# StelaBou/stylegan_directions_face_reenactment

Measured on AMD Instinct MI355X. Metric: reenacted frames/sec @256x256, higher is better.
Workload: dtype f32 (operands as fp16 hi+lo, 3 MFMA products, f32 accumulate)

## Files before the change

### include/sgdfr.h

```cpp
#ifndef SGDFR_H
#define SGDFR_H

#include <stdint.h>

#ifdef __cplusplus
extern "C" {
#endif

#define SGDFR_ABI_VERSION 23

#define SGDFR_MODE_PLAIN3 0
#define SGDFR_MODE_UP3 1
#define SGDFR_MODE_DOWN3 2

#define SGDFR_ACT_NONE 0
#define SGDFR_ACT_LRELU 1

int sgdfr_abi_version(void);
const char* sgdfr_last_error(void);

int sgdfr_fused_bias_act_f32(const float* x, const float* bias, const float* ref, float* y, int64_t n,
                             int step_b, int size_b, int act, int grad, float alpha, float scale,
                             void* stream);

int sgdfr_upfirdn2d_f32(const float* x, const float* k, float* y, int major, int in_h, int in_w, int minor,
                        int kh, int kw, int up_x, int up_y, int down_x, int down_y, int pad_x0, int pad_x1,
                        int pad_y0, int pad_y1, void* stream);

#define SGDFR_DTYPE_F32 0
#define SGDFR_DTYPE_F16 1
#define SGDFR_DTYPE_F64 2
int sgdfr_fused_bias_act(const void* x, const void* bias, const void* ref, void* y, int64_t n, int step_b, int size_b, int act,
                         int grad, float alpha, float scale, int dtype, void* stream);
int sgdfr_upfirdn2d(const void* x, const void* k, void* y, int major, int in_h, int in_w, int minor, int kh, int kw, int up_x,
                    int up_y, int down_x, int down_y, int pad_x0, int pad_x1, int pad_y0, int pad_y1, int dtype, void* stream);

int sgdfr_linear_f32(const float* x, int64_t ldx, const float* w, const float* bias, float* y, int64_t ldy,
                     int M, int N, int K, float wscale, float bscale, int act, float slope, float gain,
                     void* stream);

int sgdfr_pixelnorm_f32(const float* x, float* y, int B, int D, float eps, void* stream);
int sgdfr_pixelnorm_bwd_f32(const float* x, const float* g, float* dx, int B, int D, float eps, void* stream);

int sgdfr_latent_prepare_f32(const float* w, int w_is_plus, const float* shift, int shift_is_plus,
                             int shift_layers, const float* trunc, float psi, float* out, int B, int L, int D,
                             void* stream);

int sgdfr_modconv_prepack_f32(const float* weight, float* wp, float* q, float* qt, int Cout, int Cin, int k,
                              void* stream);

int sgdfr_modconv_prepack_t_f32(const float* weight, float* wt, int Cout, int Cin, int k, int flip, void* stream);

int sgdfr_style_demod_f32(const float* style, int64_t ld_style, const float* mod_w, const float* mod_b,
                          const float* q, float* s, float* d, int B, int D, int Cin, int Cout, void* stream);

#define SGDFR_MAX_STYLE_LAYERS 40
typedef struct sgdfr_style_layer {
    const float* mod_w;
    const float* mod_b;
    const float* q;
    float* s;
    float* d;
    int cin, cout, latent_index;
    float* s_n;
    float* d_n;
    const unsigned* x_absmax;
    int x_log2, headroom;
} sgdfr_style_layer;
int sgdfr_styles_batched_f32(const float* latent, int B, int L, int D, const sgdfr_style_layer* layers, int n_layers,
                             void* stream);

int sgdfr_split_range_f32(const float* s, const float* d, float* s_n, float* d_n, const unsigned* x_absmax,
                          int x_absmax_bstride, int x_log2, int headroom, int B, int Cin, int Cout, void* stream);

int sgdfr_absmax_f32(const float* x, int64_t x_bstride, int64_t n_per_image, int B, unsigned* out, int per_image,
                     void* stream);

int sgdfr_modconv2d_fwd_f32(const float* x, int64_t x_bstride, const float* wp, const float* s, const float* d,
                            const float* noise, int64_t noise_bstride, const float* noise_w, const float* bias,
                            float* y, int B, int Cin, int Cout, int H, int W, int mode, int act, float slope,
                            float gain, void* stream);

int sgdfr_modconv2d_splitk_hint(int B, int Cin, int Cout, int H, int W, int mode);
int sgdfr_modconv2d_splitk_f32(const float* x, int64_t x_bstride, const float* wp, const float* s, const float* d,
                               const float* noise, int64_t noise_bstride, const float* noise_w, const float* bias, float* y,
                               float* partials, int splits, int B, int Cin, int Cout, int H, int W, int mode, int act,
                               float slope, float gain, void* stream);

int sgdfr_modconv_prepack_wino_f32(const float* weight, float* u, int Cout, int Cin, int transpose_flip, void* stream);
int sgdfr_modconv2d_wino_supported(int B, int Cin, int Cout, int H, int W);
int sgdfr_modconv2d_wino_f32(const float* x, int64_t x_bstride, const float* u, const float* s, const float* d,
                             const float* noise, int64_t noise_bstride, const float* noise_w, const float* bias,
                             const float* zeros, float* y, int B, int Cin, int Cout, int H, int W, int act, float slope,
                             float gain, void* stream);

int sgdfr_blur_bias_act_f32(const float* t, const float* fir, const float* noise, int64_t noise_bstride,
                            const float* noise_w, const float* bias, float* y, int B, int C, int H, int W, int act,
                            float slope, float gain, unsigned int* y_absmax, void* stream);

int sgdfr_blur_bias_act_split_f32(const float* t, const float* fir, const float* noise, int64_t noise_bstride,
                                  const float* noise_w, const float* bias, const float* s_next, unsigned short* xs, int B, int C,
                                  int H, int W, int64_t plane_stride, int arith, int wino, int act, float slope, float gain,
                                  unsigned int* sat, void* stream);

int sgdfr_torgb_fwd_f32(const float* x, const float* w_rgb, const float* s, const float* bias, const float* skip,
                        const float* fir, float* y, int B, int Cin, int H, int W, void* stream);

#define SGDFR_SPLIT_BF16 0
#define SGDFR_SPLIT_FP16 1
#define SGDFR_SPLIT_FP16F8 2
int64_t sgdfr_modconv_prepack_split_elems(int Cout, int Cin);
int sgdfr_modconv_prepack_split_f32(const float* weight, unsigned short* wsp, int Cout, int Cin, int arith, int transpose_flip,
                                    unsigned int* sat, void* stream);
int sgdfr_modconv2d_split_supported(int B, int Cin, int Cout, int H, int W, int mode);
int sgdfr_modconv2d_split_f8_ok(int B, int Cin, int Cout, int H, int W, int mode);
int sgdfr_modconv2d_split_f32(const float* x, int64_t x_bstride, const unsigned short* wsp, const float* s, const float* d,
                              const float* noise, int64_t noise_bstride, const float* noise_w, const float* bias,
                              const float* zeros, float* y, float* partials, int ksplit, const float* rgb_w,
                              const float* rgb_s, float* rgb_part, int x_is_split, unsigned short* xs_out, const float* s_next,
                              int B, int Cin, int Cout, int H, int W, int mode, int64_t plane_stride, int arith, int act,
                              float slope, float gain, unsigned int* sat, void* stream);
long long sgdfr_split_saturation_count(int reset);
int sgdfr_modconv2d_split_xin_supported(int B, int Cin, int Cout, int H, int W, int mode);
int sgdfr_to_split_f32(const float* x, const float* s, unsigned short* xs, int B, int Cin, int H, int W, int arith,
                       unsigned int* sat, void* stream);
int sgdfr_planes_to_split_f32(const float* gt, const float* d, unsigned short* xs, int B, int C, int H, int W, int arith,
                              unsigned int* sat, void* stream);
int sgdfr_blur_adjoint_split_f32(const float* g, const float* fir, const float* t, const float* d, unsigned short* xs,
                                 float* asum, int B, int C, int H, int W, int arith, unsigned int* sat, void* stream);
int sgdfr_modconv2d_split_cout_tiles(int B, int Cin, int Cout, int H, int W, int mode);
int sgdfr_modconv2d_split_cout_tiles_xin(int B, int Cin, int Cout, int H, int W, int mode);
int sgdfr_modconv2d_split_ksplit_hint(int B, int Cin, int Cout, int H, int W, int mode);
int sgdfr_modconv2d_split_plan_info(int B, int Cin, int Cout, int H, int W, int mode, int xin_whole);

int sgdfr_modconv2d_wsplit_supported(int B, int Cin, int Cout, int H, int W, int f);
int sgdfr_modconv2d_wsplit_wide(int B, int Cin, int Cout, int H, int W);
#define SGDFR_SPLIT_HANDOVER_F8 0x100
int64_t sgdfr_modconv_prepack_wsplit_elems(int Cout, int Cin, int f);
int sgdfr_modconv_prepack_wsplit_f32(const float* weight, unsigned short* wsp, int Cout, int Cin, int f, int arith,
                                     unsigned int* sat, void* stream);
int sgdfr_to_wsplit_f32(const float* x, const float* s, unsigned short* vs, int B, int Cin, int H, int W, int f, int arith,
                        unsigned int* sat, void* stream);
int sgdfr_modconv2d_wsplit_f32(const unsigned short* v, const unsigned short* wsp, const float* d, const float* noise,
                               int64_t noise_bstride, const float* noise_w, const float* bias, const float* zeros, float* y,
                               const float* rgb_w, const float* rgb_s, float* rgb_part, unsigned short* xs_out,
                               const float* s_next, int B, int Cin, int Cout, int H, int W, int f, int arith, int act,
                               float slope, float gain, unsigned int* sat, void* stream);

int sgdfr_torgb_finish_f32(const float* part, int T, const float* bias, const float* skip, const float* fir, float* y, int B,
                           int H, int W, void* stream);

int sgdfr_torgb_finish_u8_f32(const float* part, int T, const float* bias, const float* skip, const float* fir,
                              unsigned char* y, int64_t row_pitch, int x_offset, int swap_rb, int B, int H, int W,
                              void* stream);

int sgdfr_image_to_u8_f32(const float* x, unsigned char* y, int B, int H, int W, void* stream);

#define SGDFR_MAX_GRID_PANELS 4
int sgdfr_grid_to_u8_f32(const float* const* panels, const int64_t* bstrides, int K, unsigned char* y, int B, int H,
                         int W, int swap_rb, void* stream);


#define SGDFR_DIR_ZERO 0
#define SGDFR_DIR_ANGLE 1
#define SGDFR_DIR_JAW 2
#define SGDFR_DIR_EXP 3
#define SGDFR_MAX_DIRECTIONS 64
struct sgdfr_direction {
    int kind;
    int col;
    double a;
    double b;
};

int sgdfr_make_shift_f32(const float* ang_s, int64_t ang_s_bstride, const float* pose_s, int64_t pose_s_bstride,
                         const float* exp_s, int64_t exp_s_bstride, const float* ang_t, const float* pose_t,
                         const float* exp_t, int pose_dim, int exp_dim, const struct sgdfr_direction* table, int D,
                         float* shift, int N, int arith, void* stream);

int sgdfr_make_shift_random_f32(const float* ang_s, const float* pose_s, const float* exp_s, int pose_dim, int exp_dim,
                                const int* which, const float* u, float shift_scale, const struct sgdfr_direction* table,
                                int D, float* shift, int N, void* stream);

int sgdfr_gt_reenacted_f32(const float* pose_s, const float* exp_s, const float* ang_s, const float* pose_t, const float* exp_t,
                           int pose_dim, int exp_dim, const float* shift, const int* which, float shift_scale,
                           const struct sgdfr_direction* table, int D, float* pose_gt, float* exp_gt, int B, void* stream);

#define SGDFR_PAIRLOSS_PLAIN 0
#define SGDFR_PAIRLOSS_RANGE255 1
int64_t sgdfr_pairloss_workspace_bytes(int n);
int sgdfr_pairloss_forward_f32(const float* x, const float* y, int64_t n, int mode, float* x255, float* y255, float* loss,
                               void* workspace, int64_t workspace_bytes, void* stream);
int sgdfr_pairloss_backward_f32(const float* x, const float* y, int64_t n, int mode, const float* grad_loss,
                                const float* grad_x255, float* dx, void* stream);


struct sgdfr_sweep_record {
    double start;
    double min_shift;
    double max_shift;
    double step;
    int n_lo;
    int n_hi;
};

int sgdfr_sweep_plan_f32(const float* angles, const float* pose, const float* alpha_exp, int pose_dim, int exp_dim,
                         const struct sgdfr_direction* table, int D, const int* dirs, int K, double shift_scale, int shifts_count,
                         struct sgdfr_sweep_record* records, int N, void* stream);
int sgdfr_sweep_plan_host(const float* angles, const float* pose, const float* alpha_exp, int pose_dim, int exp_dim,
                          const struct sgdfr_direction* table, int D, const int* dirs, int K, double shift_scale, int shifts_count,
                          struct sgdfr_sweep_record* records, int N);

int sgdfr_sweep_rows_f32(const struct sgdfr_sweep_record* records, const int* row_offset, const struct sgdfr_direction* table, int D,
                         const int* dirs, int K, int N, float* rows, int* row_k, int* is_start, int R, void* stream);
int sgdfr_sweep_rows_host(const struct sgdfr_sweep_record* records, const struct sgdfr_direction* table, int D, const int* dirs, int K,
                          int N, float* rows, int* row_k, int* is_start, int64_t R);

int sgdfr_sweep_frames_f32(const float* x, int R, int P, int f, const int* is_start, const float* src, int64_t src_bstride,
                           float* pooled, float* bordered, unsigned char* frames, int panels, void* stream);

int sgdfr_video_frames_f32(const float* x, int B, int P, int f, const float* const* panels, const int64_t* bstrides, int n_left,
                           unsigned char* frames, int swap_rb, void* stream);

#define SGDFR_PANEL_F32 0
#define SGDFR_PANEL_U8 1
struct sgdfr_video_panel {
    const void* data;
    const int* index;
    int kind;
    int rows;
};

int sgdfr_video_frames_px(const float* x, int B, int P, int f, const struct sgdfr_video_panel* panels, int n_left,
                          unsigned char* frames, int swap_rb, void* stream);


int sgdfr_act_grad_reduce_f32(const float* g_out, const float* out, const float* noise, int64_t noise_bstride,
                              const float* noise_w, const float* bias, float* g_pre, float* sums, int B, int C, int HW,
                              float slope, float gain, int want_y, unsigned int* g_absmax, void* stream);

int sgdfr_blur_adjoint_f32(const float* g, const float* fir, const float* t, float* gt, float* asum, int B, int C, int H,
                           int W, void* stream);

int sgdfr_scale_reduce_f32(const float* gu, const float* x, int64_t x_bstride, const float* s, float* dx, float* r, int B,
                           int C, int HW, void* stream);

int sgdfr_torgb_bwd_f32(const float* x, const float* g, const float* w_rgb, const float* s, float* dx, float* r, int B,
                        int Cin, int H, int W, void* stream);

int sgdfr_grad_join_f32(const float* out, const float* gu, const float* s_next, const float* g_rgb, const float* w_rgb,
                        const float* s_rgb, const float* g_add, const float* noise, int64_t noise_bstride, const float* noise_w,
                        const float* bias, float* g_pre, float* sums, unsigned int* g_absmax, float* r_next, float* r_rgb, int B,
                        int C, int HW, float slope, float gain, int want_y, int zero_outputs, void* stream);

typedef struct sgdfr_style_grad_layer {
    const float* gs;
    const float* rgb_r;
    const float* rgb_w;
    const float* a;
    const float* d;
    const float* s;
    const float* qt;
    const float* mod_w;
    float* ds;
    float* gmod_w;
    float* gmod_b;
    int64_t a_stride;
    int cin, cout, latent_index;
} sgdfr_style_grad_layer;
int sgdfr_styles_batched_bwd_f32(const sgdfr_style_grad_layer* layers, int n_layers, const float* latent, float* glat, int B, int L,
                                 int D, void* stream);

int sgdfr_demod_dq_f32(const float* a, int64_t a_stride, const float* d, const float* s, float* dq, int B, int Cin, int Cout,
                       void* stream);

#define SGDFR_PGRAD_BIAS 0
#define SGDFR_PGRAD_NOISE 1
#define SGDFR_PGRAD_RGB_W 2
#define SGDFR_PGRAD_RGB_B 3
#define SGDFR_MAX_PARAM_GRADS 64
typedef struct sgdfr_param_grad {
    const float* in;
    const float* aux;
    float* out;
    int kind, C, HW;
    float scale;
} sgdfr_param_grad;
int sgdfr_param_grads_f32(const sgdfr_param_grad* entries, int n, int B, void* stream);

#define SGDFR_MAX_ADAM_TENSORS 96
typedef struct sgdfr_adam_tensor {
    float* p;
    const float* g;
    float* m;
    float* v;
    int64_t n;
} sgdfr_adam_tensor;
int sgdfr_adam_f32(const sgdfr_adam_tensor* tensors, int n, const float* step, float lr, float beta1, float beta2, float eps, void* stream);

int sgdfr_demod_grad_f32(const float* gd, const float* d, const float* qt, const float* s, const float* gs, float* ds,
                         int B, int Cin, int Cout, void* stream);

int sgdfr_modconv_wgrad_f32(const float* g, const float* d, const float* x, int64_t x_bstride, const float* s, float* dwp,
                            int B, int Cin, int Cout, int H, int W, int mode, void* stream);

int sgdfr_modconv_wgrad_finish_f32(const float* dwp, const float* wp, const float* dq, float* dweight, int Cout, int Cin,
                                   void* stream);
int sgdfr_modconv_wgrad_ksplit(int B, int Cin, int Cout, int H, int W, int mode);
// ... 150 lines not shown
```

### stylegan_directions_face_reenactment_amd/_native.py

```python
import ctypes
import os

import torch

_HERE = os.path.dirname(os.path.abspath(__file__))
LIB_PATH = os.path.join(_HERE, 'csrc', 'libsgdfr_hip.so')
if os.environ.get('SGDFR_LIB'):
    if os.environ.get('SGDFR_ALLOW_LIB_OVERRIDE') == '1':
        import sys as _sys
        LIB_PATH = os.environ['SGDFR_LIB']
        _sys.stderr.write('stylegan_directions_face_reenactment_amd: loading the native library from SGDFR_LIB=%s\n' % LIB_PATH)
    else:
        import warnings as _warnings
        _warnings.warn('SGDFR_LIB is set but ignored (set SGDFR_ALLOW_LIB_OVERRIDE=1 to load a probe build)', RuntimeWarning)
ABI_VERSION = 23

_c_f32p = ctypes.c_void_p
_i, _i64, _f = ctypes.c_int, ctypes.c_int64, ctypes.c_float

SIGNATURES = {
    'sgdfr_fused_bias_act_f32': [_c_f32p, _c_f32p, _c_f32p, _c_f32p, _i64, _i, _i, _i, _i, _f, _f, ctypes.c_void_p],
    'sgdfr_upfirdn2d_f32': [_c_f32p, _c_f32p, _c_f32p] + [_i] * 14 + [ctypes.c_void_p],
    'sgdfr_linear_f32': [_c_f32p, _i64, _c_f32p, _c_f32p, _c_f32p, _i64, _i, _i, _i, _f, _f, _i, _f, _f,
                         ctypes.c_void_p],
    'sgdfr_pixelnorm_f32': [_c_f32p, _c_f32p, _i, _i, _f, ctypes.c_void_p],
    'sgdfr_pixelnorm_bwd_f32': [_c_f32p, _c_f32p, _c_f32p, _i, _i, _f, ctypes.c_void_p],
    'sgdfr_latent_prepare_f32': [_c_f32p, _i, _c_f32p, _i, _i, _c_f32p, _f, _c_f32p, _i, _i, _i, ctypes.c_void_p],
    'sgdfr_modconv_prepack_f32': [_c_f32p, _c_f32p, _c_f32p, _c_f32p, _i, _i, _i, ctypes.c_void_p],
    'sgdfr_modconv_prepack_t_f32': [_c_f32p, _c_f32p, _i, _i, _i, _i, ctypes.c_void_p],
    'sgdfr_act_grad_reduce_f32': [_c_f32p, _c_f32p, _c_f32p, _i64, _c_f32p, _c_f32p, _c_f32p, _c_f32p, _i, _i, _i, _f,
                                  _f, _i, ctypes.c_void_p, ctypes.c_void_p],
    'sgdfr_blur_adjoint_f32': [_c_f32p, _c_f32p, _c_f32p, _c_f32p, _c_f32p, _i, _i, _i, _i, ctypes.c_void_p],
    'sgdfr_scale_reduce_f32': [_c_f32p, _c_f32p, _i64, _c_f32p, _c_f32p, _c_f32p, _i, _i, _i, ctypes.c_void_p],
    'sgdfr_torgb_bwd_f32': [_c_f32p, _c_f32p, _c_f32p, _c_f32p, _c_f32p, _c_f32p, _i, _i, _i, _i, ctypes.c_void_p],
    'sgdfr_modconv_wgrad_f32': [_c_f32p, _c_f32p, _c_f32p, _i64, _c_f32p, _c_f32p, _i, _i, _i, _i, _i, _i, ctypes.c_void_p],
    'sgdfr_modconv_wgrad_finish_f32': [_c_f32p, _c_f32p, _c_f32p, _c_f32p, _i, _i, ctypes.c_void_p],
    'sgdfr_modconv_wgrad_parts_f32': [_c_f32p, _c_f32p, _c_f32p, _i64, _c_f32p, _c_f32p, _i, _i, _i, _i, _i, _i, ctypes.c_void_p],
    'sgdfr_modconv_wgrad_finish_parts_f32': [_c_f32p, _i, _c_f32p, _c_f32p, _c_f32p, _i, _i, ctypes.c_void_p],
    'sgdfr_modconv_wgrad_finish_parts_oik_f32': [_c_f32p, _i, _c_f32p, _c_f32p, _c_f32p, _i64, _c_f32p, _c_f32p, _i, _c_f32p, _i, _i,
                                                 ctypes.c_void_p],
    'sgdfr_modconv_prepack_wino_f32': [_c_f32p, _c_f32p, _i, _i, _i, ctypes.c_void_p],
    'sgdfr_modconv2d_wino_supported': [_i, _i, _i, _i, _i],
    'sgdfr_modconv2d_wino_f32': [_c_f32p, _i64, _c_f32p, _c_f32p, _c_f32p, _c_f32p, _i64, _c_f32p, _c_f32p, _c_f32p,
                                 _c_f32p, _i, _i, _i, _i, _i, _i, _f, _f, ctypes.c_void_p],
    'sgdfr_modconv_prepack_split_f32': [_c_f32p, ctypes.c_void_p, _i, _i, _i, _i, ctypes.c_void_p, ctypes.c_void_p],
    'sgdfr_modconv2d_split_supported': [_i, _i, _i, _i, _i, _i],
    'sgdfr_modconv2d_split_f32': [_c_f32p, _i64, ctypes.c_void_p, _c_f32p, _c_f32p, _c_f32p, _i64, _c_f32p, _c_f32p, _c_f32p,
                                  _c_f32p, _c_f32p, _i, _c_f32p, _c_f32p, _c_f32p, _i, ctypes.c_void_p, _c_f32p, _i, _i, _i, _i,
                                  _i, _i, _i64, _i, _i, _f, _f, ctypes.c_void_p, ctypes.c_void_p],
    'sgdfr_to_split_f32': [_c_f32p, _c_f32p, ctypes.c_void_p, _i, _i, _i, _i, _i, ctypes.c_void_p, ctypes.c_void_p],
    'sgdfr_planes_to_split_f32': [_c_f32p, _c_f32p, ctypes.c_void_p, _i, _i, _i, _i, _i, ctypes.c_void_p, ctypes.c_void_p],
    'sgdfr_blur_adjoint_split_f32': [_c_f32p, _c_f32p, _c_f32p, _c_f32p, ctypes.c_void_p, _c_f32p, _i, _i, _i, _i, _i, ctypes.c_void_p,
                                     ctypes.c_void_p],
    'sgdfr_modconv2d_split_cout_tiles': [_i, _i, _i, _i, _i, _i],
    'sgdfr_modconv2d_split_cout_tiles_xin': [_i, _i, _i, _i, _i, _i],
    'sgdfr_modconv2d_split_xin_supported': [_i, _i, _i, _i, _i, _i],
    'sgdfr_modconv2d_split_ksplit_hint': [_i, _i, _i, _i, _i, _i],
    'sgdfr_modconv2d_split_plan_info': [_i, _i, _i, _i, _i, _i, _i],
    'sgdfr_torgb_finish_f32': [_c_f32p, _i, _c_f32p, _c_f32p, _c_f32p, _c_f32p, _i, _i, _i, ctypes.c_void_p],
    'sgdfr_torgb_finish_u8_f32': [_c_f32p, _i, _c_f32p, _c_f32p, _c_f32p, ctypes.c_void_p, _i64, _i, _i, _i, _i, _i, ctypes.c_void_p],
    'sgdfr_image_to_u8_f32': [_c_f32p, ctypes.c_void_p, _i, _i, _i, ctypes.c_void_p],
    'sgdfr_grid_to_u8_f32': [ctypes.POINTER(ctypes.c_void_p), ctypes.POINTER(ctypes.c_int64), _i, ctypes.c_void_p, _i, _i, _i,
                             _i, ctypes.c_void_p],
    'sgdfr_modconv2d_splitk_hint': [_i, _i, _i, _i, _i, _i],
    'sgdfr_modconv2d_splitk_f32': [_c_f32p, _i64, _c_f32p, _c_f32p, _c_f32p, _c_f32p, _i64, _c_f32p, _c_f32p, _c_f32p,
                                   _c_f32p, _i, _i, _i, _i, _i, _i, _i, _i, _f, _f, ctypes.c_void_p],
    'sgdfr_demod_grad_f32': [_c_f32p, _c_f32p, _c_f32p, _c_f32p, _c_f32p, _c_f32p, _i, _i, _i, ctypes.c_void_p],
    'sgdfr_style_demod_f32': [_c_f32p, _i64, _c_f32p, _c_f32p, _c_f32p, _c_f32p, _c_f32p, _i, _i, _i, _i,
                              ctypes.c_void_p],
    'sgdfr_modconv2d_fwd_f32': [_c_f32p, _i64, _c_f32p, _c_f32p, _c_f32p, _c_f32p, _i64, _c_f32p, _c_f32p, _c_f32p,
                                _i, _i, _i, _i, _i, _i, _i, _f, _f, ctypes.c_void_p],
    'sgdfr_blur_bias_act_f32': [_c_f32p, _c_f32p, _c_f32p, _i64, _c_f32p, _c_f32p, _c_f32p, _i, _i, _i, _i, _i, _f,
                                _f, ctypes.c_void_p, ctypes.c_void_p],
    'sgdfr_blur_bias_act_split_f32': [_c_f32p, _c_f32p, _c_f32p, _i64, _c_f32p, _c_f32p, _c_f32p, ctypes.c_void_p, _i, _i, _i, _i, _i64,
                                      _i, _i, _i, _f, _f, ctypes.c_void_p, ctypes.c_void_p],
    'sgdfr_torgb_fwd_f32': [_c_f32p, _c_f32p, _c_f32p, _c_f32p, _c_f32p, _c_f32p, _c_f32p, _i, _i, _i, _i,
                            ctypes.c_void_p],
}



class Direction(ctypes.Structure):
    _fields_ = [('kind', ctypes.c_int), ('col', ctypes.c_int), ('a', ctypes.c_double), ('b', ctypes.c_double)]


DIR_ZERO, DIR_ANGLE, DIR_JAW, DIR_EXP = 0, 1, 2, 3
MAX_DIRECTIONS = 64
SIGNATURES['sgdfr_make_shift_f32'] = [_c_f32p, _i64, _c_f32p, _i64, _c_f32p, _i64, _c_f32p, _c_f32p, _c_f32p, _i, _i,
                                      ctypes.POINTER(Direction), _i, _c_f32p, _i, _i, ctypes.c_void_p]
SIGNATURES['sgdfr_make_shift_random_f32'] = [_c_f32p, _c_f32p, _c_f32p, _i, _i, ctypes.c_void_p, _c_f32p, _f,
                                             ctypes.POINTER(Direction), _i, _c_f32p, _i, ctypes.c_void_p]
SIGNATURES['sgdfr_gt_reenacted_f32'] = [_c_f32p, _c_f32p, _c_f32p, _c_f32p, _c_f32p, _i, _i, _c_f32p, ctypes.c_void_p, _f,
                                        ctypes.POINTER(Direction), _i, _c_f32p, _c_f32p, _i, ctypes.c_void_p]


class StyleLayer(ctypes.Structure):
    _fields_ = [('mod_w', ctypes.c_void_p), ('mod_b', ctypes.c_void_p), ('q', ctypes.c_void_p),
                ('s', ctypes.c_void_p), ('d', ctypes.c_void_p), ('cin', ctypes.c_int), ('cout', ctypes.c_int),
                ('latent_index', ctypes.c_int), ('s_n', ctypes.c_void_p), ('d_n', ctypes.c_void_p),
                ('x_absmax', ctypes.c_void_p), ('x_log2', ctypes.c_int), ('headroom', ctypes.c_int)]


SIGNATURES['sgdfr_split_range_f32'] = [_c_f32p, _c_f32p, _c_f32p, _c_f32p, ctypes.c_void_p, _i, _i, _i, _i, _i, _i, ctypes.c_void_p]
SIGNATURES['sgdfr_absmax_f32'] = [_c_f32p, _i64, _i64, _i, ctypes.c_void_p, _i, ctypes.c_void_p]
SIGNATURES['sgdfr_styles_batched_f32'] = [_c_f32p, _i, _i, _i, ctypes.POINTER(StyleLayer), _i, ctypes.c_void_p]
MAX_STYLE_LAYERS = 40


class StyleGradLayer(ctypes.Structure):
    _fields_ = [('gs', ctypes.c_void_p), ('rgb_r', ctypes.c_void_p), ('rgb_w', ctypes.c_void_p), ('a', ctypes.c_void_p),
                ('d', ctypes.c_void_p), ('s', ctypes.c_void_p), ('qt', ctypes.c_void_p), ('mod_w', ctypes.c_void_p),
                ('ds', ctypes.c_void_p), ('gmod_w', ctypes.c_void_p), ('gmod_b', ctypes.c_void_p), ('a_stride', ctypes.c_longlong),
                ('cin', ctypes.c_int), ('cout', ctypes.c_int), ('latent_index', ctypes.c_int)]


class ParamGrad(ctypes.Structure):
    _fields_ = [('inp', ctypes.c_void_p), ('aux', ctypes.c_void_p), ('out', ctypes.c_void_p), ('kind', ctypes.c_int), ('C', ctypes.c_int),
                ('HW', ctypes.c_int), ('scale', ctypes.c_float)]


class AdamTensor(ctypes.Structure):
    _fields_ = [('p', ctypes.c_void_p), ('g', ctypes.c_void_p), ('m', ctypes.c_void_p), ('v', ctypes.c_void_p), ('n', ctypes.c_int64)]


MAX_ADAM_TENSORS = 96
SIGNATURES['sgdfr_adam_f32'] = [ctypes.POINTER(AdamTensor), _i, _c_f32p, _f, _f, _f, _f, ctypes.c_void_p]
PGRAD_BIAS, PGRAD_NOISE, PGRAD_RGB_W, PGRAD_RGB_B = 0, 1, 2, 3
MAX_PARAM_GRADS = 64
SIGNATURES['sgdfr_styles_batched_bwd_f32'] = [ctypes.POINTER(StyleGradLayer), _i, _c_f32p, _c_f32p, _i, _i, _i, ctypes.c_void_p]
SIGNATURES['sgdfr_demod_dq_f32'] = [_c_f32p, _i64, _c_f32p, _c_f32p, _c_f32p, _i, _i, _i, ctypes.c_void_p]
SIGNATURES['sgdfr_param_grads_f32'] = [ctypes.POINTER(ParamGrad), _i, _i, ctypes.c_void_p]
SIGNATURES['sgdfr_grad_join_f32'] = ([_c_f32p] * 7 + [_c_f32p, _i64, _c_f32p, _c_f32p, _c_f32p, _c_f32p, ctypes.c_void_p,
                                                                  _c_f32p, _c_f32p, _i, _i, _i, _f, _f, _i, _i, ctypes.c_void_p])
SIGNATURES['sgdfr_modconv2d_wsplit_supported'] = [_i, _i, _i, _i, _i, _i]
SIGNATURES['sgdfr_modconv2d_wsplit_wide'] = [_i, _i, _i, _i, _i]
SIGNATURES['sgdfr_modconv2d_split_f8_ok'] = [_i, _i, _i, _i, _i, _i]
SPLIT_HANDOVER_F8 = 0x100
SIGNATURES['sgdfr_modconv_prepack_wsplit_f32'] = [_c_f32p, ctypes.c_void_p, _i, _i, _i, _i, ctypes.c_void_p, ctypes.c_void_p]
SIGNATURES['sgdfr_to_wsplit_f32'] = [_c_f32p, _c_f32p, ctypes.c_void_p, _i, _i, _i, _i, _i, _i, ctypes.c_void_p, ctypes.c_void_p]
SIGNATURES['sgdfr_modconv2d_wsplit_f32'] = [ctypes.c_void_p, ctypes.c_void_p, _c_f32p, _c_f32p, _i64, _c_f32p, _c_f32p, _c_f32p, _c_f32p,
                                            _c_f32p, _c_f32p, _c_f32p, ctypes.c_void_p, _c_f32p, _i, _i, _i, _i, _i, _i, _i, _i, _f, _f,
                                            ctypes.c_void_p, ctypes.c_void_p]
SIGNATURES['sgdfr_fused_bias_act'] = [ctypes.c_void_p, ctypes.c_void_p, ctypes.c_void_p, ctypes.c_void_p, _i64, _i, _i, _i, _i, _f, _f, _i,
                                      ctypes.c_void_p]
SIGNATURES['sgdfr_upfirdn2d'] = [ctypes.c_void_p, ctypes.c_void_p, ctypes.c_void_p] + [_i] * 15 + [ctypes.c_void_p]
SIGNATURES['sgdfr_lpips_prepack_f32'] = [ctypes.POINTER(ctypes.c_void_p), _c_f32p, ctypes.c_void_p]
SIGNATURES['sgdfr_lpips_features_f32'] = [_c_f32p, _i, _c_f32p, _i, _i, _i, _c_f32p, _c_f32p, ctypes.c_void_p, _i64, ctypes.c_void_p]
SIGNATURES['sgdfr_lpips_distance_f32'] = [_c_f32p, _i, _c_f32p, _i, _i, _i, _i, _i, _i, _c_f32p, _c_f32p, ctypes.c_void_p, _i64,
                                          ctypes.c_void_p]
SIGNATURES['sgdfr_lpips_backward_f32'] = [_c_f32p, _c_f32p, _i, _c_f32p, _i, _i, _i, _i, _i, _i, _c_f32p, _c_f32p, ctypes.c_void_p, _i64,
                                          ctypes.c_void_p]
LPIPS_PARAMS = 17
SIGNATURES['sgdfr_idloss_prepack_f32'] = [ctypes.POINTER(ctypes.c_void_p), _c_f32p, ctypes.c_void_p]
SIGNATURES['sgdfr_idloss_forward_f32'] = [_c_f32p, _i, _c_f32p, _i, _i, _i, _i, _c_f32p, _c_f32p, _c_f32p, ctypes.c_void_p, _i64,
                                          ctypes.c_void_p]
SIGNATURES['sgdfr_idloss_backward_f32'] = [_c_f32p, _c_f32p, _i, _i, _i, _i, _c_f32p, _c_f32p, ctypes.c_void_p, _i64, ctypes.c_void_p]
IDLOSS_PARAMS = 245
SIGNATURES['sgdfr_flame_prepack_f32'] = [ctypes.POINTER(ctypes.c_void_p), _i, _i, _i, _i, _i, _i, _c_f32p, ctypes.c_void_p]
SIGNATURES['sgdfr_flame_decode_f32'] = [_c_f32p, _c_f32p, _c_f32p, _i, _c_f32p, _c_f32p, _c_f32p, _i, _c_f32p, _c_f32p, _i, _c_f32p, _c_f32p,
                                        _c_f32p, _c_f32p, ctypes.c_void_p]
SIGNATURES['sgdfr_flame_decode_backward_f32'] = [_c_f32p, _c_f32p, _c_f32p, _c_f32p, _i, _c_f32p, _i, _c_f32p, _c_f32p, _c_f32p, _c_f32p,
                                                 _c_f32p, ctypes.c_void_p, _i64, ctypes.c_void_p]
SIGNATURES['sgdfr_shape_loss_f32'] = [_c_f32p, _c_f32p, _i, _f, _f, _f, _c_f32p, _c_f32p, _c_f32p, _c_f32p, ctypes.c_void_p, _i64,
                                      ctypes.c_void_p]
FLAME_PARAMS = 15
SIGNATURES['sgdfr_deca_prepack_f32'] = [ctypes.POINTER(ctypes.c_void_p), _c_f32p, ctypes.c_void_p]
SIGNATURES['sgdfr_deca_forward_f32'] = [_c_f32p, _c_f32p, _i, _i, _i, _c_f32p, _c_f32p, _c_f32p, _c_f32p, ctypes.c_void_p, _c_f32p,
                                        ctypes.c_void_p, _i64, ctypes.c_void_p]
SIGNATURES['sgdfr_deca_backward_f32'] = [_c_f32p, _c_f32p, _c_f32p, ctypes.c_void_p, _i, _i, _i, _c_f32p, _c_f32p, ctypes.c_void_p, _i64,
                                         ctypes.c_void_p]
SIGNATURES['sgdfr_deca_crop_f32'] = [_c_f32p, _c_f32p, _i, _i, _i, _c_f32p, ctypes.c_void_p]
SIGNATURES['sgdfr_deca_crop_backward_f32'] = [_c_f32p, _c_f32p, _c_f32p, _i, _i, _i, _c_f32p, ctypes.c_void_p]
DECA_PARAMS = 134
SIGNATURES['sgdfr_fan_prepack_f32'] = [ctypes.POINTER(ctypes.c_void_p), _c_f32p, ctypes.c_void_p]
SIGNATURES['sgdfr_fan_crop_f32'] = [_c_f32p, _c_f32p, _i, _i, _i, _i, _c_f32p, ctypes.c_void_p]
SIGNATURES['sgdfr_fan_network_f32'] = [_c_f32p, _i, _c_f32p, _c_f32p, _c_f32p, ctypes.c_void_p, _i64, ctypes.c_void_p]
SIGNATURES['sgdfr_fan_decode_f32'] = [_c_f32p, _c_f32p, _i, _c_f32p, _c_f32p, _c_f32p, ctypes.c_void_p]
SIGNATURES['sgdfr_fan_boxes_f32'] = [_c_f32p, _i, _c_f32p, ctypes.c_void_p]
SIGNATURES['sgdfr_fan_forward_f32'] = [_c_f32p, _c_f32p, _i, _i, _i, _i, _c_f32p, _c_f32p, _c_f32p, _c_f32p, _c_f32p, _c_f32p,
                                       ctypes.c_void_p, _i64, ctypes.c_void_p]
FAN_PARAMS = 735
FAN_RANGE_255, FAN_RANGE_GAN = 0, 1
SIGNATURES['sgdfr_fan_flip_add_f32'] = [_c_f32p, _i, _c_f32p, ctypes.c_void_p]
SIGNATURES['sgdfr_fan_draw_f32'] = [_c_f32p, _i, _c_f32p, ctypes.c_void_p]
SIGNATURES['sgdfr_fan_forward3d_f32'] = ([_c_f32p, _c_f32p, _i, _i, _i, _i, _i] + [_c_f32p] * 11 + [ctypes.c_void_p, _i64, ctypes.c_void_p,
                                                                                                     _i64, ctypes.c_void_p])
SIGNATURES['sgdfr_fandepth_prepack_f32'] = [ctypes.POINTER(ctypes.c_void_p), _c_f32p, ctypes.c_void_p]
SIGNATURES['sgdfr_fandepth_network_f32'] = [_c_f32p, _c_f32p, _i, _c_f32p, _c_f32p, _c_f32p, ctypes.c_void_p, _i64, ctypes.c_void_p]
FANDEPTH_PARAMS = 312
_ip = ctypes.c_void_p
SIGNATURES['sgdfr_s3fd_level_dims'] = [_i, _i, ctypes.POINTER(ctypes.c_int)]
SIGNATURES['sgdfr_s3fd_prepack_f32'] = [ctypes.POINTER(ctypes.c_void_p), _c_f32p, ctypes.c_void_p]
SIGNATURES['sgdfr_s3fd_network_f32'] = [_c_f32p, _i, _i, _i, _i, _c_f32p, _c_f32p, _c_f32p, ctypes.c_void_p, _i64, ctypes.c_void_p]
SIGNATURES['sgdfr_s3fd_candidates_f32'] = [ctypes.POINTER(ctypes.c_void_p), ctypes.POINTER(ctypes.c_int), _i, _f, _i, _c_f32p, _ip, _ip,
                                           ctypes.c_void_p]
SIGNATURES['sgdfr_s3fd_nms_f32'] = [_c_f32p, _ip, _i, _i, _c_f32p, _ip, _ip, ctypes.c_void_p]
SIGNATURES['sgdfr_s3fd_forward_f32'] = [_c_f32p, _i, _i, _i, _i, _c_f32p, _f, _i, _c_f32p, _ip, _ip, _c_f32p, _ip, _ip, _c_f32p, _c_f32p,
                                        ctypes.c_void_p, _i64, ctypes.c_void_p]
S3FD_PARAMS = 50
SIGNATURES['sgdfr_e4e_prepack_f32'] = [ctypes.POINTER(ctypes.c_void_p), _i, _c_f32p, ctypes.c_void_p]
SIGNATURES['sgdfr_e4e_forward_f32'] = [_c_f32p, _i, _i, _c_f32p, _c_f32p, _c_f32p, ctypes.c_void_p, _i64, ctypes.c_void_p]
_u8p = ctypes.c_void_p
# ... 163 lines not shown
```

### stylegan_directions_face_reenactment_amd/chain.py

```python
import torch

from . import _native as N
from .config import config
from .functional import (_shape_query, blur_bias_act, blur_bias_act_split, modconv_split, modconv_wsplit, split_ok, wsplit_ok)


class SplitAct:
    __slots__ = ('xs', 'shape', 'wino', 'arith')

    def __init__(self, xs, shape, wino=0, arith=None):
        self.xs, self.shape, self.wino = xs, tuple(shape), (2 if wino is True else int(wino or 0))
        self.arith = arith


def xin_ok(B, cin, cout, H, W, mode=N.MODE_PLAIN3):
    return config().use_split_chain and split_ok(B, cin, cout, H, W, mode) and \
        bool(_shape_query('sgdfr_modconv2d_split_xin_supported', B, cin, cout, H, W, mode))


def styled_conv_split(x, wsp, s, d, cout, upsample=False, fir=None, noise=None, noise_weight=None, bias=None, batch=None,
                      s_next=None, rgb=None, want_y=True, wino_next=False, arith_next=None, xs_arith=None):
    if isinstance(x, SplitAct) and x.wino:
        if upsample:
            raise RuntimeError('styled_conv_split: the Winograd input form feeds plain convs only')
        B, cin, H, W = x.shape
        res = modconv_wsplit(x.xs, x.shape, wsp, d, cout, noise, noise_weight, bias, True, rgb=rgb,
                             want_y=want_y and s_next is None, s_next=s_next, f=x.wino, arith=x.arith,
                             xs_arith=xs_arith if s_next is not None else None)
        if s_next is not None:
            _, part, xs = res
            return SplitAct(xs, (B, cout, H, W), arith=xs_arith), part
        return res if rgb is not None else (res, None)
    x_arith = None
    if isinstance(x, SplitAct):
        B, cin, H, W = x.shape
        xin, x_split, s_arg = x.xs, x.shape, None
        batch = B
        x_arith = x.arith
    else:
        xin, x_split, s_arg = x, None, s
        B = s.shape[0] if batch is None else batch
        H, W = x.shape[2], x.shape[3]
    if not upsample:
        res = modconv_split(xin, wsp, s_arg, d, cout, noise, noise_weight, bias, True, batch=batch, rgb=rgb,
                            want_y=want_y and s_next is None, x_split=x_split, s_next=s_next, arith=x_arith)
        if s_next is not None:
            _, part, xs = res
            return SplitAct(xs, (B, cout, H, W)), part
        return res if rgb is not None else (res, None)
    if s_next is not None and config().use_plane_padding and \
            _shape_query('sgdfr_modconv2d_split_ksplit_hint', B, x_split[1] if x_split else x.shape[1], cout, H, W, N.MODE_UP3) == 1:
        ps = ((H + 1) * (W + 1) + 31) // 32 * 32
        planes = modconv_split(xin, wsp, s_arg, d, cout, batch=batch, mode=N.MODE_UP3, x_split=x_split, plane_stride=ps, arith=x_arith)
        xs = blur_bias_act_split(planes, fir, H, W, s_next, noise, noise_weight, bias, True, plane_stride=ps, wino=wino_next,
                                 arith=arith_next if wino_next != 2 else None)
        return SplitAct(xs, (B, cout, 2 * H, 2 * W), wino_next, arith_next if wino_next != 2 else None), None
    planes = modconv_split(xin, wsp, s_arg, d, cout, batch=batch, mode=N.MODE_UP3, x_split=x_split, arith=x_arith)
    if s_next is not None:
        xs = blur_bias_act_split(planes, fir, H, W, s_next, noise, noise_weight, bias, True, wino=wino_next,
                                 arith=arith_next if wino_next != 2 else None)
        return SplitAct(xs, (B, cout, 2 * H, 2 * W), wino_next, arith_next if wino_next != 2 else None), None
    return blur_bias_act(planes, fir, H, W, noise, noise_weight, bias, True), None


def _interleaved_planes_ok(B, cin, H, W):
    import os
    if not config().use_plane_padding or os.environ.get('SGDFR_PLANE_IL', '1') == '0':
        return False
    return all(_shape_query('sgdfr_modconv2d_split_ksplit_hint', B, c, cin, H // 2, W // 2, N.MODE_UP3) == 1 for c in (cin, 2 * cin))


def wsplit_chain_f(B, cin, cout, H, W):
    if not (config().use_wsplit and config().use_split_chain and config().wsplit_min_cin > 0 and cin >= config().wsplit_min_cin and W <= 256):
        return 0
    if W > 128 and not _interleaved_planes_ok(B, cin, H, W):
        return 0
    for f in ((4, 2) if config().wsplit_f == 4 else (2,)):
        if wsplit_ok(B, cin, cout, H, W, f) and (f == 4 or cin >= max(config().wsplit_min_cin, 256)) and (W <= 128 or f == 4):
            return f
    return 0


def _f8_cross_on():
    return config().precision == 'fp16x3' and config().cross_terms == 'fp8' and config().range_plan is True


def wsplit_chain_arith(B, cin, cout, H, W, f):
    if f == 4 and _f8_cross_on() and cin % 32 == 0 and \
            _shape_query('sgdfr_modconv2d_wsplit_wide', B, cin, cout, H, W):
        return 'fp16f8'
    return None


def xs_chain_arith(B, cin, cout, H, W, nxt_cout):
    if _f8_cross_on() and \
            _shape_query('sgdfr_modconv2d_split_f8_ok', B, cout, nxt_cout, H, W, N.MODE_UP3) and \
            _shape_query('sgdfr_modconv2d_split_ksplit_hint', B, cout, nxt_cout, H, W, N.MODE_UP3) == 1:
        return 'fp16f8'
    return None


def xs_plain_arith(B, cin, cout, H, W):
    if _f8_cross_on() and \
            _shape_query('sgdfr_modconv2d_split_f8_ok', B, cin, cout, H, W, N.MODE_PLAIN3) and \
            _shape_query('sgdfr_modconv2d_split_ksplit_hint', B, cin, cout, H, W, N.MODE_PLAIN3) == 1:
        return 'fp16f8'
    return None


def wsplit_chain_ok(B, cin, cout, H, W):
    return wsplit_chain_f(B, cin, cout, H, W) != 0


def rgb_fusable(B, cin, cout, H, W):
    return config().use_rgb_fusion and split_ok(B, cin, cout, H, W) and \
        (not config().use_splitk or _shape_query('sgdfr_modconv2d_split_ksplit_hint', B, cin, cout, H, W, N.MODE_PLAIN3) == 1)


class StreamPipeline:

    def __init__(self, n=2, device=None):
        self.streams = [torch.cuda.Stream(device=device) for _ in range(max(1, int(n)))]
        self._i = 0
        self.last = None

    def next(self):
        s = self.streams[self._i % len(self.streams)]
        self._i += 1
        s.wait_stream(torch.cuda.current_stream(s.device))
        self.last = s
        return torch.cuda.stream(s)

    def join(self, *tensors, stream=None):
        cur = torch.cuda.current_stream(self.streams[0].device)
        for s in ([stream] if stream is not None else self.streams):
            cur.wait_stream(s)
        for t in tensors:
            if isinstance(t, torch.Tensor) and t.is_cuda:
                t.record_stream(cur)
```

### stylegan_directions_face_reenactment_amd/csrc/split.hip

```cpp
#include "split_kernel.h"

namespace sgdfr {

template <int ET>
__global__ __launch_bounds__(256) void to_split_kernel(const float* __restrict__ x, const float* __restrict__ s,
                                                      unsigned char* __restrict__ xs, int B, int Cin, int HW,
                                                      unsigned* __restrict__ sat_word) {
    const int G = Cin / 8;
    const int64_t n = (int64_t)B * G * HW;
    unsigned sat = 0;
    for (int64_t idx = (int64_t)blockIdx.x * blockDim.x + threadIdx.x; idx < n; idx += (int64_t)gridDim.x * blockDim.x) {
        const int pix = (int)(idx % HW);
        const int64_t bg = idx / HW;
        const int g = (int)(bg % G);
        const int b = (int)(bg / G);
        const float* xp = x + ((int64_t)b * Cin + g * 8) * HW + pix;
        const float* sp = s + (int64_t)b * Cin + g * 8;
        uint4 vh, vl;
        unsigned* ph = reinterpret_cast<unsigned*>(&vh);
        unsigned* pl = reinterpret_cast<unsigned*>(&vl);
        constexpr int ETM = ws_main_et<ET>::value;
        const float sc = (ETM == SGDFR_SPLIT_FP16) ? SPLIT_F16_XSCALE : 1.f;
#pragma unroll
        for (int c = 0; c < 4; ++c)
// ... 145 lines not shown
            p.simgs = 1;
        } else if (PT % HW == 0) {
            span = (PT / HW - 1) * p.R * p.P + (H - 1) * p.P + (W - 1);
            p.simgs = PT / HW;
        } else {
            return 0;
        }
        p.xlen = span + 2 * p.P + 3;
        p.n_pix_tiles = (int)((p.total_pix + PT - 1) / PT);
    }
    const bool slim = plan.cfg == 8;
    p.xs = (plan.nw == 8 || slim) ? (p.xlen + 63) & ~63 : (p.xlen + 7) & ~7;
    p.n_cout_tiles = (Cout + plan.nt - 1) / plan.nt;
    const int nthr = plan.nw * 64;
    if ((2 * p.xs + nthr - 1) / nthr > (mode == SGDFR_MODE_DOWN3 ? 3 : 4)) return 0;
    const size_t lds = split_lds_bytes(p, plan.nt, plan.nss, down, 2, plan.pt, slim);
    if (lds > (plan.nw == 8 ? 160 : 80) * 1024) return 0;
    if (slim && p.simgs > 2) return 0;
    if (out) *out = p;
    return 1;
}

static const SplitPlan* split_plan(int B, int Cin, int Cout, int H, int W, int mode, SplitParams* out, bool xin_whole = false) {
    static const int deep = getenv("SGDFR_SPLIT_DEEP") ? atoi(getenv("SGDFR_SPLIT_DEEP")) : 1;
    static const int narrow_first = getenv("SGDFR_SPLIT_UP_NARROW") ? atoi(getenv("SGDFR_SPLIT_UP_NARROW")) : 0;
    const SplitPlan* order[6] = {nullptr, nullptr, nullptr, nullptr, nullptr, nullptr};
    int n = 0;
    if (mode == SGDFR_MODE_UP3) {
        const bool big = (int64_t)B * (H + 1) * (W + 1) * (Cout / 64) >= 256 * 256;
        if (deep && big) order[n++] = &kPlanUpDeep;
        if (narrow_first && big) order[n++] = &kPlanUpNarrow;
        if (Cout % 128 == 0) order[n++] = &kPlanUpWide;
        order[n++] = &kPlanUpNarrow;
    } else if (mode == SGDFR_MODE_PLAIN3) {
        static const int xl = getenv("SGDFR_SPLIT_XL") ? atoi(getenv("SGDFR_SPLIT_XL")) : 1;
        if (xl && xin_whole && Cout % 128 == 0 && (int64_t)B * H * W * (Cout / 128) >= 2ll * 256 * 512) order[n++] = &kPlanPlainXL;
        const int p4 = getenv("SGDFR_SPLIT_P4") ? atoi(getenv("SGDFR_SPLIT_P4")) : 64;
        const bool p4_ok = p4 > 0 && xin_whole && Cin <= p4 && (int64_t)B * H * W * ((Cout + 63) / 64) >= 4ll * 512 * 256;
        if (p4_ok && Cout % 128 == 0 && p4 >= 128) order[n++] = &kPlanPlain4;
        if (Cout % 128 == 0) order[n++] = &kPlanPlainWide;
        if (p4_ok) order[n++] = &kPlanPlain4;
        order[n++] = &kPlanPlainNarrow;
    } else if (mode == SGDFR_MODE_DOWN3) {
        order[n++] = &kPlanDown;
    }
    for (int i = 0; i < n; ++i)
        if (split_geometry(B, Cin, Cout, H, W, mode, *order[i], out)) return order[i];
    return nullptr;
}


extern "C" int sgdfr_modconv2d_split_supported(int B, int Cin, int Cout, int H, int W, int mode) {
    SplitParams p;
    return split_plan(B, Cin, Cout, H, W, mode, &p) ? 1 : 0;
}

extern "C" int sgdfr_modconv2d_split_f8_ok(int B, int Cin, int Cout, int H, int W, int mode) {
    SplitParams p;
    if (mode != SGDFR_MODE_UP3 && mode != SGDFR_MODE_PLAIN3) return 0;
    const SplitPlan* plan = split_plan(B, Cin, Cout, H, W, mode, &p, true);
    return plan && plan->cfg == (mode == SGDFR_MODE_UP3 ? 4 : 8) ? 1 : 0;
}

extern "C" int sgdfr_modconv2d_split_ksplit_hint(int B, int Cin, int Cout, int H, int W, int mode) {
    SplitParams p;
    if (!split_plan(B, Cin, Cout, H, W, mode, &p)) return 1;
    const int blocks = p.n_pix_tiles * p.n_cout_tiles;
    if (blocks >= 192) return 1;
    static const int target = getenv("SGDFR_SPLIT_KTARGET") ? atoi(getenv("SGDFR_SPLIT_KTARGET")) : 256;
    int s = target / blocks;
    const int max_by_k = (Cin / SPLIT_CB) / 2;
    if (s > max_by_k) s = max_by_k;
    if (s > 16) s = 16;
    return s < 2 ? 1 : s;
}

extern "C" int sgdfr_to_split_f32(const float* x, const float* s, unsigned short* xs, int B, int Cin, int H, int W, int arith,
                                  unsigned int* sat, void* stream) {
    SGDFR_REQUIRE(B >= 0 && Cin > 0 && Cin % 8 == 0 && H > 0 && W > 0, "to_split: bad shape B=%d Cin=%d H=%d W=%d (Cin %% 8)", B, Cin, H, W);
    SGDFR_REQUIRE(arith == SGDFR_SPLIT_BF16 || arith == SGDFR_SPLIT_FP16 || arith == SGDFR_SPLIT_FP16F8, "to_split: arith must be SGDFR_SPLIT_BF16/FP16/FP16F8");
    if (B == 0) return 0;
    SGDFR_REQUIRE(x && s && xs && (reinterpret_cast<uintptr_t>(xs) & 15) == 0, "to_split: null or misaligned pointer");
    int64_t g = ((int64_t)B * (Cin / 8) * H * W + 255) / 256;
    if (g > 256 * 32) g = 256 * 32;
    if (arith == SGDFR_SPLIT_FP16F8)
        hipLaunchKernelGGL(to_split_kernel<SGDFR_SPLIT_FP16F8>, dim3((int)g), dim3(256), 0, as_stream(stream), x, s,
                           reinterpret_cast<unsigned char*>(xs), B, Cin, H * W, sat);
    else if (arith == SGDFR_SPLIT_FP16)
        hipLaunchKernelGGL(to_split_kernel<SGDFR_SPLIT_FP16>, dim3((int)g), dim3(256), 0, as_stream(stream), x, s,
                           reinterpret_cast<unsigned char*>(xs), B, Cin, H * W, sat);
    else
        hipLaunchKernelGGL(to_split_kernel<SGDFR_SPLIT_BF16>, dim3((int)g), dim3(256), 0, as_stream(stream), x, s,
                           reinterpret_cast<unsigned char*>(xs), B, Cin, H * W, sat);
    return check_launch("to_split");
}

extern "C" int sgdfr_planes_to_split_f32(const float* gt, const float* d, unsigned short* xs, int B, int C, int H, int W,
                                        int arith, unsigned int* sat, void* stream) {
    SGDFR_REQUIRE(B >= 0 && C > 0 && C % 8 == 0 && H > 0 && W > 0, "planes_to_split: bad shape B=%d C=%d H=%d W=%d (C %% 8)", B, C, H, W);
    SGDFR_REQUIRE(arith == SGDFR_SPLIT_BF16 || arith == SGDFR_SPLIT_FP16, "planes_to_split: arith must be SGDFR_SPLIT_BF16/FP16");
    if (B == 0) return 0;
    SGDFR_REQUIRE(gt && xs && (reinterpret_cast<uintptr_t>(xs) & 15) == 0, "planes_to_split: null or misaligned pointer");
    const int RP = (H + 1) * (W + 1);
    int64_t g = ((int64_t)B * 4 * (C / 8) * RP + 255) / 256;
    if (g > 256 * 32) g = 256 * 32;
    if (arith == SGDFR_SPLIT_FP16)
        hipLaunchKernelGGL(planes_to_split_kernel<SGDFR_SPLIT_FP16>, dim3((int)g), dim3(256), 0, as_stream(stream), gt, d,
                           reinterpret_cast<unsigned char*>(xs), B, C, RP, sat);
    else
        hipLaunchKernelGGL(planes_to_split_kernel<SGDFR_SPLIT_BF16>, dim3((int)g), dim3(256), 0, as_stream(stream), gt, d,
                           reinterpret_cast<unsigned char*>(xs), B, C, RP, sat);
    return check_launch("planes_to_split");
}

unsigned int blur_split_saturation_count(int reset);
namespace sgdfr { unsigned int wsplit_saturation_count(int reset); }

extern "C" long long sgdfr_split_saturation_count(int reset) {
    unsigned int v = 0;
    if (hipMemcpyFromSymbol(&v, HIP_SYMBOL(g_split_saturated), sizeof(v)) != hipSuccess) return -1;
    if (reset) {
        const unsigned int z = 0;
        if (hipMemcpyToSymbol(HIP_SYMBOL(g_split_saturated), &z, sizeof(z)) != hipSuccess) return -1;
    }
    return (long long)v + (long long)blur_split_saturation_count(reset) + (long long)sgdfr::wsplit_saturation_count(reset);
}

#ifdef SGDFR_SPLIT_PROBE
extern "C" int sgdfr_split_trace_read(unsigned long long* out, int n) {
    if (n > 4096) n = 4096;
    if (hipDeviceSynchronize() != hipSuccess) return 1;
    return hipMemcpyFromSymbol(out, HIP_SYMBOL(g_split_trace), sizeof(unsigned long long) * n) == hipSuccess ? 0 : 1;
}
#endif

extern "C" int sgdfr_modconv2d_split_xin_supported(int B, int Cin, int Cout, int H, int W, int mode) {
    SplitParams p;
    const SplitPlan* plan = split_plan(B, Cin, Cout, H, W, mode, &p);
    if (!plan || !(plan->cfg == 0 || plan->cfg == 1 || plan->cfg == 3 || plan->cfg == 4 || plan->cfg == 5)) return 0;
    if (plan->nss == 3 && plan->cfg != 5 && split_lds_bytes(p, plan->nt, plan->nss, false, 3) > 160 * 1024) return 0;
    return 1;
}

extern "C" int sgdfr_modconv2d_split_cout_tiles(int B, int Cin, int Cout, int H, int W, int mode) {
    SplitParams p;
    return split_plan(B, Cin, Cout, H, W, mode, &p) ? p.n_cout_tiles : 0;
}

extern "C" int sgdfr_modconv2d_split_cout_tiles_xin(int B, int Cin, int Cout, int H, int W, int mode) {
    SplitParams p;
    return split_plan(B, Cin, Cout, H, W, mode, &p, true) ? p.n_cout_tiles : 0;
}

extern "C" int sgdfr_modconv2d_split_plan_info(int B, int Cin, int Cout, int H, int W, int mode, int xin_whole) {
    SplitParams p;
    const SplitPlan* plan = split_plan(B, Cin, Cout, H, W, mode, &p, xin_whole != 0);
    if (!plan) return -1;
    const int nthr = plan->nw * 64, nex = (2 * p.xs + nthr - 1) / nthr;
    const int nex_max = mode == SGDFR_MODE_DOWN3 ? 3 : 4;
    const int half = (plan->nt == 64 && Cout % 64 == 32) ? 1 : 0;
    return plan->cfg | (nex <= 2 ? 2 : nex == 3 ? 3 : nex_max) << 4 | p.simgs << 8 | half << 20;
}

static int64_t split_pack_body_elems(int n_out, int n_in) { return (int64_t)((n_out + 63) / 64 * 64) * n_in * 9 * 2; }
extern "C" int64_t sgdfr_modconv_prepack_split_elems(int Cout, int Cin) { return split_pack_body_elems(Cout, Cin) + 8; }

extern "C" int sgdfr_modconv_prepack_split_f32(const float* weight, unsigned short* wsp, int Cout, int Cin, int arith,
                                               int transpose_flip, unsigned int* sat, void* stream) {
    SGDFR_REQUIRE(arith == SGDFR_SPLIT_BF16 || arith == SGDFR_SPLIT_FP16 || (arith == SGDFR_SPLIT_FP16F8 && transpose_flip == 0),
                  "prepack_split: arith must be SGDFR_SPLIT_BF16/FP16 (or FP16F8 for a forward pack)");
    SGDFR_REQUIRE(transpose_flip >= 0 && transpose_flip <= 2, "prepack_split: transpose_flip is 0 (forward), 1 (adjoint of "
                  "the plain conv) or 2 (adjoint of the transposed conv)");
    const int n_out = transpose_flip ? Cin : Cout, n_in = transpose_flip ? Cout : Cin;
    SGDFR_REQUIRE(Cout > 0 && Cin > 0 && n_in % SPLIT_CB == 0 && (n_out % 64 == 0 || (transpose_flip == 0 && n_out % 64 == 32)),
                  "prepack_split: needs in-channels %% 16 == 0 and out-channels %% 64 == 0 (forward pack: %% 32), got in=%d out=%d",
                  n_in, n_out);
    SGDFR_REQUIRE(weight && wsp, "prepack_split: null pointer");
    if (n_out % 64 != 0) {
        if (hipMemsetAsync(wsp, 0, sizeof(unsigned short) * (size_t)split_pack_body_elems(Cout, Cin), as_stream(stream)) !=
            hipSuccess) {
            set_error("prepack_split: hipMemsetAsync failed");
            return 2;
        }
    }
    const int64_t n = (int64_t)Cout * Cin * 9;
    int64_t g = (n + 255) / 256;
    if (g > 4096) g = 4096;
    const float scale = (arith != SGDFR_SPLIT_BF16 ? SPLIT_F16_WSCALE : 1.f) / sqrtf((float)Cin * 9);
    {
        unsigned* const trailer = reinterpret_cast<unsigned*>(wsp + split_pack_body_elems(n_out, n_in));
        if (hipMemsetAsync(trailer, 0, 16, as_stream(stream)) != hipSuccess) { (void)hipGetLastError(); set_error("prepack_split: hipMemsetAsync failed"); return 2; }
        if (arith == SGDFR_SPLIT_FP16F8) hipLaunchKernelGGL(split_absmax_kernel, dim3(256), dim3(256), 0, as_stream(stream), weight, n, scale, trailer);
    }
    hipLaunchKernelGGL(prepack_split_kernel, dim3((int)g), dim3(256), 0, as_stream(stream), weight, wsp, Cout, Cin,
                       64, scale, arith, transpose_flip, sat);
    return check_launch("modconv_prepack_split");
}

template <int MODE, int ET, int WM, int WN, int MI, int NI, int NSS = 3, bool XIN = false>
static int launch_split(const SplitParams& p, hipStream_t st, int lid0 = 0, int count = -1) {
    constexpr int NTHR = WM * WN * 64;
    const int nex = (2 * p.xs + NTHR - 1) / NTHR;
    constexpr int NEX_MAX = (MODE == SGDFR_MODE_DOWN3) ? 3 : 4;
    SGDFR_REQUIRE(nex <= NEX_MAX, "modconv_split: staged range %d too long for mode %d", p.xlen, MODE);
    void (*kern)(SplitParams) = nex <= 2   ? split_mfma_kernel<MODE, ET, WM, WN, MI, NI, 2, NSS, XIN>
                                : nex == 3 ? split_mfma_kernel<MODE, ET, WM, WN, MI, NI, 3, NSS, XIN>
                                           : split_mfma_kernel<MODE, ET, WM, WN, MI, NI, NEX_MAX, NSS, XIN>;
    const size_t lds = split_lds_bytes(p, WM * MI * 32, NSS, MODE == SGDFR_MODE_DOWN3,
                                       (XIN && MODE != SGDFR_MODE_DOWN3 && NSS == 3 && NI <= 2 && WM * WN == 8) ? 3 : 2, WN * NI * 32,
                                       XIN && WM * WN == 4);
    if (hipFuncSetAttribute(reinterpret_cast<const void*>(kern), hipFuncAttributeMaxDynamicSharedMemorySize, (int)lds) !=
        hipSuccess) {
        (void)hipGetLastError();
        set_error("modconv_split: LDS request %zu B refused (B=%d Cin=%d Cout=%d H=%d W=%d xs=%d simgs=%d)", lds, p.B, p.Cin, p.Cout,
                  p.H, p.W, p.xs, p.simgs);
        return 2;
    }
    SplitParams q = p;
    q.total_blocks = count >= 0 ? count : p.n_pix_tiles * p.n_cout_tiles * p.ksplit;
    q.lid0 = lid0;
    static const int persist = getenv("SGDFR_SPLIT_PERSIST") ? atoi(getenv("SGDFR_SPLIT_PERSIST")) : 256;
    static const int persist_min = getenv("SGDFR_SPLIT_PERSIST_MIN") ? atoi(getenv("SGDFR_SPLIT_PERSIST_MIN")) : 4;
    static const int persist_min_up = getenv("SGDFR_SPLIT_PERSIST_MIN_UP") ? atoi(getenv("SGDFR_SPLIT_PERSIST_MIN_UP")) : 4;
    constexpr bool kCanPersist = XIN && NSS == 3 && WM * WN == 8 && (MODE == SGDFR_MODE_PLAIN3 || MODE == SGDFR_MODE_UP3);
    const bool persistent = kCanPersist && persist > 0 &&
                            q.total_blocks >= (MODE == SGDFR_MODE_UP3 ? persist_min_up : persist_min) * persist;
    const int grid = persistent ? persist : q.total_blocks;
    hipLaunchKernelGGL(kern, dim3(grid), dim3(NTHR), lds, st, q);
    return check_launch("modconv2d_split");
}

template <int MODE, int ET, int MI, bool XIN>
static int launch_deep_tail(const SplitParams& p, hipStream_t st) {
    const char* env = getenv("SGDFR_SPLIT_UP_TAIL");
    const int total = p.n_pix_tiles * p.n_cout_tiles;
    const int n_full = total / 256 * 256, tail = total - n_full;
    const int max_full = (env && atoi(env) > 1) ? atoi(env) : (MODE == SGDFR_MODE_DOWN3 ? 1024 : 512);
    if ((env && atoi(env) == 0) || p.ksplit != 1 || n_full == 0 || n_full > max_full || tail == 0 || tail > 128)
        return launch_split<MODE, ET, 2, 4, MI, 2, 1, XIN>(p, st);
    if (int rc = launch_split<MODE, ET, 2, 4, MI, 2, 1, XIN>(p, st, 0, n_full)) return rc;
    SplitParams t = p;
    constexpr int PT2 = 128;
    t.xlen = PT2 + p.P + 2;
    t.xs = (t.xlen + 63) & ~63;
    t.simgs = (t.xlen - 1) / p.rps + 2;
    t.n_pix_tiles = (int)((p.total_pix + PT2 - 1) / PT2);
    t.desync = 0;
    fill_fastdivs(t);
    const int c0 = n_full / p.n_pix_tiles, p0 = n_full - c0 * p.n_pix_tiles;
    const int lid0 = c0 * t.n_pix_tiles + 2 * p0;
    const int count = t.n_cout_tiles * t.n_pix_tiles - lid0;
    if (count <= 0) return 0;
    return launch_split<MODE, ET, 2, 4, MI, 1, 1, XIN>(t, st, lid0, count);
}

template <int ET>
static int launch_plan(int cfg, const SplitParams& p, hipStream_t st, bool xin) {
    if (xin) {
        switch (cfg) {
            case 0: return launch_split<SGDFR_MODE_PLAIN3, ET, 2, 4, 2, 2, 3, true>(p, st);
            case 1: return launch_split<SGDFR_MODE_PLAIN3, ET, 1, 8, 2, 2, 3, true>(p, st);
            case 3: return launch_split<SGDFR_MODE_UP3, ET, 2, 4, 1, 2, 3, true>(p, st);
            case 4: return launch_deep_tail<SGDFR_MODE_UP3, ET, 1, true>(p, st);
            case 5: return launch_deep_tail<SGDFR_MODE_DOWN3, ET, 2, true>(p, st);
            case 6: return launch_split<SGDFR_MODE_PLAIN3, ET, 2, 4, 2, 4, 3, true>(p, st);
            case 8: return launch_split<SGDFR_MODE_PLAIN3, ET, 1, 4, 2, 2, 3, true>(p, st);
            default: set_error("modconv_split: pre-split input is not built for tiling plan %d", cfg); return 1;
        }
    }
    if (cfg == 5) {
        set_error("modconv_split: DOWN3 reads the phase-major split planes of sgdfr_planes_to_split_f32 (x_is_split = 1)");
        return 1;
    }
    switch (cfg) {
        case 0: return launch_split<SGDFR_MODE_PLAIN3, ET, 2, 4, 2, 2, 3>(p, st);
        case 1: return launch_split<SGDFR_MODE_PLAIN3, ET, 1, 8, 2, 2, 3>(p, st);
        case 2: return launch_split<SGDFR_MODE_UP3, ET, 4, 2, 1, 2, 3>(p, st);
        case 3: return launch_split<SGDFR_MODE_UP3, ET, 2, 4, 1, 2, 3>(p, st);
        default: return launch_deep_tail<SGDFR_MODE_UP3, ET, 1, false>(p, st);
    }
}

extern "C" int sgdfr_modconv2d_split_f32(const float* x, int64_t x_bstride, const unsigned short* wsp, const float* s,
                                         const float* d, const float* noise, int64_t noise_bstride, const float* noise_w,
                                         const float* bias, const float* zeros, float* y, float* partials, int ksplit,
                                         const float* rgb_w, const float* rgb_s, float* rgb_part, int x_is_split,
                                         unsigned short* xs_out, const float* s_next, int B, int Cin, int Cout, int H, int W,
                                         int mode, int64_t plane_stride, int arith, int act, float slope, float gain,
                                         unsigned int* sat, void* stream) {
    SGDFR_REQUIRE(arith == SGDFR_SPLIT_BF16 || arith == SGDFR_SPLIT_FP16 ||
                      (arith == SGDFR_SPLIT_FP16F8 && sgdfr_modconv2d_split_f8_ok(B, Cin, Cout, H, W, mode) && x_is_split && ksplit <= 1),
                  "modconv_split: arith must be SGDFR_SPLIT_BF16/FP16 (FP16F8: only where sgdfr_modconv2d_split_f8_ok() says so, with a "
                  "pre-split input and no K slices)");
    SGDFR_REQUIRE(B >= 0 && Cin > 0 && Cout > 0 && H > 0 && W > 0, "modconv_split: bad shape B=%d Cin=%d Cout=%d H=%d W=%d",
                  B, Cin, Cout, H, W);
    if (B == 0) return 0;
    SGDFR_REQUIRE(sgdfr_modconv2d_split_supported(B, Cin, Cout, H, W, mode),
                  "modconv_split: shape B=%d Cin=%d Cout=%d H=%d W=%d mode=%d not supported; use sgdfr_modconv2d_fwd_f32", B,
                  Cin, Cout, H, W, mode);
    SGDFR_REQUIRE(mode == SGDFR_MODE_PLAIN3 || (!noise && !bias && !act), "modconv_split: UP3 writes raw parity planes "
                  "(noise / bias / activation belong to sgdfr_blur_bias_act_f32), DOWN3 a raw gradient");
    SGDFR_REQUIRE(mode != SGDFR_MODE_DOWN3 || (x_is_split && y && !rgb_part && !xs_out), "modconv_split: DOWN3 takes "
                  "pre-split planes and writes y only");
    SGDFR_REQUIRE(x && wsp && zeros && (y || rgb_part || xs_out) && (s || x_is_split), "modconv_split: null pointer");
    SGDFR_REQUIRE(!xs_out || (s_next && mode == SGDFR_MODE_PLAIN3 && ksplit <= 1 && Cout % 8 == 0 &&
                              (reinterpret_cast<uintptr_t>(xs_out) & 15) == 0),
                  "modconv_split: xs_out needs s_next, mode PLAIN3, ksplit == 1 and a 16-byte aligned buffer");
    SGDFR_REQUIRE(!x_is_split || (x_bstride != 0 && (reinterpret_cast<uintptr_t>(x) & 15) == 0),
                  "modconv_split: a pre-split input is per image and 16-byte aligned");
    SGDFR_REQUIRE(!noise || noise_w, "modconv_split: noise without noise_w");
    SGDFR_REQUIRE(((reinterpret_cast<uintptr_t>(wsp) | reinterpret_cast<uintptr_t>(s)) & 15) == 0,
                  "modconv_split: wsp and s must be 16-byte aligned");
    SplitParams p;
    const SplitPlan* plan = split_plan(B, Cin, Cout, H, W, mode, &p, x_is_split != 0 && ksplit <= 1);
    if (plane_stride != 0) {
        SGDFR_REQUIRE(mode == SGDFR_MODE_UP3 && plane_stride >= (int64_t)p.R * p.P && plane_stride < (1 << 30) && ksplit <= 1,
                      "modconv_split: plane_stride is for UP3 launches without K slices, >= (H+1)*(W+1)");
        p.rps = (int)plane_stride;
        static const int il_env = getenv("SGDFR_PLANE_IL") ? atoi(getenv("SGDFR_PLANE_IL")) : 1;
        p.plane_il = il_env;
        p.total_pix = (int64_t)B * p.rps;
        SGDFR_REQUIRE(p.total_pix + 4ll * p.P + 8 < (1ll << 31), "modconv_split: padded position space too large");
        p.n_pix_tiles = (int)((p.total_pix + plan->pt - 1) / plan->pt);
        p.simgs = (p.xlen - 1) / p.rps + 2;
    }
    p.f8_max = nullptr;
    p.x = x; p.x_bstride = x_bstride; p.wsp = wsp; p.s = s; p.d = d; p.noise = noise; p.noise_bstride = noise_bstride;
    p.noise_w = noise_w; p.bias = bias; p.zeros = zeros; p.y = y;
    p.act = act; p.slope = slope; p.gain = gain; p.sat = sat;
    if (ksplit < 1) ksplit = 1;
    SGDFR_REQUIRE(!rgb_part || (rgb_w && rgb_s && mode == SGDFR_MODE_PLAIN3 && ksplit == 1),
                  "modconv_split: the fused ToRGB needs rgb_w, rgb_s, mode PLAIN3 and ksplit == 1");
    p.rgb_w = rgb_w; p.rgb_s = rgb_s; p.rgb_part = rgb_part;
    p.xs_out = reinterpret_cast<unsigned char*>(xs_out); p.s_next = s_next;
    SGDFR_REQUIRE(ksplit == 1 || (partials && ksplit <= Cin / SPLIT_CB), "modconv_split: ksplit %d needs a partials buffer "
                  "and at most %d slices", ksplit, Cin / SPLIT_CB);
    const int64_t n_out = (mode == SGDFR_MODE_UP3) ? (int64_t)B * Cout * 4 * p.rps : (int64_t)B * Cout * H * W;
    p.ksplit = ksplit;
    p.split_stride = n_out;
    if (ksplit > 1) p.y = partials;
    static const int stagger = getenv("SGDFR_SPLIT_STAGGER") ? atoi(getenv("SGDFR_SPLIT_STAGGER")) : 1;
    p.stagger = stagger;
    p.dbg = getenv("SGDFR_SPLIT_DBG") ? atoi(getenv("SGDFR_SPLIT_DBG")) : 0;
    {
        static const int pct = getenv("SGDFR_SPLIT_DESYNC") ? atoi(getenv("SGDFR_SPLIT_DESYNC")) : 75;
        const bool up = mode == SGDFR_MODE_UP3;
        const double mfma_clk = (double)(Cin / SPLIT_CB / ksplit) * (up ? 54 : 108) * 32 * 2 / 0.55;
        const double store_clk = (double)plan->nt * plan->pt * (up ? 4 : 1) * 4 / 8.3;
        const int blocks = p.n_pix_tiles * p.n_cout_tiles * ksplit;
        p.desync = (up && pct > 0 && blocks >= 1024) ? (int)((mfma_clk + store_clk) * pct / 100 / 4096) : 0;
    }
    fill_fastdivs(p);
    hipStream_t st = as_stream(stream);
    if (arith == SGDFR_SPLIT_FP16F8) {
        p.f8_max = reinterpret_cast<const float*>(wsp + split_pack_body_elems(Cout, Cin));
        return mode == SGDFR_MODE_UP3 ? launch_split<SGDFR_MODE_UP3, SGDFR_SPLIT_FP16F8, 2, 4, 1, 2, 1, true>(p, st)
                                      : launch_split<SGDFR_MODE_PLAIN3, SGDFR_SPLIT_FP16F8, 1, 4, 2, 2, 3, true>(p, st);
    }
    const int rc = arith == SGDFR_SPLIT_FP16 ? launch_plan<SGDFR_SPLIT_FP16>(plan->cfg, p, st, x_is_split != 0)
                                             : launch_plan<SGDFR_SPLIT_BF16>(plan->cfg, p, st, x_is_split != 0);
    if (rc || ksplit == 1) return rc;
    const bool plain = mode == SGDFR_MODE_PLAIN3;
    return launch_splitk_reduce(partials, ksplit, n_out, plain ? noise : nullptr, noise_bstride, noise_w, plain ? bias : nullptr, y,
                                Cout, plain ? H * W : 1, plain ? act : 0, slope, gain, st);
}
```

### stylegan_directions_face_reenactment_amd/csrc/split_kernel.h

```cpp
#pragma once
#include <stdlib.h>

#include <type_traits>

#include "common.h"

namespace sgdfr {

typedef float f32x16 __attribute__((ext_vector_type(16)));
typedef __bf16 bf16x8 __attribute__((ext_vector_type(8)));
typedef __bf16 bf16x2 __attribute__((ext_vector_type(2)));
typedef _Float16 f16x8 __attribute__((ext_vector_type(8)));
typedef _Float16 f16x2 __attribute__((ext_vector_type(2)));
typedef float f32x2 __attribute__((ext_vector_type(2)));
typedef int frag128 __attribute__((ext_vector_type(4)));

template <int ET>
__device__ __forceinline__ f32x16 split_mfma(frag128 a, frag128 b, f32x16 c) {
    if (ET == SGDFR_SPLIT_FP16 || ET == SGDFR_SPLIT_FP16F8)
        return __builtin_amdgcn_mfma_f32_32x32x16_f16(__builtin_bit_cast(f16x8, a), __builtin_bit_cast(f16x8, b), c, 0, 0, 0);
    return __builtin_amdgcn_mfma_f32_32x32x16_bf16(__builtin_bit_cast(bf16x8, a), __builtin_bit_cast(bf16x8, b), c, 0, 0, 0);
}
static __device__ unsigned int g_split_saturated = 0;

#ifdef SGDFR_SPLIT_PROBE
__device__ unsigned long long g_split_trace[4096];
#define SPLIT_TRACE(id)                                                                                              \
    do {                                                                                                             \
        if (trace_on) {                                                                                              \
            if (ntrace < 4094)                                                                                       \
                g_split_trace[1 + ntrace] = ((unsigned long long)(id) << 48) | (__builtin_amdgcn_s_memtime() & 0xffffffffffffull); \
            ++ntrace;                                                                                                \
        }                                                                                                            \
    } while (0)
#else
#define SPLIT_TRACE(id) do {} while (0)
#endif

#define SGDFR_MODE_UPF 3

constexpr float SPLIT_F16_XSCALE = 0.0625f, SPLIT_F16_WSCALE = 64.f, SPLIT_F16_OUT = 0.25f, SPLIT_F16_MAX = 65504.f;

struct SplitParams {
    const float* x;
    int64_t x_bstride;
    const unsigned short* wsp;
    const float* s;
    const float* d;
    const float* noise;
    int64_t noise_bstride;
    const float* noise_w;
    const float* bias;
    const float* zeros;
    float* y;
    const float* rgb_w;
    const float* rgb_s;
    float* rgb_part;
    unsigned char* xs_out;
    const float* s_next;
    unsigned* sat;
    int B, Cin, Cout, H, W;
    int P, R;
    int n_pix_tiles, n_cout_tiles;
    int xs, xlen;
    int patch;
    int TC, TR, tiles_x, tiles_y, seglen;
    int simgs;
    int64_t total_pix;
    int act;
    float slope, gain;
    int ksplit;
    int64_t split_stride;
    int desync;
    int stagger;
    int dbg;
    int total_blocks;
    int rps;
    int plane_il;
    int tstep_r, tstep_c, torg;
    int tpos;
    const float* fir;
    const float* f8_max;
    FastDiv fd_xs, fd_seglen, fd_P, fd_R, fd_RP, fd_rps, fd_HW, fd_W, fd_TC, fd_tiles_x, fd_per_img, fd_npt, fd_tps, fd_Cin;
    int lid0;
};

static void fill_fastdivs(SplitParams& p) {
    p.fd_xs = make_fastdiv(p.xs); p.fd_seglen = make_fastdiv(p.seglen); p.fd_P = make_fastdiv(p.P); p.fd_R = make_fastdiv(p.R);
    p.fd_RP = make_fastdiv(p.R * p.P); p.fd_rps = make_fastdiv(p.rps); p.fd_HW = make_fastdiv(p.H * p.W); p.fd_W = make_fastdiv(p.W);
    p.fd_TC = make_fastdiv(p.TC); p.fd_tiles_x = make_fastdiv(p.tiles_x); p.fd_per_img = make_fastdiv(p.tiles_x * p.tiles_y);
    p.fd_npt = make_fastdiv(p.n_pix_tiles); p.fd_tps = make_fastdiv(p.n_pix_tiles * p.n_cout_tiles); p.fd_Cin = make_fastdiv(p.Cin);
}

constexpr int SPLIT_CB = 16;

template <int N>
__device__ __forceinline__ void split_wait_vmcnt() {
    asm volatile("s_waitcnt vmcnt(%0)" ::"n"(N) : "memory");
}

__device__ __forceinline__ void split_wait_vmcnt_dyn(int n) {
    switch (n) {
        case 0: split_wait_vmcnt<0>(); break;
        case 1: split_wait_vmcnt<1>(); break;
        case 2: split_wait_vmcnt<2>(); break;
        case 3: split_wait_vmcnt<3>(); break;
        case 4: split_wait_vmcnt<4>(); break;
        case 5: split_wait_vmcnt<5>(); break;
        case 6: split_wait_vmcnt<6>(); break;
        case 7: split_wait_vmcnt<7>(); break;
        default: split_wait_vmcnt<8>(); break;
    }
}

template <int ET>
__device__ __forceinline__ void split_pair(float a, float b, unsigned& hi, unsigned& lo, unsigned& sat) {
    if (ET == SGDFR_SPLIT_FP16) {
        sat += (!(fabsf(a) <= SPLIT_F16_MAX) || !(fabsf(b) <= SPLIT_F16_MAX)) ? 1u : 0u;
        a = __builtin_amdgcn_fmed3f(a, -SPLIT_F16_MAX, SPLIT_F16_MAX);
        b = __builtin_amdgcn_fmed3f(b, -SPLIT_F16_MAX, SPLIT_F16_MAX);
        f32x2 v = {a, b};
        f16x2 h = __builtin_convertvector(v, f16x2);
        hi = __builtin_bit_cast(unsigned, h);
        f32x2 hf = __builtin_convertvector(h, f32x2);
        f32x2 r = {a - hf[0], b - hf[1]};
        f16x2 l = __builtin_convertvector(r, f16x2);
        lo = __builtin_bit_cast(unsigned, l);
    } else {
        f32x2 v = {a, b};
        bf16x2 h = __builtin_convertvector(v, bf16x2);
        hi = __builtin_bit_cast(unsigned, h);
        const float ha = __builtin_bit_cast(float, hi << 16), hb = __builtin_bit_cast(float, hi & 0xffff0000u);
        f32x2 r = {a - ha, b - hb};
        bf16x2 l = __builtin_convertvector(r, bf16x2);
        lo = __builtin_bit_cast(unsigned, l);
    }
}

__device__ __forceinline__ void split_flush_saturation(unsigned sat, unsigned* word) {
    if (__builtin_expect(sat != 0, 0)) atomicAdd(word ? word : &g_split_saturated, sat);
}

template <int MODE, int ET_, int WM, int WN, int MI, int NI, int NEX, int NSS, bool XIN = false>
__global__ __launch_bounds__(WM * WN * 64, WM * WN == 4 ? 2 : 1) void split_mfma_kernel(SplitParams p) {
    constexpr bool F8 = (ET_ == SGDFR_SPLIT_FP16F8);
    constexpr int ET = F8 ? SGDFR_SPLIT_FP16 : ET_;
    static_assert(!F8 || (XIN && ((MODE == SGDFR_MODE_UP3 && NSS == 1 && MI == 1) || (MODE == SGDFR_MODE_PLAIN3 && NSS == 3 && NI == 2 && WM * WN == 4))),
                  "fp8 cross terms: the deep transposed plan and the 4-wave plain plan only");
    constexpr int NW = WM * WN;
    constexpr int NTHR = NW * 64;
    constexpr int NT = WM * MI * 32, PT = WN * NI * 32;
    constexpr bool UPF = (MODE == SGDFR_MODE_UPF);
    constexpr bool UP = (MODE == SGDFR_MODE_UP3) || UPF, DOWN = (MODE == SGDFR_MODE_DOWN3);
    static_assert(!UPF || (XIN && NSS == 1 && MI == 1 && NI == 2 && NW == 8), "the fused blur epilogue is written for the 64 x 256 deep plan");
    constexpr int PH = UP ? 4 : 1;
    static_assert(!DOWN || (XIN && NSS == 1), "DOWN3 stages pre-split planes, one (channel block, phase) pair per stage");
    static_assert(NW == 8 || NW == 4, "4 or 8 waves per block");
    static_assert(NT % 64 == 0 && (NSS == 1 || NSS == 3), "cout tiles are packed 64 wide");
    constexpr int RPS = 3 / NSS;
    constexpr int WT = NT / 64;
    constexpr int WROW64 = 64 * 192;
    constexpr int WTAP = 4096;
    constexpr int WSLOT_TAPS = DOWN ? 4 : RPS * 3;
    constexpr int WTILE_BYTES = WSLOT_TAPS * WTAP;
    constexpr int WROW_BYTES = WT * WTILE_BYTES;
    constexpr int WCHUNKS = WROW_BYTES / 1024;
    constexpr bool RING3 = XIN && !DOWN && NSS == 3 && NI <= 2 && NW == 8;
    constexpr int NWS = RING3 ? 3 : 2;
    extern __shared__ __attribute__((aligned(16))) unsigned char smem[];
    const int xbuf_bytes = 64 * p.xs;
    unsigned char* const xb0 = smem;
    unsigned char* const wb0 = smem + 2 * xbuf_bytes;
    float* const ls = reinterpret_cast<float*>(wb0 + NWS * WROW_BYTES);

    const int tid = threadIdx.x, lane = tid & 63, wave = __builtin_amdgcn_readfirstlane(tid >> 6);
    const int f8_sa = F8 ? 127 + ws_f8_wexp(*p.f8_max) - WS_F8_XLO : 127;
    const int wm = wave / WN, wn = wave % WN;
    const int l31 = lane & 31, hi = lane >> 5;
    const int HW = p.H * p.W;
    const int HWin = DOWN ? p.R * p.P : HW;

    constexpr bool PERSIST = XIN && NW == 8 && (MODE == SGDFR_MODE_PLAIN3 || (UP && RING3));
    auto lid_of = [&](int base) -> int {
        if (base >= p.total_blocks) return -1;
        const int nblk = PERSIST ? min((int)gridDim.x, p.total_blocks - base) : (int)gridDim.x, q8 = nblk >> 3, r8 = nblk & 7;
        if ((int)blockIdx.x >= nblk) return -1;
        const int xcd = blockIdx.x & 7, idx = blockIdx.x >> 3;
        return p.lid0 + base + (xcd < r8 ? xcd * (q8 + 1) : r8 * (q8 + 1) + (xcd - r8) * q8) + idx;
    };
    struct TileOrg { int ks, ct, pt, q0, img0, row0, col0; };
    auto tile_org = [&](int lid) -> TileOrg {
        TileOrg t;
        const int tiles_per_slice = p.n_pix_tiles * p.n_cout_tiles;
        t.ks = fdiv(lid, p.fd_tps);
        const int lt = lid - t.ks * tiles_per_slice;
        t.ct = fdiv(lt, p.fd_npt);
        t.pt = lt - t.ct * p.n_pix_tiles;
        t.q0 = 0; t.row0 = 0; t.col0 = 0;
        if (p.patch) {
            const int per_img = p.tiles_x * p.tiles_y;
            t.img0 = fdiv(t.pt, p.fd_per_img);
            const int rem = t.pt - t.img0 * per_img;
            const int ty = fdiv(rem, p.fd_tiles_x), tx = rem - ty * p.tiles_x;
            t.row0 = ty * p.tstep_r + p.torg;
            t.col0 = tx * p.tstep_c + p.torg;
        } else if (UP || DOWN) {
            t.q0 = t.pt * PT;
            t.img0 = fdiv(t.q0, UP ? p.fd_rps : p.fd_RP);
        } else {
            const int p0 = t.pt * PT;
            t.img0 = fdiv(p0, p.fd_HW);
            const int rem = p0 - t.img0 * HW;
            const int a = fdiv(rem, p.fd_W), b = rem - a * p.W;
            t.q0 = (t.img0 * p.R + a + 1) * p.P + b + 1 - p.P - 1;
        }
        return t;
    };
    auto xin_addr = [&](const TileOrg& t, int e) -> int64_t {
        const int i = tid + e * NTHR;
        const int h = fdiv(i, p.fd_xs);
        const int j = i - h * p.xs;
        if (!(h < 2 && j < p.xs)) return -2;
        bool ok = j < p.xlen;
        int img, pix;
        if (p.patch) {
            const int sg = fdiv(j, p.fd_seglen), cc = j - sg * p.seglen;
            const int row = t.row0 - 1 + sg, col = t.col0 - 1 + cc;
            img = t.img0;
            ok = ok && row >= 0 && row < p.H && col >= 0 && col < p.W && img < p.B;
            pix = row * p.W + col;
        } else if (DOWN) {
            const int q = t.q0 + j;
            img = fdiv(q, p.fd_RP);
            pix = q - img * HWin;
            ok = ok && img < p.B;
        } else if (UP) {
            const int q = t.q0 + j;
            img = fdiv(q, p.fd_rps);
            const int r = q - img * p.rps;
            const int pr = fdiv(r, p.fd_P), pc = r - pr * p.P;
            ok = ok && r < p.R * p.P && pc >= 1 && pr >= 1 && img < p.B;
            pix = (pr - 1) * p.W + (pc - 1);
        } else {
            const int q = t.q0 + j;
            const int qq = q < 0 ? 0 : q;
            const int pir = fdiv(qq, p.fd_P), pc = qq - pir * p.P;
            img = fdiv(pir, p.fd_R);
            const int pr = pir - img * p.R;
            ok = ok && pc >= 1 && pr >= 1 && img < p.B && q >= 0;
            pix = (pr - 1) * p.W + (pc - 1);
        }
        return ok ? ((((int64_t)img * (p.Cin / 8) + h) * 2) * HWin + pix) * 16 : -1;
    };
    const bool late = XIN && !DOWN && NW == 8 && wave >= 4 && !(p.stagger & 4);
    int nxw[2] = {0, 0};
    if (RING3) {
#pragma unroll
        for (int e = 0; e < NEX; ++e)
            if (wave * 64 + e * NTHR < 2 * p.xs) nxw[e & 1] += 2;
    }
    unsigned sat = 0;
    int base = 0;
    int xsel = 0, wsel = 0;
    bool prefetched = false;
#ifdef SGDFR_SPLIT_PROBE
    const bool trace_on = (p.dbg & 64) && (int)blockIdx.x == ((p.dbg >> 8) & 0xff) && tid == 64 * ((p.dbg >> 16) & 7);
    int ntrace = 0;
#endif
    do {
    SPLIT_TRACE(1);
    const int lid = lid_of(base);
    if (lid < 0) break;
    const int lid_n = PERSIST ? lid_of(base + gridDim.x) : -1;
    const bool has_next = PERSIST && lid_n >= 0 && p.simgs <= 2;
    if (p.desync > 0 && blockIdx.x < 256 && base == 0) {
        const int slot = (int)((blockIdx.x * 2654435761u) >> 24);
        const int n_sleep = (slot * p.desync) >> 8;
        for (int i = 0; i < n_sleep; ++i) __builtin_amdgcn_s_sleep(64);
    }
    const TileOrg T = tile_org(lid), Tn = has_next ? tile_org(lid_n) : T;
    const int ks = T.ks, ct = T.ct, pt = T.pt, q0 = T.q0, img0 = T.img0, row0 = T.row0, col0 = T.col0;
    const int n0 = ct * NT;

    const bool whole = p.ksplit == 1;
    const bool fuse_rgb = !UP && !DOWN && whole && p.rgb_part != nullptr;
    const bool early = p.simgs <= 2;
    constexpr bool SLIM = XIN && NW == 4;
    float* const dl = early ? ls + ((DOWN || SLIM) ? 0 : ((p.simgs * p.Cin + 3) & ~3)) : reinterpret_cast<float*>(smem);
    float* const bl = dl + p.simgs * NT;
    float* const cw = bl + NT;
    float* const red = cw + p.simgs * NT * 4;
    float* const sn = red + WM * PT * 3;
    const bool emit_xs = (!UP || UPF) && !DOWN && whole && p.xs_out != nullptr;
    struct TabVals { float dv, bv, sv, rv, w0, w1, w2; };
    auto tables_load = [&](int e) -> TabVals {
        const int m = e / NT, c = e - m * NT;
        const bool cok = n0 + c < p.Cout;
        const bool in = img0 + m < p.B && cok;
        const int64_t bc = (int64_t)(img0 + m) * p.Cout + n0 + c;
        TabVals t;
        t.dv = (p.d && in) ? p.d[bc] : 1.f;
        t.bv = (whole && p.bias && cok) ? p.bias[n0 + c] : 0.f;
        t.sv = (emit_xs && in) ? p.s_next[bc] : 0.f;
        t.rv = (fuse_rgb && in) ? p.rgb_s[bc] : 0.f;
        t.w0 = (fuse_rgb && cok) ? p.rgb_w[n0 + c] : 0.f;
        t.w1 = (fuse_rgb && cok) ? p.rgb_w[p.Cout + n0 + c] : 0.f;
        t.w2 = (fuse_rgb && cok) ? p.rgb_w[2 * p.Cout + n0 + c] : 0.f;
        return t;
    };
    auto tables_store = [&](int e, const TabVals& t) {
        const float oscale = (ET == SGDFR_SPLIT_FP16) ? SPLIT_F16_OUT : 1.f;
        const float xsc = (ET == SGDFR_SPLIT_FP16) ? SPLIT_F16_XSCALE : 1.f;
        const float rs = rsqrtf((float)p.Cout);
        const int m = e / NT, c = e - m * NT;
        dl[e] = t.dv * oscale;
        if (m == 0) bl[c] = t.bv;
        if (emit_xs) sn[e] = t.sv * xsc;
        if (fuse_rgb) *reinterpret_cast<float4*>(cw + 4 * e) = make_float4(t.w0 * (t.rv * rs), t.w1 * (t.rv * rs), t.w2 * (t.rv * rs), 0.f);
    };
    auto fill_tables = [&]() {
        for (int e = tid; e < p.simgs * NT; e += NTHR) tables_store(e, tables_load(e));
    };
    const bool tv_has = early && tid < p.simgs * NT;
    TabVals tv{};
    if (tv_has) tv = tables_load(tid);

    int boff[NI];
    int64_t ybase[NI];
    int64_t nzoff[NI];
    int dimg[NI];
    const int pitch = p.patch ? p.seglen : p.P;
    const int RP = p.R * p.P;
#pragma unroll
    for (int n = 0; n < NI; ++n) {
        const int l = (wn * NI + n) * 32 + l31;
        if (UPF) {
            const int lc = min(l, p.TR * p.TC - 1);
            const int r = fdiv(lc, p.fd_TC), c = lc - r * p.TC;
            boff[n] = r * p.seglen + c;
            ybase[n] = 0; nzoff[n] = 0; dimg[n] = img0;
        } else if (UP) {
            int64_t pix = (int64_t)pt * PT + l;
            const bool ok = pix < p.total_pix;
            if (!ok) pix = p.total_pix - 1;
            const int img = fdiv((int)pix, p.fd_rps);
            const int rem = (int)(pix - (int64_t)img * p.rps);
            boff[n] = l;
            ybase[n] = (ok && rem < RP) ? (int64_t)img * p.Cout * 4 * p.rps + rem : -1;
            nzoff[n] = 0;
            dimg[n] = img;
        } else if (DOWN) {
            int64_t pix = (int64_t)pt * PT + l;
            bool ok = pix < p.total_pix;
            if (!ok) pix = p.total_pix - 1;
            const int img = fdiv((int)pix, p.fd_RP);
            const int rem = (int)(pix - (int64_t)img * RP);
            const int a = fdiv(rem, p.fd_P), b = rem - a * p.P;
            ok = ok && a < p.H && b < p.W;
            boff[n] = l;
            ybase[n] = ok ? (int64_t)img * p.Cout * HW + a * p.W + b : -1;
            nzoff[n] = 0;
            dimg[n] = img;
        } else if (p.patch) {
            const int r = fdiv(l, p.fd_TC), c = l - r * p.TC;
            boff[n] = (r + 1) * p.seglen + c + 1;
            const int rem = (row0 + r) * p.W + col0 + c;
            const bool ok = img0 < p.B;
            ybase[n] = ok ? (int64_t)img0 * p.Cout * HW + rem : -1;
            nzoff[n] = (int64_t)img0 * p.noise_bstride + rem;
            dimg[n] = img0;
        } else {
            int64_t pix = (int64_t)pt * PT + l;
            const bool ok = pix < p.total_pix;
            if (!ok) pix = p.total_pix - 1;
            const int img = fdiv((int)pix, p.fd_HW);
            const int rem = (int)(pix - (int64_t)img * HW);
            const int a = fdiv(rem, p.fd_W), b = rem - a * p.W;
            boff[n] = (img * p.R + a + 1) * p.P + b + 1 - q0;
            ybase[n] = ok ? (int64_t)img * p.Cout * HW + rem : -1;
            nzoff[n] = (int64_t)img * p.noise_bstride + rem;
            dimg[n] = img;
        }
        boff[n] += hi * p.xs;
    }

    const float* xsrc[NEX];
    int64_t xs16[NEX];
    int soff[NEX];
    int ldst[NEX];
#pragma unroll
    for (int e = 0; e < NEX; ++e) {
        if (XIN) {
            xs16[e] = xin_addr(T, e);
            xsrc[e] = nullptr; soff[e] = -1; ldst[e] = 0;
            continue;
        }
        const int i = tid + e * NTHR;
        const int h = fdiv(i, p.fd_xs);
        const int j = i - h * p.xs;
        const bool in_range = (h < 2) && (j < p.xlen);
        bool ok;
        int img, pix;
        if (p.patch) {
            const int sg = fdiv(j, p.fd_seglen), cc = j - sg * p.seglen;
            const int row = row0 - 1 + sg, col = col0 - 1 + cc;
            img = img0;
            ok = in_range && row >= 0 && row < p.H && col >= 0 && col < p.W && img < p.B;
            pix = row * p.W + col;
        } else if (UP) {
            const int q = q0 + j;
            img = fdiv(q, p.fd_rps);
            const int r = q - img * p.rps;
            const int pr = fdiv(r, p.fd_P), pc = r - pr * p.P;
            ok = in_range && r < p.R * p.P && pc >= 1 && pr >= 1 && img < p.B;
            pix = (pr - 1) * p.W + (pc - 1);
        } else {
            const int q = q0 + j;
            const int qq = q < 0 ? 0 : q;
            const int pir = fdiv(qq, p.fd_P), pc = qq - pir * p.P;
            img = fdiv(pir, p.fd_R);
            const int pr = pir - img * p.R;
            ok = in_range && pc >= 1 && pr >= 1 && img < p.B && q >= 0;
            pix = (pr - 1) * p.W + (pc - 1);
        }
        xsrc[e] = ok ? p.x + (int64_t)img * p.x_bstride + (int64_t)(8 * h) * HW + pix : nullptr;
        soff[e] = !(h < 2 && j < p.xs) ? -1 : ok ? (img - img0) * p.Cin + 8 * h : 0;
        ldst[e] = (h * p.xs + j) * 16;
        xs16[e] = -2;
    }

    SPLIT_TRACE(2);
    f32x16 acc[PH][MI][NI];
#pragma unroll
    for (int ph = 0; ph < PH; ++ph)
#pragma unroll
        for (int m = 0; m < MI; ++m)
#pragma unroll
            for (int n = 0; n < NI; ++n)
// ... 589 lines not shown
                        *reinterpret_cast<uint4*>(dst + OHW * 16) = make_uint4(ll[0][rr][0], ll[1][rr][0], ll[0][rr][1], ll[1][rr][1]);
                    }
                }
            }
        }
        break;
    }
    if (!early) {
        __syncthreads();
        fill_tables();
        __syncthreads();
    }
    float* const yout = p.y + (int64_t)ks * p.split_stride;
    float rgb[NI][3];
#pragma unroll
    for (int n = 0; n < NI; ++n) rgb[n][0] = rgb[n][1] = rgb[n][2] = 0.f;
    const float e_slope = (whole && p.act) ? p.slope : 1.f, e_gain = (whole && p.act) ? p.gain : 1.f;
    auto epilogue = [&](auto has_y_t, auto emit_xs_t, auto fuse_rgb_t) {
        constexpr bool HAS_Y = decltype(has_y_t)::value, EMIT_XS = decltype(emit_xs_t)::value, FUSE_RGB = decltype(fuse_rgb_t)::value;
#pragma unroll
        for (int n = 0; n < NI; ++n) {
            if (ybase[n] < 0) continue;
            const int io = (dimg[n] - img0) * NT + wm * (MI * 32) + 4 * hi;
            if (UP) {
                const float4* const d4p = reinterpret_cast<const float4*>(dl + io);
                float* const yp = yout + ybase[n] + (int64_t)(n0 + wm * (MI * 32) + 4 * hi) * 4 * p.rps;
                if (p.plane_il) {
                    float* const yq = yp + 3 * (ybase[n] - (int64_t)dimg[n] * p.Cout * 4 * p.rps);
#pragma unroll
                    for (int m = 0; m < MI; ++m) {
                        if (n0 + wm * (MI * 32) + m * 32 >= p.Cout) continue;
#pragma unroll
                        for (int g = 0; g < 4; ++g) {
                            const float4 d4 = d4p[m * 8 + 2 * g];
                            const float dv[4] = {d4.x, d4.y, d4.z, d4.w};
#pragma unroll
                            for (int j = 0; j < 4; ++j)
                                *reinterpret_cast<float4*>(yq + (int64_t)(m * 32 + 8 * g + j) * 4 * p.rps) =
                                    make_float4(acc[0][m][n][4 * g + j] * dv[j], acc[PH > 2 ? 2 : 0][m][n][4 * g + j] * dv[j],
                                                acc[PH > 1 ? 1 : 0][m][n][4 * g + j] * dv[j], acc[PH > 3 ? 3 : 0][m][n][4 * g + j] * dv[j]);
                        }
                    }
                    continue;
                }
#pragma unroll
                for (int m = 0; m < MI; ++m) {
                    if (n0 + wm * (MI * 32) + m * 32 >= p.Cout) continue;
#pragma unroll
                    for (int g = 0; g < 4; ++g) {
                        const float4 d4 = d4p[m * 8 + 2 * g];
                        const float dv[4] = {d4.x, d4.y, d4.z, d4.w};
#pragma unroll
                        for (int j = 0; j < 4; ++j) {
                            float* dst = yp + (int64_t)(m * 32 + 8 * g + j) * 4 * p.rps;
#pragma unroll
                            for (int ph = 0; ph < PH; ++ph) dst[(int64_t)ph * p.rps] = acc[ph][m][n][4 * g + j] * dv[j];
                        }
                    }
                }
                continue;
            }
            const float4* const d4p = reinterpret_cast<const float4*>(dl + io);
            const float4* const b4p = reinterpret_cast<const float4*>(bl + wm * (MI * 32) + 4 * hi);
            const float4* const s4p = reinterpret_cast<const float4*>(sn + io);
            const float4* const cwp = reinterpret_cast<const float4*>(cw) + io;
            const int rem = (int)(ybase[n] - (int64_t)dimg[n] * p.Cout * HW);
            float* const yp = yout + ybase[n] + (int64_t)(n0 + wm * (MI * 32) + 4 * hi) * HW;
            unsigned char* const xp =
                p.xs_out + ((((int64_t)dimg[n] * (p.Cout / 8) + (n0 + wm * (MI * 32)) / 8) * 2) * HW + rem) * 16 + 8 * hi;
#pragma unroll
            for (int m = 0; m < MI; ++m) {
                if (n0 + wm * (MI * 32) + m * 32 >= p.Cout) continue;
                float4 d4[2], b4[2], s4[2], q[2][4];
                d4[0] = d4p[m * 8];
                b4[0] = b4p[m * 8];
                if (EMIT_XS) s4[0] = s4p[m * 8];
                if (FUSE_RGB) {
#pragma unroll
                    for (int j = 0; j < 4; ++j) q[0][j] = cwp[m * 32 + j];
                }
#pragma unroll
                for (int g = 0; g < 4; ++g) {
                    if (g + 1 < 4) {
                        d4[(g + 1) & 1] = d4p[m * 8 + 2 * (g + 1)];
                        b4[(g + 1) & 1] = b4p[m * 8 + 2 * (g + 1)];
                        if (EMIT_XS) s4[(g + 1) & 1] = s4p[m * 8 + 2 * (g + 1)];
                        if (FUSE_RGB) {
#pragma unroll
                            for (int j = 0; j < 4; ++j) q[(g + 1) & 1][j] = cwp[m * 32 + (g + 1) * 8 + j];
                        }
                    }
                    const float4 dq = d4[g & 1], bq = b4[g & 1], sq = s4[g & 1];
                    const float dv[4] = {dq.x, dq.y, dq.z, dq.w}, bv[4] = {bq.x, bq.y, bq.z, bq.w};
                    float v[4];
#pragma unroll
                    for (int j = 0; j < 4; ++j) v[j] = lrelu_gain(acc[0][m][n][4 * g + j] * dv[j] + nz[n] + bv[j], e_slope, e_gain);
                    if (HAS_Y) {
#pragma unroll
                        for (int j = 0; j < 4; ++j) yp[(int64_t)(m * 32 + 8 * g + j) * HW] = v[j];
                    }
                    if (EMIT_XS) {
                        unsigned h01, l01, h23, l23;
                        split_pair<ET>(v[0] * sq.x, v[1] * sq.y, h01, l01, sat);
                        split_pair<ET>(v[2] * sq.z, v[3] * sq.w, h23, l23, sat);
                        unsigned char* dst = xp + (int64_t)(m * 4 + g) * 2 * HW * 16;
                        *reinterpret_cast<uint2*>(dst) = make_uint2(h01, h23);
                        *reinterpret_cast<uint2*>(dst + (int64_t)HW * 16) = make_uint2(l01, l23);
                    }
                    if (FUSE_RGB) {
#pragma unroll
                        for (int j = 0; j < 4; ++j) {
                            rgb[n][0] = fmaf(v[j], q[g & 1][j].x, rgb[n][0]);
                            rgb[n][1] = fmaf(v[j], q[g & 1][j].y, rgb[n][1]);
                            rgb[n][2] = fmaf(v[j], q[g & 1][j].z, rgb[n][2]);
                        }
                    }
                }
            }
        }
    };
    {
        using yes = std::true_type;
        using no = std::false_type;
        if (UP || DOWN) {
            epilogue(yes{}, no{}, no{});
        } else {
            switch ((p.y ? 1 : 0) | (emit_xs ? 2 : 0) | (fuse_rgb ? 4 : 0)) {
                case 1: epilogue(yes{}, no{}, no{}); break;
                case 2: epilogue(no{}, yes{}, no{}); break;
                case 3: epilogue(yes{}, yes{}, no{}); break;
                case 4: epilogue(no{}, no{}, yes{}); break;
                case 5: epilogue(yes{}, no{}, yes{}); break;
                case 6: epilogue(no{}, yes{}, yes{}); break;
                case 7: epilogue(yes{}, yes{}, yes{}); break;
                default: break;
            }
        }
    }
    SPLIT_TRACE(5);
    if (fuse_rgb) {
#pragma unroll
        for (int n = 0; n < NI; ++n)
#pragma unroll
            for (int j = 0; j < 3; ++j) {
                rgb[n][j] += __shfl_xor(rgb[n][j], 32, 64);
                if (hi == 0) red[(wm * PT + (wn * NI + n) * 32 + l31) * 3 + j] = rgb[n][j];
            }
        __syncthreads();
        if (wm == 0 && hi == 0) {
#pragma unroll
            for (int n = 0; n < NI; ++n) {
                if (ybase[n] < 0) continue;
                const int rem = (int)(ybase[n] - (int64_t)dimg[n] * p.Cout * HW);
#pragma unroll
                for (int j = 0; j < 3; ++j) {
                    float t = 0.f;
#pragma unroll
                    for (int w2 = 0; w2 < WM; ++w2) t += red[(w2 * PT + (wn * NI + n) * 32 + l31) * 3 + j];
                    p.rgb_part[(((int64_t)dimg[n] * p.n_cout_tiles + ct) * 3 + j) * HW + rem] = t;
                }
            }
        }
    }
    SPLIT_TRACE(6);
    if (PERSIST) __syncthreads();
    SPLIT_TRACE(7);
    } while (PERSIST && (base += gridDim.x) < p.total_blocks);
    if (ET == SGDFR_SPLIT_FP16) split_flush_saturation(sat, p.sat);
#ifdef SGDFR_SPLIT_PROBE
    if (trace_on) g_split_trace[0] = (unsigned long long)ntrace;
#endif
}

}
```

### stylegan_directions_face_reenactment_amd/functional.py

```python
import functools
import math
import sys
import threading
import types

import torch
from torch.autograd import Function

from . import _native as N
from . import config as _config
from .config import Config, config, precision, set_default, set_precision, using
from . import timing
from .timing import timed_conv as _timed_conv, timed_hbm as _timed_hbm

SQRT2 = 2 ** 0.5

_CHAIN_NAMES = ('SplitAct', 'xin_ok', 'styled_conv_split', 'wsplit_chain_f', 'wsplit_chain_arith', 'xs_chain_arith', 'xs_plain_arith', 'wsplit_chain_ok', 'rgb_fusable', 'StreamPipeline')


class _Facade(types.ModuleType):

    def __getattr__(self, name):
        if name in _config.LEGACY:
            return getattr(config(), _config.LEGACY[name])
        if name == 'DEFAULT':
            return _config.DEFAULT
        if name in _CHAIN_NAMES:
            from . import chain
            return getattr(chain, name)
        raise AttributeError('module %r has no attribute %r' % (self.__name__, name))

    def __setattr__(self, name, value):
        if name in _config.LEGACY or name == 'DEFAULT':
            raise AttributeError('functional.%s is a read-only view of the ambient Config: use `with functional.using(functional.'
                                 'config().replace(%s=...))`, functional.set_default(...), or a Generator\'s `config`'
                                 % (name, _config.LEGACY.get(name, 'field')))
        super().__setattr__(name, value)


sys.modules[__name__].__class__ = _Facade


def pixel_norm(x, eps=1e-8):
    N.require_device(x)
    x2 = N.f32c(x).reshape(x.shape[0], -1) if x.ndim != 2 else N.f32c(x)
    y = torch.empty_like(x2)
    N.call('sgdfr_pixelnorm_f32', N.ptr(x2), N.ptr(y), x2.shape[0], x2.shape[1], float(eps), N.stream())
    return y.view(x.shape)


def linear(x, weight, bias=None, wscale=1.0, bscale=1.0, lrelu=False, slope=0.2, gain=SQRT2):
    N.require_device(x, weight, bias)
    K = weight.shape[1]
    if x.shape[-1] != K:
        raise RuntimeError('linear: input has %d features, weight expects %d' % (x.shape[-1], K))
    x2 = x.reshape(-1, K)
    if x2.stride(1) != 1 or (x2.shape[0] > 1 and x2.stride(0) < K):
        x2 = x2.contiguous()
    ldx = x2.stride(0) if x2.shape[0] > 1 else K
    w = N.f32c(weight)
    b = N.f32c(bias) if bias is not None else None
    M, Nn = x2.shape[0], w.shape[0]
    y = torch.empty(M, Nn, device=x.device, dtype=torch.float32)
    N.call('sgdfr_linear_f32', N.ptr(x2), ldx, N.ptr(w), N.ptr(b), N.ptr(y), Nn, M, Nn, K, float(wscale),
           float(bscale), N.ACT_LRELU if lrelu else N.ACT_NONE, float(slope), float(gain), N.stream())
    return y.view(*x.shape[:-1], Nn)


def latent_prepare(w, n_latent, shift=None, shift_layers=0, trunc=None, psi=1.0):
    N.require_device(w, shift, trunc)
    w = N.f32c(w)
    B, D = w.shape[0], w.shape[-1]
    w_plus = w.ndim == 3
    if w_plus and w.shape[1] != n_latent:
        raise RuntimeError('W+ code has %d rows, generator needs %d' % (w.shape[1], n_latent))
    shift_plus = 0
    if shift is not None:
        shift = N.f32c(shift)
        shift_plus = int(shift.ndim == 3)
        if shift_plus:
            shift_layers = shift.shape[1]
        if shift.shape[0] != B or shift.shape[-1] != D:
            raise RuntimeError('shift shape %s does not match latent %s' % (tuple(shift.shape), tuple(w.shape)))
    if trunc is not None:
        trunc = N.f32c(trunc).reshape(-1)
        if trunc.numel() != D:
            raise RuntimeError('truncation latent must have %d elements' % D)
    out = torch.empty(B, n_latent, D, device=w.device, dtype=torch.float32)
    N.call('sgdfr_latent_prepare_f32', N.ptr(w), int(w_plus), N.ptr(shift), shift_plus, int(shift_layers),
           N.ptr(trunc), float(psi), N.ptr(out), B, n_latent, D, N.stream())
    return out



def prepack(weight):
    N.require_device(weight)
    w = N.f32c(weight)
    _, cout, cin, k, _ = w.shape
    wp = torch.empty(cin, k * k, cout, device=w.device, dtype=torch.float32)
    q = torch.empty(cout, cin, device=w.device, dtype=torch.float32)
    qt = torch.empty(cin, cout, device=w.device, dtype=torch.float32)
    N.call('sgdfr_modconv_prepack_f32', N.ptr(w), N.ptr(wp), N.ptr(q), N.ptr(qt), cout, cin, k, N.stream())
    return wp, q, qt


def prepack_t(weight, flip):
    N.require_device(weight)
    w = N.f32c(weight)
    _, cout, cin, k, _ = w.shape
    wt = torch.empty(cout, k * k, cin, device=w.device, dtype=torch.float32)
    N.call('sgdfr_modconv_prepack_t_f32', N.ptr(w), N.ptr(wt), cout, cin, k, int(bool(flip)), N.stream())
    return wt


def style_demod(style, mod_weight, mod_bias, q=None, cout=0):
    N.require_device(style, mod_weight, mod_bias, q)
    B, D = style.shape
    if style.stride(1) != 1:
        style = style.contiguous()
    ld = style.stride(0) if B > 1 else D
    cin = mod_weight.shape[0]
    s = torch.empty(B, cin, device=style.device, dtype=torch.float32)
    d = torch.empty(B, cout, device=style.device, dtype=torch.float32) if q is not None else None
    N.call('sgdfr_style_demod_f32', N.ptr(style), ld, N.ptr(N.f32c(mod_weight)), N.ptr(N.f32c(mod_bias)),
           N.ptr(q), N.ptr(s), N.ptr(d), B, D, cin, cout, N.stream())
    return s, d


def styles_batched(latent, specs, plans=None):
    N.require_device(latent)
    latent = N.f32c(latent)
    B, L, D = latent.shape
    if len(specs) > N.MAX_STYLE_LAYERS:
        raise RuntimeError('too many modulated layers (%d)' % len(specs))
    planned = [plans is not None and plans[i] is not None and specs[i][3] is not None for i in range(len(specs))]
    n_s = sum(mw.shape[0] for _, mw, _, _, _ in specs)
    n_d = sum(cout for _, _, _, q, cout in specs if q is not None)
    n_sn = sum(specs[i][1].shape[0] for i in range(len(specs)) if planned[i])
    n_dn = sum(specs[i][4] for i in range(len(specs)) if planned[i])
    buf = torch.empty(B * (n_s + n_d + n_sn + n_dn) + 1, device=latent.device, dtype=torch.float32)
    offs = [0]

    def take(n, shape):
        v = buf[offs[0]:offs[0] + n].view(shape)
        offs[0] += n
        return v
    arr = (N.StyleLayer * len(specs))()
    out, keep = [], []
    for i, (li, mw, mb, q, cout) in enumerate(specs):
        N.require_device(mw, mb, q)
        cin = mw.shape[0]
        s = take(B * cin, (B, cin))
        d = take(B * cout, (B, cout)) if q is not None else None
        e = arr[i]
        e.mod_w, e.mod_b = N.f32c(mw).data_ptr(), N.f32c(mb).data_ptr()
        e.q = q.data_ptr() if q is not None else None
        e.s, e.d = s.data_ptr(), (d.data_ptr() if d is not None else None)
        e.cin, e.cout, e.latent_index = cin, cout, li
        e.s_n = e.d_n = e.x_absmax = None
        e.x_log2 = e.headroom = 0
        if planned[i]:
            bound, headroom = plans[i]
            s, d = take(B * cin, (B, cin)), take(B * cout, (B, cout))
            e.s_n, e.d_n, e.headroom = s.data_ptr(), d.data_ptr(), int(headroom)
            if isinstance(bound, torch.Tensor):
                keep.append(bound)
                e.x_absmax = bound.data_ptr()
            else:
                e.x_log2 = int(bound)
        out.append((s, d))
# ... 76 lines not shown


def current_sink():
    return getattr(_sink, 'word', None)


class saturation_sink:

    def __init__(self, word):
        if word is not None and (word.dtype != torch.int32 or not word.is_cuda or word.numel() != 1):
            raise RuntimeError('a saturation word is one int32 on the device (new_saturation_word)')
        self.word, self.prev = word, None

    def __enter__(self):
        self.prev = current_sink()
        _sink.word = self.word
        return self.word

    def __exit__(self, *exc):
        _sink.word = self.prev


def new_saturation_word(device):
    return torch.zeros(1, device=device, dtype=torch.int32)


def _sat():
    return N.ptr(getattr(_sink, 'word', None))


def split_saturation_count(reset=True):
    n = N.load().sgdfr_split_saturation_count(int(bool(reset)))
    if n < 0:
        raise RuntimeError('sgdfr_split_saturation_count failed')
    return int(n)


def mfma_ceiling(arith='fp16x3', lds_fragments=True, random_operands=True, iters=2000):
    import ctypes
    if not hasattr(N.load(), 'sgdfr_mfma_ceiling_probe'):
        raise RuntimeError('this build of libsgdfr_hip.so has no sgdfr_mfma_ceiling_probe (measurement-only symbol)')
    scratch = torch.empty(256 * 512, device='cuda', dtype=torch.float32)
    out = ctypes.c_double(0.0)
    N.call('sgdfr_mfma_ceiling_probe', N.SPLIT_FP16 if arith == 'fp16x3' else N.SPLIT_BF16, int(bool(lds_fragments)),
           int(bool(random_operands)), int(iters), 256, N.ptr(scratch), ctypes.byref(out), N.stream())
    return float(out.value)


class capture_graph:

    def __init__(self, g):
        self.ctx = torch.cuda.graph(g, capture_error_mode='thread_local')
        self.was = False

    def __enter__(self):
        import gc
        self.was = gc.isenabled()
        gc.collect()
        gc.disable()
        try:
            return self.ctx.__enter__()
        except BaseException:
            if self.was:
                gc.enable()
            raise

    def __exit__(self, *exc):
        import gc
        try:
            return self.ctx.__exit__(*exc)
        finally:
            if self.was:
                gc.enable()


def _zero_words(device):
    z = _zeros.get(device)
    if z is None:
        z = _zeros[device] = torch.zeros(64, device=device, dtype=torch.float32)
    return z


def prepack_wino(weight, adjoint=False):
    N.require_device(weight)
    w = N.f32c(weight)
    _, cout, cin, k, _ = w.shape
    u = torch.empty((cout if adjoint else cin), (cin if adjoint else cout), 16, device=w.device, dtype=torch.float32)
    N.call('sgdfr_modconv_prepack_wino_f32', N.ptr(w), N.ptr(u), cout, cin, int(bool(adjoint)), N.stream())
    return u


def wino_ok(B, cin, cout, H, W):
    if not config().use_winograd:
        return False
    if not N.load().sgdfr_modconv2d_wino_supported(B, cin, cout, H, W):
        return False
    return ((B * (H // 2) * (W // 2) + 63) // 64) * (cout // 64) >= config().winograd_min_blocks


def modconv_wino(x, u, s, d, cout, noise=None, noise_weight=None, bias=None, activate=False, slope=0.2, gain=SQRT2,
                 batch=None, desc=None):
    N.require_device(x, u, s, d, bias, noise_weight)
    x = N.f32c(x)
    B = s.shape[0] if batch is None else batch
    _, cin, H, W = x.shape
    xb = 0 if (x.shape[0] == 1 and B != 1) else cin * H * W
    nz, nzb = _noise_args(noise, B, H, W)
    y = torch.empty(B, cout, H, W, device=x.device, dtype=torch.float32)
    st = N.stream()
    _timed_conv(desc or ('wino3 %d->%d @%dx%d' % (cin, cout, H, W)), B * conv_flops(cin, cout, H, W), lambda: N.call(
        'sgdfr_modconv2d_wino_f32', N.ptr(x), xb, N.ptr(u), N.ptr(s), N.ptr(d), N.ptr(nz), nzb,
        N.ptr(noise_weight) if nz is not None else None, N.ptr(bias), N.ptr(_zero_words(x.device)), N.ptr(y), B, cin,
        cout, H, W, int(activate), float(slope), float(gain), st))
    return y


_SPLIT_ARITH = {'bf16x3': N.SPLIT_BF16, 'fp16x3': N.SPLIT_FP16}
_WSPLIT_ARITH = dict(_SPLIT_ARITH, fp16f8=N.SPLIT_FP16F8)


def _f8_tag(arith):
    return ' [f8 cross]' if (arith & 0xff) == N.SPLIT_FP16F8 else ''


def _plan_tag(B, cin, cout, H, W, mode, ks):
    if mode == N.MODE_UP3 and ks <= 1 and timing.active() is not None and _shape_query('sgdfr_modconv2d_split_f8_ok', B, cin, cout, H, W, mode):
        return '/deep'
    return ''


def prepack_split(weight, arith=None, adjoint=False):
    arith = _WSPLIT_ARITH[arith or config().precision]
    N.require_device(weight)
    w = N.f32c(weight)
    _, cout, cin, k, _ = w.shape
    n = N.load().sgdfr_modconv_prepack_split_elems(cout, cin)
    wsp = torch.empty(n, device=w.device, dtype=torch.int16)
    N.call('sgdfr_modconv_prepack_split_f32', N.ptr(w), N.ptr(wsp), cout, cin, arith, 2 if adjoint == 'down' else int(bool(adjoint)),
           _sat(), N.stream())
    return wsp


@functools.lru_cache(maxsize=None)
def _shape_query(name, *shape):
    return getattr(N.load(), name)(*shape)


def split_ok(B, cin, cout, H, W, mode=N.MODE_PLAIN3):
    return config().precision in _SPLIT_ARITH and bool(_shape_query('sgdfr_modconv2d_split_supported', B, cin, cout, H, W, mode))


def modconv_split(x, wsp, s, d, cout, noise=None, noise_weight=None, bias=None, activate=False, slope=0.2, gain=SQRT2,
                  batch=None, desc=None, mode=N.MODE_PLAIN3, arith=None, rgb=None, out=None, want_y=True, x_split=None, s_next=None,
                  plane_stride=0):
    arith = _WSPLIT_ARITH[arith or config().precision]
    N.require_device(s, d, bias, noise_weight)
    if not wsp.is_cuda or wsp.dtype != torch.int16:
        raise RuntimeError('modconv_split: wsp must be the int16 device buffer made by prepack_split')
    if x_split is not None:
        if not x.is_cuda or x.dtype != torch.int16:
            raise RuntimeError('modconv_split: a pre-split input is the int16 buffer made by to_split')
        B, cin, H, W = x_split
        xb = cin * H * W
        if mode == N.MODE_DOWN3:
            xb = cin * 4 * (H + 1) * (W + 1)
    else:
        N.require_device(x)
        x = N.f32c(x)
        B = s.shape[0] if batch is None else batch
        _, cin, H, W = x.shape
        xb = 0 if (x.shape[0] == 1 and B != 1) else cin * H * W
    if mode == N.MODE_DOWN3:
        if x_split is None:
            raise RuntimeError('modconv_split: DOWN3 reads the buffer made by planes_to_split (x_split=(B, C, H, W))')
        nz, nzb = None, 0
        y = torch.empty(B, cout, H, W, device=x.device, dtype=torch.float32)
    elif mode == N.MODE_UP3:
        nz, nzb = None, 0
        pshape = (B, cout, 4, H + 1, W + 1) if not plane_stride else (B, cout, 4, int(plane_stride))
        y = out if out is not None else torch.empty(pshape, device=x.device, dtype=torch.float32)
        if tuple(y.shape) != pshape or not y.is_contiguous():
            raise RuntimeError('modconv_split: out must be a contiguous %s tensor' % (pshape,))
    else:
        nz, nzb = _noise_args(noise, B, H, W)
        if not want_y and rgb is None and s_next is None:
            raise RuntimeError('modconv_split: want_y=False only makes sense with the fused ToRGB (rgb=...) or s_next')
        y = torch.empty(B, cout, H, W, device=x.device, dtype=torch.float32) if want_y else None
    st, sat = N.stream(), _sat()
    ks = _shape_query('sgdfr_modconv2d_split_ksplit_hint', B, cin, cout, H, W, mode) if config().use_splitk else 1
    if ks > 1 and y is None:
        raise RuntimeError('modconv_split: this launch is K-sliced and cannot fuse ToRGB (check rgb_fusable first)')
    partials = torch.empty((ks,) + tuple(y.shape), device=x.device, dtype=torch.float32) if ks > 1 else None
    rgb_w = rgb_s = part = xs_out = None
    if s_next is not None:
        if ks > 1 or mode != N.MODE_PLAIN3:
            raise RuntimeError('modconv_split: this launch cannot emit the split activation (K-sliced or not PLAIN3)')
        N.require_device(s_next)
        s_next = N.f32c(s_next)
        xs_out = torch.empty(B, cout // 8, 2, H * W, 8, device=s_next.device, dtype=torch.int16)
    if rgb is not None:
        if ks > 1 or mode != N.MODE_PLAIN3:
            raise RuntimeError('modconv_split: this launch cannot fuse ToRGB (check rgb_fusable first)')
        rgb_w, rgb_s = N.f32c(rgb[0]), N.f32c(rgb[1])
        N.require_device(rgb_w, rgb_s)
        tiles = _shape_query('sgdfr_modconv2d_split_cout_tiles_xin' if (x_split is not None and ks <= 1) else
                             'sgdfr_modconv2d_split_cout_tiles', B, cin, cout, H, W, mode)
        part = torch.empty(B, tiles * 3, H, W, device=x.device, dtype=torch.float32)
    _timed_conv((desc or ('split mode%d%s %d->%d @%dx%d%s' % (mode, _plan_tag(B, cin, cout, H, W, mode, ks), cin, cout, H, W,
                                                              ' K/%d' % ks if ks > 1 else ''))) + _f8_tag(arith),
                B * conv_flops(cin, cout, H, W), lambda: N.call(
        'sgdfr_modconv2d_split_f32', N.ptr(x), xb, N.ptr(wsp), N.ptr(s), N.ptr(d), N.ptr(nz), nzb,
        N.ptr(noise_weight) if nz is not None else None, N.ptr(bias), N.ptr(_zero_words(x.device)), N.ptr(y),
        N.ptr(partials), ks, N.ptr(rgb_w), N.ptr(rgb_s), N.ptr(part), int(x_split is not None), N.ptr(xs_out),
        N.ptr(s_next) if s_next is not None else None, B, cin, cout, H, W, mode, int(plane_stride), arith, int(activate),
        float(slope), float(gain), sat, st))
    if s_next is not None:
        return y, part, xs_out
    return y if rgb is None else (y, part)


def prepack_wsplit(weight, arith=None, f=2):
    arith = _WSPLIT_ARITH[arith or config().precision]
    N.require_device(weight)
    w = N.f32c(weight)
    _, cout, cin, k, _ = w.shape
    wsp = torch.empty(N.load().sgdfr_modconv_prepack_wsplit_elems(cout, cin, f), device=w.device, dtype=torch.int16)
    N.call('sgdfr_modconv_prepack_wsplit_f32', N.ptr(w), N.ptr(wsp), cout, cin, f, arith, _sat(), N.stream())
    return wsp


def wsplit_ok(B, cin, cout, H, W, f=2):
    return config().precision in _SPLIT_ARITH and bool(_shape_query('sgdfr_modconv2d_wsplit_supported', B, cin, cout, H, W, f))


WSPLIT_GROWTH_LOG2 = {2: 1, 4: 4}


def to_wsplit(x, s, arith=None, f=2):
    arith = _WSPLIT_ARITH[arith or config().precision]
    N.require_device(x, s)
    x, s = N.f32c(x), N.f32c(s)
    B, cin, H, W = x.shape
    vs = torch.empty(B, cin // 8, f + 2, 2, H * W // f, 8, device=x.device, dtype=torch.int16)
    N.call('sgdfr_to_wsplit_f32', N.ptr(x), N.ptr(s), N.ptr(vs), B, cin, H, W, f, arith, _sat(), N.stream())
    return vs


def modconv_wsplit(vs, shape, wsp, d, cout, noise=None, noise_weight=None, bias=None, activate=False, slope=0.2, gain=SQRT2,
                   arith=None, rgb=None, want_y=True, s_next=None, desc=None, f=2, xs_arith=None):
    arith = _WSPLIT_ARITH[arith or config().precision]
    if xs_arith not in (None, 'fp16f8'):
        raise ValueError("modconv_wsplit: xs_arith is None or 'fp16f8'")
    if xs_arith == 'fp16f8':
        arith |= N.SPLIT_HANDOVER_F8
    N.require_device(d, bias, noise_weight)
    if not vs.is_cuda or vs.dtype != torch.int16 or not wsp.is_cuda or wsp.dtype != torch.int16:
        raise RuntimeError('modconv_wsplit: vs / wsp are the int16 device buffers made by to_wsplit / prepack_wsplit')
    B, cin, H, W = shape
    nz, nzb = _noise_args(noise, B, H, W)
    if not want_y and rgb is None and s_next is None:
        raise RuntimeError('modconv_wsplit: want_y=False only makes sense with the fused ToRGB (rgb=...) or s_next')
    y = torch.empty(B, cout, H, W, device=vs.device, dtype=torch.float32) if want_y else None
    rgb_w = rgb_s = part = xs_out = None
    if s_next is not None:
        N.require_device(s_next)
        s_next = N.f32c(s_next)
        xs_out = torch.empty(B, cout // 8, 2, H * W, 8, device=vs.device, dtype=torch.int16)
    if rgb is not None:
        rgb_w, rgb_s = N.f32c(rgb[0]), N.f32c(rgb[1])
        N.require_device(rgb_w, rgb_s)
        part = torch.empty(B, (cout // 128) * 3, H, W, device=vs.device, dtype=torch.float32)
    _timed_conv((desc or ('wsplit F(%d,3) %d->%d @%dx%d' % (f, cin, cout, H, W))) + _f8_tag(arith), B * conv_flops(cin, cout, H, W), lambda: N.call(
        'sgdfr_modconv2d_wsplit_f32', N.ptr(vs), N.ptr(wsp), N.ptr(d), N.ptr(nz), nzb,
        N.ptr(noise_weight) if nz is not None else None, N.ptr(bias), N.ptr(_zero_words(vs.device)), N.ptr(y), N.ptr(rgb_w),
        N.ptr(rgb_s), N.ptr(part), N.ptr(xs_out), N.ptr(s_next) if s_next is not None else None, B, cin, cout, H, W, f, arith,
        int(activate), float(slope), float(gain), _sat(), N.stream()))
    if s_next is not None:
        return y, part, xs_out
    return y if rgb is None else (y, part)


def planes_to_split(gt, d, arith=None):
    arith = _SPLIT_ARITH[arith or config().precision]
    N.require_device(gt, d)
    gt = N.f32c(gt)
    B, C, _, R, P = gt.shape
    xs = torch.empty(B, 4 * C // 8, 2, R * P, 8, device=gt.device, dtype=torch.int16)
    N.call('sgdfr_planes_to_split_f32', N.ptr(gt), N.ptr(N.f32c(d)) if d is not None else None, N.ptr(xs), B, C, R - 1, P - 1, arith,
           _sat(), N.stream())
    return xs


def to_split(x, s, arith=None):
    arith = _WSPLIT_ARITH[arith or config().precision]
    N.require_device(x, s)
    x, s = N.f32c(x), N.f32c(s)
    B, cin, H, W = x.shape
    xs = torch.empty(B, cin // 8, 2, H * W, 8, device=x.device, dtype=torch.int16)
    N.call('sgdfr_to_split_f32', N.ptr(x), N.ptr(s), N.ptr(xs), B, cin, H, W, arith, _sat(), N.stream())
    return xs


class U8Target:
    __slots__ = ('frames', 'panel', 'swap_rb')

    def __init__(self, frames=None, panel=0, swap_rb=False):
        self.frames, self.panel, self.swap_rb = frames, int(panel), bool(swap_rb)


def torgb_finish(part, bias=None, skip=None, fir=None, u8=None):
    N.require_device(part, bias, skip, fir)
    B, c3, H, W = part.shape
    if skip is not None and tuple(skip.shape) != (B, 3, H // 2, W // 2):
        raise RuntimeError('skip shape %s does not match output [%d,3,%d,%d]/2' % (tuple(skip.shape), B, H, W))
    skip_bytes = 3 * (H // 2) * (W // 2) * 4 if skip is not None else 0
    if u8 is not None:
        frames = u8.frames
        if frames is None:
            frames = torch.empty(B, H, W, 3, device=part.device, dtype=torch.uint8)
        if frames.dtype != torch.uint8 or not frames.is_cuda or not frames.is_contiguous() or frames.ndim != 4 or \
                frames.shape[0] != B or frames.shape[1] != H or frames.shape[3] != 3 or frames.shape[2] < (u8.panel + 1) * W:
            raise RuntimeError('uint8 target %s cannot hold panel %d of [%d,%d,%d,3] frames' % (tuple(frames.shape), u8.panel, B, H, W))
        _timed_hbm('torgb_finish_u8 T=%d @%dx%d' % (c3 // 3, H, W), B * (c3 * H * W * 4 + skip_bytes + 3 * H * W), lambda: N.call(
            'sgdfr_torgb_finish_u8_f32', N.ptr(part), c3 // 3, N.ptr(N.f32c(bias)) if bias is not None else None,
            N.ptr(N.f32c(skip)) if skip is not None else None, N.ptr(N.f32c(fir)) if fir is not None else None, N.ptr(frames),
            frames.shape[2] * 3, u8.panel * W, int(u8.swap_rb), B, H, W, N.stream()))
        return frames
    y = torch.empty(B, 3, H, W, device=part.device, dtype=torch.float32)
    _timed_hbm('torgb_finish T=%d @%dx%d' % (c3 // 3, H, W), B * (c3 * H * W * 4 + skip_bytes + 3 * H * W * 4), lambda: N.call(
        'sgdfr_torgb_finish_f32', N.ptr(part), c3 // 3, N.ptr(N.f32c(bias)) if bias is not None else None,
        N.ptr(N.f32c(skip)) if skip is not None else None, N.ptr(N.f32c(fir)) if fir is not None else None, N.ptr(y), B, H, W,
        N.stream()))
    return y


def modconv_raw(x, wp, s, d, cout, mode, H, W, noise=None, noise_weight=None, bias=None, activate=False, slope=0.2,
                gain=SQRT2, batch=None, desc=None):
    N.require_device(x, wp, s, d, bias, noise_weight)
    x = N.f32c(x)
    B = s.shape[0] if batch is None else batch
    cin = x.shape[1]
    per_img = x[0].numel()
    xb = 0 if (x.shape[0] == 1 and B != 1) else per_img
    if x.shape[0] not in (1, B):
        raise RuntimeError('input batch %d does not match styles %d' % (x.shape[0], B))
    if mode == N.MODE_UP3:
        y = torch.empty(B, cout, 4, H + 1, W + 1, device=x.device, dtype=torch.float32)
    else:
        y = torch.empty(B, cout, H, W, device=x.device, dtype=torch.float32)
    nz, nzb = _noise_args(noise, B, H, W) if mode == N.MODE_PLAIN3 else (None, 0)
    st = N.stream()
    splits = N.load().sgdfr_modconv2d_splitk_hint(B, cin, cout, H, W, mode) if config().use_splitk else 1
    if splits > 1:
        partials = torch.empty((splits,) + tuple(y.shape), device=x.device, dtype=torch.float32)
        _timed_conv((desc or 'conv') + ' splitK%d' % splits, B * conv_flops(cin, cout, H, W), lambda: N.call(
            'sgdfr_modconv2d_splitk_f32', N.ptr(x), xb, N.ptr(wp), N.ptr(s), N.ptr(d), N.ptr(nz), nzb,
            N.ptr(noise_weight) if nz is not None else None, N.ptr(bias), N.ptr(y), N.ptr(partials), splits, B, cin, cout,
            H, W, mode, int(activate), float(slope), float(gain), st))
        return y
    _timed_conv(desc or ('mode%d %d->%d @%dx%d' % (mode, cin, cout, H, W)), B * conv_flops(cin, cout, H, W), lambda: N.call(
        'sgdfr_modconv2d_fwd_f32', N.ptr(x), xb, N.ptr(wp), N.ptr(s), N.ptr(d), N.ptr(nz), nzb,
        N.ptr(noise_weight) if nz is not None else None, N.ptr(bias), N.ptr(y), B, cin, cout, H, W, mode,
        int(activate), float(slope), float(gain), st))
    return y


def blur_bias_act(planes, fir, H, W, noise=None, noise_weight=None, bias=None, activate=False, slope=0.2, gain=SQRT2, out=None,
                  absmax_out=None):
    N.require_device(planes, fir, bias, noise_weight)
    B, C = planes.shape[0], planes.shape[1]
    nz, nzb = _noise_args(noise, B, 2 * H, 2 * W)
    y = out if out is not None else torch.empty(B, C, 2 * H, 2 * W, device=planes.device, dtype=torch.float32)
    if tuple(y.shape) != (B, C, 2 * H, 2 * W) or not y.is_contiguous():
        raise RuntimeError('blur_bias_act: out must be a contiguous [B,C,2H,2W] tensor')
    if absmax_out is not None and (absmax_out.dtype != torch.int32 or not absmax_out.is_cuda or absmax_out.numel() != B * C or
                                   not absmax_out.is_contiguous()):
        raise RuntimeError('blur_bias_act: absmax_out must be a contiguous int32 device tensor with B*C words')
    _timed_hbm('blur %d ch %dx%d -> %dx%d fp32' % (C, H, W, 2 * H, 2 * W), B * C * (16 * (H + 1) * (W + 1) + 16 * H * W), lambda: N.call(
        'sgdfr_blur_bias_act_f32', N.ptr(planes), N.ptr(N.f32c(fir)), N.ptr(nz), nzb,
        N.ptr(noise_weight) if nz is not None else None, N.ptr(bias), N.ptr(y), B, C, H, W, int(activate),
        float(slope), float(gain), N.ptr(absmax_out), N.stream()))
    return y


def blur_bias_act_split(planes, fir, H, W, s_next, noise=None, noise_weight=None, bias=None, activate=False, slope=0.2,
                        gain=SQRT2, arith=None, plane_stride=0, wino=False):
    wino = 2 if wino is True else int(wino or 0)
    arith = (_WSPLIT_ARITH if wino != 2 else _SPLIT_ARITH)[arith or config().precision]
    N.require_device(planes, fir, bias, noise_weight, s_next)
    B, C = planes.shape[0], planes.shape[1]
    nz, nzb = _noise_args(noise, B, 2 * H, 2 * W)
    if wino:
        xs = torch.empty(B, C // 8, wino + 2, 2, 4 * H * W // wino, 8, device=planes.device, dtype=torch.int16)
    else:
        xs = torch.empty(B, C // 8, 2, 4 * H * W, 8, device=planes.device, dtype=torch.int16)
    out_b = 4 * H * W * (4 * (wino + 2) // wino if wino else 4)
    _timed_hbm('blur %d ch %dx%d -> %dx%d %s' % (C, H, W, 2 * H, 2 * W, 'WS F(%d,3)' % wino if wino else 'XS'),
               B * C * (16 * (H + 1) * (W + 1) + out_b), lambda: N.call(
        'sgdfr_blur_bias_act_split_f32', N.ptr(planes), N.ptr(N.f32c(fir)), N.ptr(nz), nzb,
        N.ptr(noise_weight) if nz is not None else None, N.ptr(bias), N.ptr(N.f32c(s_next)), N.ptr(xs), B, C, H, W,
        int(plane_stride), arith, wino, int(activate), float(slope), float(gain), _sat(), N.stream()))
    return xs


def modconv3x3(x, wp, s, d, cout, upsample=False, fir=None, noise=None, noise_weight=None, bias=None,
               activate=False, slope=0.2, gain=SQRT2, batch=None, return_planes=False, wino=None, split=None, rgb=None,
               want_y=True, ranged=False, x_absmax=None, absmax_out=None):
    _, cin, H, W = x.shape
    if not upsample:
        B = s.shape[0] if batch is None else batch
        if split is not None and split_ok(B, cin, cout, H, W):
            if config().range_plan and not ranged and config().precision == 'fp16x3' and d is not None:
                s, d = _exact_range(x, s, d, batch, x_absmax)
            return modconv_split(x, split() if callable(split) else split, s, d, cout, noise, noise_weight, bias,
                                 activate, slope, gain, batch, rgb=rgb, want_y=want_y)
        if rgb is not None:
            raise RuntimeError('modconv3x3: ToRGB fusion needs the split kernel (check rgb_fusable first)')
        if wino is not None and wino_ok(B, cin, cout, H, W):
            return modconv_wino(x, wino() if callable(wino) else wino, s, d, cout, noise, noise_weight, bias, activate,
                                slope, gain, batch)
        return modconv_raw(x, wp, s, d, cout, N.MODE_PLAIN3, H, W, noise, noise_weight, bias, activate, slope, gain,
                           batch, 'plain3 %d->%d @%dx%d' % (cin, cout, H, W))
    if fir is None:
        raise RuntimeError('upsample modconv needs the blur FIR taps')
    Bu = s.shape[0] if batch is None else batch
    use_split = split is not None and split_ok(Bu, cin, cout, H, W, N.MODE_UP3)
    if use_split:
        if config().range_plan and not ranged and config().precision == 'fp16x3' and d is not None:
            s, d = _exact_range(x, s, d, batch, x_absmax)
        planes = modconv_split(x, split() if callable(split) else split, s, d, cout, batch=batch, mode=N.MODE_UP3)
    else:
        planes = modconv_raw(x, wp, s, d, cout, N.MODE_UP3, H, W, batch=batch, desc='up3 %d->%d @%dx%d' % (cin, cout, H, W))
    y = blur_bias_act(planes, fir, H, W, noise, noise_weight, bias, activate, slope, gain, absmax_out=absmax_out)
    return (y, planes) if return_planes else y


def torgb(x, w_rgb, s, bias=None, skip=None, fir=None):
    N.require_device(x, w_rgb, s, bias, skip, fir)
    x = N.f32c(x)
    B, cin, H, W = x.shape
    if skip is not None and tuple(skip.shape) != (B, 3, H // 2, W // 2):
        raise RuntimeError('skip shape %s does not match output [%d,3,%d,%d]/2' % (tuple(skip.shape), B, H, W))
    y = torch.empty(B, 3, H, W, device=x.device, dtype=torch.float32)
    _timed_hbm('torgb %d ch @%dx%d' % (cin, H, W), B * ((cin + 3) * H * W * 4 + (3 * (H // 2) * (W // 2) * 4 if skip is not None else 0)),
               lambda: N.call(
        'sgdfr_torgb_fwd_f32', N.ptr(x), N.ptr(N.f32c(w_rgb)), N.ptr(s), N.ptr(N.f32c(bias)) if bias is not None else None,
        N.ptr(N.f32c(skip)) if skip is not None else None, N.ptr(N.f32c(fir)) if fir is not None else None,
        N.ptr(y), B, cin, H, W, N.stream()))
    return y


def conv_flops(cin, cout, h, w, upsample=False):
    return 2.0 * 9 * cin * cout * h * w



class _Affine(Function):

    @staticmethod
    def forward(ctx, x, weight, bias):
        ctx.save_for_backward(x, weight)
        ctx.has_bias = bias is not None
        return linear(x, weight, bias)

    @staticmethod
    def backward(ctx, g):
        x, weight = ctx.saved_tensors
        g2 = g.reshape(-1, weight.shape[0])
        x2 = x.reshape(-1, weight.shape[1])
        gx = gw = gb = None
        if ctx.needs_input_grad[0]:
            gx = linear(g2, weight.t().contiguous()).view_as(x)
        if ctx.needs_input_grad[1]:
            gw = linear(g2.t().contiguous(), x2.t().contiguous())
        if ctx.has_bias and ctx.needs_input_grad[2]:
# ... 217 lines not shown
```

### stylegan_directions_face_reenactment_amd/model.py

```python
import math
import os
import random
import struct
import warnings

import torch
from torch import nn

from . import autograd as AG
from . import functional as F_
from .graph_runner import GraphReplayMixin
from .planner import PlannerMixin
from .range_plan import RangePlanMixin, RangeToken
from .op import FusedLeakyReLU, fused_leaky_relu, upfirdn2d


def make_kernel(k):
    k = torch.as_tensor(k, dtype=torch.float32)
    if k.ndim == 1:
        k = torch.outer(k, k)
    return k / k.sum()


_SIDE_STREAMS = {}
# ... 115 lines not shown
        super()._load_from_state_dict(*args, **kwargs)
        self.invalidate_packs()

    def packed(self):
        key = self._key()
        if self._pack is None or self._pack[0] != key:
            with torch.no_grad():
                self._pack = (key,) + F_.prepack(self.weight.detach())
            self._pack_t = None
        return self._pack[1], self._pack[2], self._pack[3]

    def packed_t(self):
        key = self._key()
        if getattr(self, '_pack_t', None) is None or self._pack_t[0] != key:
            with torch.no_grad():
                self._pack_t = (key, F_.prepack_t(self.weight.detach(), flip=not self.upsample))
        return self._pack_t[1]

    def packed_wino(self, adjoint=False):
        key = self._key()
        cache = getattr(self, '_pack_w', None)
        if cache is None or cache[0] != key:
            cache = self._pack_w = [key, None, None]
        if cache[1 + int(adjoint)] is None:
            with torch.no_grad():
                cache[1 + int(adjoint)] = F_.prepack_wino(self.weight.detach(), adjoint=adjoint)
        return cache[1 + int(adjoint)]

    def packed_split(self, adjoint=False, arith=None):
        arith = arith or F_.config().precision
        key = self._key()
        cache = getattr(self, '_pack_s', None)
        if cache is None or cache[0] != key:
            cache = self._pack_s = [key, {}]
        slot = (arith, adjoint if adjoint == 'down' else bool(adjoint))
        if slot not in cache[1]:
            with torch.no_grad():
                cache[1][slot] = F_.prepack_split(self.weight.detach(), arith=arith, adjoint=adjoint)
        return cache[1][slot]

    def packed_wsplit(self, arith=None, f=2):
        arith = arith or F_.config().precision
        key = self._key()
        cache = getattr(self, '_pack_s', None)
        if cache is None or cache[0] != key:
            cache = self._pack_s = [key, {}]
        slot = (arith, 'wino', f)
        if slot not in cache[1]:
            with torch.no_grad():
                cache[1][slot] = F_.prepack_wsplit(self.weight.detach(), arith=arith, f=f)
        return cache[1][slot]

    def style_spec(self, latent_index):
        q = self.packed()[1] if (self.kernel_size == 3 and self.demodulate) else None
        return (latent_index, self.modulation.weight, self.modulation.bias, q, self.out_channel)

    def styles(self, style):
        mod = self.modulation
        q = qt = None
        if self.kernel_size == 3 and self.demodulate:
            _, q, qt = self.packed()
        if _needs_grad(style, mod.weight, mod.bias):
            out = AG.StyleFn.apply(style, mod.weight, mod.bias, q, qt, self.out_channel)
            return out if q is not None else (out, None)
        return F_.style_demod(style, mod.weight, mod.bias, q, self.out_channel)

    def fused(self, input, style, noise=None, noise_weight=None, bias=None, activate=False, batch=None, sd=None, rgb=None,
              want_y=True, ranged=False):
        if self.kernel_size != 3:
            raise NotImplementedError('only the 3x3 modulated conv has a fused StyledConv form (1x1 lives in ToRGB)')
        s, d = self.styles(style) if sd is None else sd
        if _needs_grad(input, s, d, self.weight, noise_weight, bias):
            return AG.StyledConvFn.apply(input, s, d, self.weight, noise_weight, bias, noise, self, activate, batch)
        return F_.modconv3x3(input, self.packed()[0], s, d, self.out_channel, upsample=self.upsample,
                             fir=self.blur.kernel if self.upsample else None, noise=noise,
                             noise_weight=noise_weight, bias=bias, activate=activate, batch=batch,
                             wino=None if self.upsample else self.packed_wino,
                             split=self.packed_split, rgb=rgb, want_y=want_y, ranged=ranged)

    def forward(self, input, style):
        if self.kernel_size == 1:
            if self.demodulate or self.out_channel != 3:
                raise NotImplementedError('1x1 modulated conv is only built as ToRGB (3 outputs, no demodulation)')
            s, _ = self.styles(style)
            if _needs_grad(input, s, self.weight):
                return AG.ToRGBFn.apply(input, s, self.weight, None, None, None)
            return F_.torgb(input, self.weight.view(3, self.in_channel), s)
        return self.fused(input, style)


class NoiseInjection(nn.Module):

    def __init__(self):
        super().__init__()
        self.weight = nn.Parameter(torch.zeros(1))

    def forward(self, image, noise=None):
        if noise is None:
            batch, _, height, width = image.shape
            noise = image.new_empty(batch, 1, height, width).normal_()
        return image + self.weight * noise


class ConstantInput(nn.Module):
    def __init__(self, channel, size=4):
        super().__init__()
        self.input = nn.Parameter(torch.randn(1, channel, size, size))

    def forward(self, input):
        return self.input.repeat(input.shape[0], 1, 1, 1)


class StyledConv(nn.Module):

    def __init__(self, in_channel, out_channel, kernel_size, style_dim, upsample=False, blur_kernel=[1, 3, 3, 1],
                 demodulate=True):
        super().__init__()
        self.conv = ModulatedConv2d(in_channel, out_channel, kernel_size, style_dim, upsample=upsample,
                                    blur_kernel=blur_kernel, demodulate=demodulate)
        self.noise = NoiseInjection()
        self.activate = FusedLeakyReLU(out_channel)

    def forward(self, input, style, noise=None, batch=None, sd=None, rgb=None, want_y=True, ranged=False):
        if noise is None:
            B = style.shape[0] if sd is None else sd[0].shape[0]
            r = input.shape[-1] * (2 if self.conv.upsample else 1)
            noise = torch.empty(B, 1, r, r, device=input.device, dtype=torch.float32).normal_()
        return self.conv.fused(input, style, noise=noise, noise_weight=self.noise.weight, bias=self.activate.bias,
                               activate=True, batch=batch, sd=sd, rgb=rgb, want_y=want_y, ranged=ranged)


class ToRGB(nn.Module):

    def __init__(self, in_channel, style_dim, upsample=True, blur_kernel=[1, 3, 3, 1]):
        super().__init__()
        if upsample:
            self.upsample = Upsample(blur_kernel)
        self.conv = ModulatedConv2d(in_channel, 3, 1, style_dim, demodulate=False)
        self.bias = nn.Parameter(torch.zeros(1, 3, 1, 1))

    def forward(self, input, style, skip=None, sd=None):
        conv = self.conv
        s = sd[0] if sd is not None else conv.styles(style)[0]
        fir = None
        if skip is not None:
            up = getattr(self, 'upsample', None)
            if up is None or tuple(up.kernel.shape) != (4, 4) or up.pad != (2, 1):
                raise NotImplementedError('ToRGB skip path is built for the 4-tap 2x Upsample')
            fir = up.kernel
        if _needs_grad(input, s, skip, conv.weight, self.bias):
            return AG.ToRGBFn.apply(input, s, conv.weight, self.bias, skip, fir)
        return F_.torgb(input, conv.weight.view(3, conv.in_channel), s, bias=self.bias.view(3), skip=skip, fir=fir)

    def finish(self, part, skip=None, u8=None):
        fir = None
        if skip is not None:
            up = getattr(self, 'upsample', None)
            if up is None or tuple(up.kernel.shape) != (4, 4) or up.pad != (2, 1):
                raise NotImplementedError('ToRGB skip path is built for the 4-tap 2x Upsample')
            fir = up.kernel
        return F_.torgb_finish(part, bias=self.bias.view(3), skip=skip, fir=fir, u8=u8)


class Generator(RangePlanMixin, GraphReplayMixin, PlannerMixin, nn.Module):
    def __init__(self, size, style_dim, n_mlp, channel_multiplier=2, blur_kernel=[1, 3, 3, 1], lr_mlp=0.01):
        super().__init__()
        self.size = size
        self.style_dim = style_dim
        self.channel_multiplier = channel_multiplier
        self.style = nn.Sequential(
            PixelNorm(), *[EqualLinear(style_dim, style_dim, lr_mul=lr_mlp, activation='fused_lrelu')
                           for _ in range(n_mlp)])
        self.channels = {
            4: 512, 8: 512, 16: 512, 32: 512,
            64: 256 * channel_multiplier, 128: 128 * channel_multiplier, 256: 64 * channel_multiplier,
            512: 32 * channel_multiplier, 1024: 16 * channel_multiplier,
        }
        self.input = ConstantInput(self.channels[4])
        self.conv1 = StyledConv(self.channels[4], self.channels[4], 3, style_dim, blur_kernel=blur_kernel)
        self.to_rgb1 = ToRGB(self.channels[4], style_dim, upsample=False)
        self.log_size = int(math.log(size, 2))
        self.num_layers = (self.log_size - 2) * 2 + 1
        self.convs = nn.ModuleList()
        self.upsamples = nn.ModuleList()
        self.to_rgbs = nn.ModuleList()
        self.noises = nn.Module()
        for layer_idx in range(self.num_layers):
            res = (layer_idx + 5) // 2
            self.noises.register_buffer('noise_{}'.format(layer_idx), torch.randn(1, 1, 2 ** res, 2 ** res))
        in_channel = self.channels[4]
        for i in range(3, self.log_size + 1):
            out_channel = self.channels[2 ** i]
            self.convs.append(StyledConv(in_channel, out_channel, 3, style_dim, upsample=True,
                                         blur_kernel=blur_kernel))
            self.convs.append(StyledConv(out_channel, out_channel, 3, style_dim, blur_kernel=blur_kernel))
            self.to_rgbs.append(ToRGB(out_channel, style_dim))
            in_channel = out_channel
        self.n_latent = self.log_size * 2 - 2
        self.overlap_rgb = True
        self.config = None

    def invalidate_packs(self):
        for m in self.modules():
            if isinstance(m, ModulatedConv2d):
                m.invalidate_packs()
        self._chain_plans = {}
        self.__dict__.pop('_wino_cache', None)
        self._range_state = None
        self._plist = None
        self._stamp_list = None
        self._drop_graphs()

    def _apply(self, fn, *args, **kwargs):
        out = super()._apply(fn, *args, **kwargs)
        self._chain_plans, self._range_state, self._plist, self._stamp_list = {}, None, None, None
        self._drop_graphs()
        return out

    def _load_from_state_dict(self, *args, **kwargs):
        super()._load_from_state_dict(*args, **kwargs)
        self._chain_plans, self._range_state, self._plist, self._stamp_list = {}, None, None, None
        self._drop_graphs()

    def make_noise(self):
        device = self.input.input.device
        noises = [torch.randn(1, 1, 4, 4, device=device)]
        for i in range(3, self.log_size + 1):
            for _ in range(2):
                noises.append(torch.randn(1, 1, 2 ** i, 2 ** i, device=device))
        return noises

    def mean_latent(self, n_latent):
        latent_in = torch.randn(n_latent, self.style_dim, device=self.input.input.device)
        return self.style(latent_in).mean(0, keepdim=True)

    def get_latent(self, input):
        return self.style(input)


    def _params(self):
        plist = getattr(self, '_plist', None)
        if plist is None:
            plist = self._plist = list(self.parameters())
        return plist

    def _weights_stamp(self):
        tl = getattr(self, '_stamp_list', None)
        if tl is None:
            tl = self._stamp_list = self._params() + list(self.noises.buffers())
        w = tl[0]
        v = 0
        for p in tl:
            v += p._version
        return (w.data_ptr(), w.device, v)

    def __deepcopy__(self, memo):
        import copy
        cls = self.__class__
        new = cls.__new__(cls)
        memo[id(self)] = new
        skip = ('_sat', '_sat_seen', '_sat_tokens', '_graphs', '_graph_calls', '_last_token', '_plist', '_stamp_list', '_all_mods')
        for k, v in self.__dict__.items():
            if k not in skip:
                new.__dict__[k] = copy.deepcopy(v, memo)
        return new

    def __getstate__(self):
        st = dict(self.__dict__)
        for k in ('_sat', '_sat_seen', '_sat_tokens', '_graphs', '_graph_calls', '_last_token', '_plist', '_stamp_list', '_all_mods'):
            st.pop(k, None)
        return st

    verify_range_default = os.environ.get('SGDFR_VERIFY_RANGE', '1') != '0'
    fused_backward = os.environ.get('SGDFR_FUSED_BACKWARD', '1') != '0'

    def forward(self, styles, return_latents=False, return_features=False, inject_index=None, truncation=1,
                truncation_latent=None, input_is_latent=False, noise=None, randomize_noise=False, image_out=None,
                verify_range=None, graph=None):
        cfg = getattr(self, 'config', None)
        if cfg is not None and cfg is not F_.config():
            with F_.using(cfg):
                return self.forward(styles, return_latents, return_features, inject_index, truncation, truncation_latent,
                                    input_is_latent, noise, randomize_noise, image_out, verify_range, graph)
        verify_explicit = verify_range is not None
        if verify_range is None:
            verify_range = bool(self.verify_range_default)
        key = self._graph_key(styles, return_latents, inject_index, truncation, truncation_latent, input_is_latent, noise,
                              randomize_noise, image_out, verify_range, graph, verify_explicit)
        if key is None:
            return self._forward_impl(styles, return_latents, return_features, inject_index, truncation, truncation_latent,
                                      input_is_latent, noise, randomize_noise, image_out, verify_range)
        return self._replay_or_run(key, styles, return_latents, return_features, inject_index, truncation, truncation_latent,
                                   input_is_latent, image_out, verify_range)

    def _forward_impl(self, styles, return_latents=False, return_features=False, inject_index=None, truncation=1,
                      truncation_latent=None, input_is_latent=False, noise=None, randomize_noise=False, image_out=None,
                      verify_range=False, depth=0):
        styles_in = styles
        if not input_is_latent:
            styles = [self.style(s) for s in styles]
        if noise is None:
            noise = [None] * self.num_layers if randomize_noise else \
                [getattr(self.noises, 'noise_{}'.format(i)) for i in range(self.num_layers)]
            if randomize_noise and verify_range and not torch.is_grad_enabled():
                nb = styles[0].shape[0]
                noise = [torch.randn(nb, 1, 2 ** (2 + (i + 1) // 2), 2 ** (2 + (i + 1) // 2), device=styles[0].device)
                         for i in range(self.num_layers)]
        trunc = truncation_latent if truncation < 1 else None
        if truncation < 1 and truncation_latent is None:
            raise RuntimeError('truncation < 1 needs truncation_latent')
        grad = _needs_grad(*styles, trunc, *self._params())

        def prepare(w, rows):
            if _needs_grad(w, trunc):
                return AG.LatentPrepareFn.apply(w, None, trunc, rows, 0, truncation)
            return F_.latent_prepare(w, rows, trunc=trunc, psi=truncation)

        if len(styles) < 2:
            latent = prepare(styles[0], self.n_latent)
        else:
            if inject_index is None:
                inject_index = random.randint(1, self.n_latent - 1)
            latent = torch.cat([prepare(styles[0], inject_index), prepare(styles[1], self.n_latent - inject_index)], 1)

        order = [(self.conv1.conv, 0), (self.to_rgb1.conv, 1)]
        i = 1
        for conv1, conv2, to_rgb in zip(self.convs[::2], self.convs[1::2], self.to_rgbs):
            order += [(conv1.conv, i), (conv2.conv, i + 1), (to_rgb.conv, i + 2)]
            i += 2
        layers = [self.conv1] + list(self.convs)
        to_rgbs = [self.to_rgb1] + list(self.to_rgbs)
        self.__dict__['_last_token'] = None
        with F_.saturation_sink(self._sat_word()):
            if grad:
                frozen = not any(p.requires_grad for p in self._params())
                hooked = any(m._forward_hooks or m._forward_pre_hooks or m._backward_hooks for m in layers + to_rgbs)
                if self.fused_backward and not hooked and not return_features and image_out is None:
                    image = AG.SynthesisFn.apply(latent, self, order, layers, to_rgbs, noise, *AG.synthesis_params(self, layers, to_rgbs))
                    return (image, latent) if return_latents else (image, None)
                if frozen:
                    flat = iter(AG.StylesBatchedFn.apply(latent, order))
                    sd = [(next(flat), next(flat) if (m.kernel_size == 3 and m.demodulate) else None) for m, _ in order]
                else:
                    sd = [m.styles(latent[:, li]) for m, li in order]
                return self._synthesis(latent, sd, layers, to_rgbs, noise, True, False, return_latents, image_out)
            specs = [m.style_spec(li) for m, li in order]
            plans, arith = None, None
            if F_.config().precision == 'fp16x3' and F_.config().range_plan is True:
                plans, arith = self._range_plans(latent, noise, specs, order, layers)
            if arith is not None and arith != F_.config().precision:
                with F_.precision(arith):
                    return self._synthesis(latent, F_.styles_batched(latent, specs), layers, to_rgbs, noise, False, False,
                                           return_latents, image_out)
            out = self._synthesis(latent, F_.styles_batched(latent, specs, plans), layers, to_rgbs, noise, False,
                                  plans is not None, return_latents, image_out)
            if plans is None:
                return out
            self._settle_oldest_if_full()
            tok = self._snapshot()
            if not verify_range or tok is None:
                self.__dict__['_last_token'] = tok
                return out
            if self.range_ok(tok):
                return out
            self.__dict__['_rerendered'] = self.__dict__.get('_rerendered', 0) + 1
            if depth <= self.AUTO_RECALIBRATIONS and (getattr(self, '_range_state', None) or {}).get('recal'):
                return self._forward_impl(styles_in, return_latents, return_features, inject_index, truncation, truncation_latent,
                                          input_is_latent, noise, False, image_out, True, depth + 1)
            with F_.precision('bf16x3'):
                return self._synthesis(latent, F_.styles_batched(latent, specs), layers, to_rgbs, noise, False, False,
                                       return_latents, image_out)

    def _synthesis(self, latent, sd, layers, to_rgbs, noise, grad, ranged, return_latents, image_out=None):
        batch = latent.shape[0]
        sd_of_layer = [0] + [2 + 3 * (i // 2) + (i % 2) for i in range(len(self.convs))]
        sd_of_rgb = [1] + [4 + 3 * k for k in range(len(self.to_rgbs))]
        hooked = any(m._forward_hooks or m._forward_pre_hooks for m in layers + to_rgbs)
        chain = (not grad) and (not hooked) and F_.config().precision in ('fp16x3', 'bf16x3') and \
            not (F_.config().precision == 'fp16x3' and F_.config().range_plan == 'exact')

        side = _side_stream(latent.device) if (self.overlap_rgb and not grad) else None
        main = torch.cuda.current_stream() if side is not None else None
        on_side = [False]

        if image_out is not None and grad:
            raise RuntimeError('image_out (uint8 frames) is an inference output: call the generator under torch.no_grad()')
        wrote_u8 = [False]

        def rgb(layer, x, part_in, skip_in, sdl, last=False):
            if part_in is not None:
                if on_side[0]:
                    main.wait_stream(side)
                    skip_in.record_stream(main)
                    on_side[0] = False
                if last and image_out is not None:
                    wrote_u8[0] = True
                    return layer.finish(part_in, skip_in, u8=image_out)
                return layer.finish(part_in, skip_in)
            run = lambda: layer(x, None, skip_in, sd=sdl)
            if side is None:
                return run()
            on_side[0] = True
            side.wait_stream(main)
            x.record_stream(side)
            if skip_in is not None:
                skip_in.record_stream(side)
            with torch.cuda.stream(side):
                return run()

        plan = self._chain_plan(batch, chain, noise, layers)

        x, skip = self.input.input, None
        for li, layer in enumerate(layers):
            c = layer.conv
            up = c.upsample
            sdl = sd[sd_of_layer[li]]
            nz = noise[li]
            first = li == 0
            use_chain, fuse, to_next, want_y, wino_next, arith_next, xs_arith = plan[li]
            k = li // 2
            if not use_chain:
                if isinstance(x, F_.SplitAct):
                    raise RuntimeError('internal: a split activation reached a layer that cannot take it')
                out, part = layer(x, None, noise=nz, batch=batch if first else None, sd=sdl, ranged=ranged), None
            else:
                rgb_arg = (to_rgbs[k].conv.weight.view(3, c.out_channel), sd[sd_of_rgb[k]][0]) if fuse else None
                wino_in = x.wino if isinstance(x, F_.SplitAct) else 0
                out, part = F_.styled_conv_split(
                    x, c.packed_wsplit(arith=x.arith, f=wino_in) if wino_in else c.packed_split(arith=getattr(x, 'arith', None)),
                    sdl[0], sdl[1], c.out_channel, upsample=up,
                    fir=c.blur.kernel if up else None, noise=nz, noise_weight=layer.noise.weight, bias=layer.activate.bias,
                    batch=batch if first else None, s_next=sd[sd_of_layer[li + 1]][0] if to_next else None, rgb=rgb_arg,
                    want_y=want_y, wino_next=wino_next, arith_next=arith_next, xs_arith=xs_arith)
            if not up:
                skip = rgb(to_rgbs[k], out, part, skip, sd[sd_of_rgb[k]], last=li == len(layers) - 1)
            x = out
        if side is not None and on_side[0]:
            main.wait_stream(side)
            skip.record_stream(main)
        image = skip
        if image_out is not None and not wrote_u8[0]:
            from .reenact import images_to_uint8, grid_frames_uint8
            if image_out.frames is None and not image_out.swap_rb:
                image = images_to_uint8(image)
            else:
                B, _, H, W = image.shape
                frames = image_out.frames if image_out.frames is not None else torch.empty(B, H, W, 3, device=image.device, dtype=torch.uint8)
                K = frames.shape[2] // W
                grid_frames_uint8([image if k == image_out.panel else None for k in range(K)], swap_rb=image_out.swap_rb, out=frames)
                image = frames
        return (image, latent) if return_latents else (image, None)
```

Baseline: 11410.

## Fold ToRGB finish (bias, skip upsample, uint8 store) into split modconv epilogue

Adds a finish path to the split modulated-conv kernel: when the plan uses one 64-wide cout tile, the fused ToRGB partial is combined in the epilogue with the ToRGB bias and the FIR-upsampled skip, then written directly as fp32 RGB or uint8 frames. This removes the separate torgb_finish launch and the round trip of RGB partials through memory for eligible plain layers. It is on by default and can be disabled with SGDFR_FOLD_FINISH=0. In exchange it adds more registers and epilogue work to the conv kernel, plus scattered skip reads per pixel.

```diff
diff --git a/include/sgdfr.h b/include/sgdfr.h
--- a/include/sgdfr.h
+++ b/include/sgdfr.h
@@ -154,6 +154,15 @@
                               unsigned char* y, int64_t row_pitch, int x_offset, int swap_rb, int B, int H, int W,
                               void* stream);
 
+int sgdfr_modconv2d_split_fin_ok(int B, int Cin, int Cout, int H, int W, int xin_whole);
+int sgdfr_modconv2d_split_fin_f32(const float* x, int64_t x_bstride, const unsigned short* wsp, const float* s, const float* d,
+                                  const float* noise, int64_t noise_bstride, const float* noise_w, const float* bias,
+                                  const float* zeros, float* y, const float* rgb_w, const float* rgb_s, int x_is_split,
+                                  unsigned short* xs_out, const float* s_next, int B, int Cin, int Cout, int H, int W, int arith,
+                                  int act, float slope, float gain, const float* fin_bias, const float* fin_skip, const float* fir,
+                                  float* fin_y, unsigned char* fin_y8, int64_t row_pitch, int x_offset, int swap_rb,
+                                  unsigned int* sat, void* stream);
+
 int sgdfr_image_to_u8_f32(const float* x, unsigned char* y, int B, int H, int W, void* stream);
 
 #define SGDFR_MAX_GRID_PANELS 4
diff --git a/stylegan_directions_face_reenactment_amd/_native.py b/stylegan_directions_face_reenactment_amd/_native.py
--- a/stylegan_directions_face_reenactment_amd/_native.py
+++ b/stylegan_directions_face_reenactment_amd/_native.py
@@ -48,6 +48,10 @@
     'sgdfr_modconv2d_split_f32': [_c_f32p, _i64, ctypes.c_void_p, _c_f32p, _c_f32p, _c_f32p, _i64, _c_f32p, _c_f32p, _c_f32p,
                                   _c_f32p, _c_f32p, _i, _c_f32p, _c_f32p, _c_f32p, _i, ctypes.c_void_p, _c_f32p, _i, _i, _i, _i,
                                   _i, _i, _i64, _i, _i, _f, _f, ctypes.c_void_p, ctypes.c_void_p],
+    'sgdfr_modconv2d_split_fin_ok': [_i, _i, _i, _i, _i, _i],
+    'sgdfr_modconv2d_split_fin_f32': [_c_f32p, _i64, ctypes.c_void_p, _c_f32p, _c_f32p, _c_f32p, _i64, _c_f32p, _c_f32p, _c_f32p, _c_f32p,
+                                      _c_f32p, _c_f32p, _i, ctypes.c_void_p, _c_f32p, _i, _i, _i, _i, _i, _i, _i, _f, _f, _c_f32p,
+                                      _c_f32p, _c_f32p, _c_f32p, ctypes.c_void_p, _i64, _i, _i, ctypes.c_void_p, ctypes.c_void_p],
     'sgdfr_to_split_f32': [_c_f32p, _c_f32p, ctypes.c_void_p, _i, _i, _i, _i, _i, ctypes.c_void_p, ctypes.c_void_p],
     'sgdfr_planes_to_split_f32': [_c_f32p, _c_f32p, ctypes.c_void_p, _i, _i, _i, _i, _i, ctypes.c_void_p, ctypes.c_void_p],
     'sgdfr_blur_adjoint_split_f32': [_c_f32p, _c_f32p, _c_f32p, _c_f32p, ctypes.c_void_p, _c_f32p, _i, _i, _i, _i, _i, ctypes.c_void_p,
diff --git a/stylegan_directions_face_reenactment_amd/chain.py b/stylegan_directions_face_reenactment_amd/chain.py
--- a/stylegan_directions_face_reenactment_amd/chain.py
+++ b/stylegan_directions_face_reenactment_amd/chain.py
@@ -2,7 +2,7 @@
 
 from . import _native as N
 from .config import config
-from .functional import (_shape_query, blur_bias_act, blur_bias_act_split, modconv_split, modconv_wsplit, split_ok, wsplit_ok)
+from .functional import (_shape_query, blur_bias_act, blur_bias_act_split, fin_foldable, modconv_split, modconv_wsplit, split_ok, wsplit_ok)
 
 
 class SplitAct:
@@ -19,7 +19,9 @@
 
 
 def styled_conv_split(x, wsp, s, d, cout, upsample=False, fir=None, noise=None, noise_weight=None, bias=None, batch=None,
-                      s_next=None, rgb=None, want_y=True, wino_next=False, arith_next=None, xs_arith=None):
+                      s_next=None, rgb=None, want_y=True, wino_next=False, arith_next=None, xs_arith=None, fin=None):
+    if fin is not None and (upsample or rgb is None or (isinstance(x, SplitAct) and x.wino)):
+        raise RuntimeError('styled_conv_split: the ToRGB finish folds into the direct plain conv with a fused ToRGB only')
     if isinstance(x, SplitAct) and x.wino:
         if upsample:
             raise RuntimeError('styled_conv_split: the Winograd input form feeds plain convs only')
@@ -43,7 +45,7 @@
         H, W = x.shape[2], x.shape[3]
     if not upsample:
         res = modconv_split(xin, wsp, s_arg, d, cout, noise, noise_weight, bias, True, batch=batch, rgb=rgb,
-                            want_y=want_y and s_next is None, x_split=x_split, s_next=s_next, arith=x_arith)
+                            want_y=want_y and s_next is None, x_split=x_split, s_next=s_next, arith=x_arith, fin=fin)
         if s_next is not None:
             _, part, xs = res
             return SplitAct(xs, (B, cout, H, W)), part
@@ -117,6 +119,12 @@
         (not config().use_splitk or _shape_query('sgdfr_modconv2d_split_ksplit_hint', B, cin, cout, H, W, N.MODE_PLAIN3) == 1)
 
 
+def fin_chain_ok(x, B, cin, cout, H, W):
+    if isinstance(x, SplitAct) and x.wino:
+        return False
+    return fin_foldable(B, cin, cout, H, W, isinstance(x, SplitAct))
+
+
 class StreamPipeline:
 
     def __init__(self, n=2, device=None):
diff --git a/stylegan_directions_face_reenactment_amd/csrc/split.hip b/stylegan_directions_face_reenactment_amd/csrc/split.hip
--- a/stylegan_directions_face_reenactment_amd/csrc/split.hip
+++ b/stylegan_directions_face_reenactment_amd/csrc/split.hip
@@ -321,6 +321,12 @@
     return split_plan(B, Cin, Cout, H, W, mode, &p, true) ? p.n_cout_tiles : 0;
 }
 
+extern "C" int sgdfr_modconv2d_split_fin_ok(int B, int Cin, int Cout, int H, int W, int xin_whole) {
+    SplitParams p;
+    const SplitPlan* plan = split_plan(B, Cin, Cout, H, W, SGDFR_MODE_PLAIN3, &p, xin_whole != 0);
+    return plan && plan->nt == 64 && p.n_cout_tiles == 1 && H % 2 == 0 && W % 2 == 0 ? 1 : 0;
+}
+
 extern "C" int sgdfr_modconv2d_split_plan_info(int B, int Cin, int Cout, int H, int W, int mode, int xin_whole) {
     SplitParams p;
     const SplitPlan* plan = split_plan(B, Cin, Cout, H, W, mode, &p, xin_whole != 0);
@@ -450,13 +456,21 @@
     }
 }
 
-extern "C" int sgdfr_modconv2d_split_f32(const float* x, int64_t x_bstride, const unsigned short* wsp, const float* s,
-                                         const float* d, const float* noise, int64_t noise_bstride, const float* noise_w,
-                                         const float* bias, const float* zeros, float* y, float* partials, int ksplit,
-                                         const float* rgb_w, const float* rgb_s, float* rgb_part, int x_is_split,
-                                         unsigned short* xs_out, const float* s_next, int B, int Cin, int Cout, int H, int W,
-                                         int mode, int64_t plane_stride, int arith, int act, float slope, float gain,
-                                         unsigned int* sat, void* stream) {
+struct SplitFin {
+    const float *bias, *skip, *fir;
+    float* y;
+    unsigned char* y8;
+    int64_t pitch;
+    int x_off, swap_rb;
+};
+
+static int modconv2d_split_impl(const float* x, int64_t x_bstride, const unsigned short* wsp, const float* s,
+                                const float* d, const float* noise, int64_t noise_bstride, const float* noise_w,
+                                const float* bias, const float* zeros, float* y, float* partials, int ksplit,
+                                const float* rgb_w, const float* rgb_s, float* rgb_part, int x_is_split,
+                                unsigned short* xs_out, const float* s_next, int B, int Cin, int Cout, int H, int W,
+                                int mode, int64_t plane_stride, int arith, int act, float slope, float gain,
+                                unsigned int* sat, void* stream, const SplitFin* fin) {
     SGDFR_REQUIRE(arith == SGDFR_SPLIT_BF16 || arith == SGDFR_SPLIT_FP16 ||
                       (arith == SGDFR_SPLIT_FP16F8 && sgdfr_modconv2d_split_f8_ok(B, Cin, Cout, H, W, mode) && x_is_split && ksplit <= 1),
                   "modconv_split: arith must be SGDFR_SPLIT_BF16/FP16 (FP16F8: only where sgdfr_modconv2d_split_f8_ok() says so, with a "
@@ -471,7 +485,7 @@
                   "(noise / bias / activation belong to sgdfr_blur_bias_act_f32), DOWN3 a raw gradient");
     SGDFR_REQUIRE(mode != SGDFR_MODE_DOWN3 || (x_is_split && y && !rgb_part && !xs_out), "modconv_split: DOWN3 takes "
                   "pre-split planes and writes y only");
-    SGDFR_REQUIRE(x && wsp && zeros && (y || rgb_part || xs_out) && (s || x_is_split), "modconv_split: null pointer");
+    SGDFR_REQUIRE(x && wsp && zeros && (y || rgb_part || xs_out || fin) && (s || x_is_split), "modconv_split: null pointer");
     SGDFR_REQUIRE(!xs_out || (s_next && mode == SGDFR_MODE_PLAIN3 && ksplit <= 1 && Cout % 8 == 0 &&
                               (reinterpret_cast<uintptr_t>(xs_out) & 15) == 0),
                   "modconv_split: xs_out needs s_next, mode PLAIN3, ksplit == 1 and a 16-byte aligned buffer");
@@ -498,9 +512,20 @@
     p.noise_w = noise_w; p.bias = bias; p.zeros = zeros; p.y = y;
     p.act = act; p.slope = slope; p.gain = gain; p.sat = sat;
     if (ksplit < 1) ksplit = 1;
-    SGDFR_REQUIRE(!rgb_part || (rgb_w && rgb_s && mode == SGDFR_MODE_PLAIN3 && ksplit == 1),
+    SGDFR_REQUIRE(!(rgb_part || fin) || (rgb_w && rgb_s && mode == SGDFR_MODE_PLAIN3 && ksplit == 1),
                   "modconv_split: the fused ToRGB needs rgb_w, rgb_s, mode PLAIN3 and ksplit == 1");
     p.rgb_w = rgb_w; p.rgb_s = rgb_s; p.rgb_part = rgb_part;
+    if (fin) {
+        SGDFR_REQUIRE(!rgb_part && p.n_cout_tiles == 1 && plan->nt == 64, "modconv_split_fin: the finish folds into launches with ONE "
+                      "cout tile of 64 (this plan: %d of %d; ask sgdfr_modconv2d_split_fin_ok) and replaces rgb_part", p.n_cout_tiles, plan->nt);
+        SGDFR_REQUIRE((fin->y != nullptr) != (fin->y8 != nullptr), "modconv_split_fin: exactly one of the fp32 and the uint8 target");
+        SGDFR_REQUIRE(!fin->skip || (fin->fir && H % 2 == 0 && W % 2 == 0), "modconv_split_fin: skip needs fir taps and even H, W");
+        SGDFR_REQUIRE(!fin->y8 || (fin->x_off >= 0 && fin->pitch >= (int64_t)(fin->x_off + W) * 3),
+                      "modconv_split_fin: panel at pixel %d of %d does not fit rows of %lld bytes", fin->x_off, W, (long long)fin->pitch);
+        p.fin = fin->y8 ? 2 : 1;
+        p.fin_bias = fin->bias; p.fin_skip = fin->skip; p.fin_fir = fin->fir; p.fin_y = fin->y; p.fin_y8 = fin->y8;
+        p.fin_pitch = fin->pitch; p.fin_xoff = fin->x_off; p.fin_swap = fin->swap_rb;
+    }
     p.xs_out = reinterpret_cast<unsigned char*>(xs_out); p.s_next = s_next;
     SGDFR_REQUIRE(ksplit == 1 || (partials && ksplit <= Cin / SPLIT_CB), "modconv_split: ksplit %d needs a partials buffer "
                   "and at most %d slices", ksplit, Cin / SPLIT_CB);
@@ -533,3 +558,28 @@
     return launch_splitk_reduce(partials, ksplit, n_out, plain ? noise : nullptr, noise_bstride, noise_w, plain ? bias : nullptr, y,
                                 Cout, plain ? H * W : 1, plain ? act : 0, slope, gain, st);
 }
+
+extern "C" int sgdfr_modconv2d_split_f32(const float* x, int64_t x_bstride, const unsigned short* wsp, const float* s,
+                                         const float* d, const float* noise, int64_t noise_bstride, const float* noise_w,
+                                         const float* bias, const float* zeros, float* y, float* partials, int ksplit,
+                                         const float* rgb_w, const float* rgb_s, float* rgb_part, int x_is_split,
+                                         unsigned short* xs_out, const float* s_next, int B, int Cin, int Cout, int H, int W,
+                                         int mode, int64_t plane_stride, int arith, int act, float slope, float gain,
+                                         unsigned int* sat, void* stream) {
+    return modconv2d_split_impl(x, x_bstride, wsp, s, d, noise, noise_bstride, noise_w, bias, zeros, y, partials, ksplit, rgb_w, rgb_s,
+                                rgb_part, x_is_split, xs_out, s_next, B, Cin, Cout, H, W, mode, plane_stride, arith, act, slope, gain,
+                                sat, stream, nullptr);
+}
+
+extern "C" int sgdfr_modconv2d_split_fin_f32(const float* x, int64_t x_bstride, const unsigned short* wsp, const float* s,
+                                             const float* d, const float* noise, int64_t noise_bstride, const float* noise_w,
+                                             const float* bias, const float* zeros, float* y, const float* rgb_w, const float* rgb_s,
+                                             int x_is_split, unsigned short* xs_out, const float* s_next, int B, int Cin, int Cout,
+                                             int H, int W, int arith, int act, float slope, float gain, const float* fin_bias,
+                                             const float* fin_skip, const float* fir, float* fin_y, unsigned char* fin_y8,
+                                             int64_t row_pitch, int x_offset, int swap_rb, unsigned int* sat, void* stream) {
+    const SplitFin fin = {fin_bias, fin_skip, fir, fin_y, fin_y8, row_pitch, x_offset, swap_rb};
+    return modconv2d_split_impl(x, x_bstride, wsp, s, d, noise, noise_bstride, noise_w, bias, zeros, y, nullptr, 1, rgb_w, rgb_s, nullptr,
+                                x_is_split, xs_out, s_next, B, Cin, Cout, H, W, SGDFR_MODE_PLAIN3, 0, arith, act, slope, gain, sat,
+                                stream, &fin);
+}
diff --git a/stylegan_directions_face_reenactment_amd/csrc/split_kernel.h b/stylegan_directions_face_reenactment_amd/csrc/split_kernel.h
--- a/stylegan_directions_face_reenactment_amd/csrc/split_kernel.h
+++ b/stylegan_directions_face_reenactment_amd/csrc/split_kernel.h
@@ -83,6 +83,14 @@
     const float* f8_max;
     FastDiv fd_xs, fd_seglen, fd_P, fd_R, fd_RP, fd_rps, fd_HW, fd_W, fd_TC, fd_tiles_x, fd_per_img, fd_npt, fd_tps, fd_Cin;
     int lid0;
+    int fin;
+    int fin_xoff, fin_swap;
+    int64_t fin_pitch;
+    const float* fin_bias;
+    const float* fin_skip;
+    const float* fin_fir;
+    float* fin_y;
+    unsigned char* fin_y8;
 };
 
 static void fill_fastdivs(SplitParams& p) {
@@ -93,6 +101,61 @@
 }
 
 constexpr int SPLIT_CB = 16;
+
+__device__ __forceinline__ void split_fin_store(const SplitParams& p, int img, int rem, const float (&t3)[3]) {
+    const int oy = fdiv(rem, p.fd_W), ox = rem - oy * p.W;
+    const int HW = p.H * p.W, Hs = p.H >> 1, Ws = p.W >> 1;
+    int sidx[2][2];
+    float kf[2][2];
+    bool tok[2][2];
+    if (p.fin_skip) {
+#pragma unroll
+        for (int a = 0; a < 2; ++a) {
+            const int ky = (oy & 1) + 2 * a, m = (oy + ky - 2) >> 1;
+            const bool rok = oy + ky - 2 >= 0 && m < Hs;
+#pragma unroll
+            for (int c = 0; c < 2; ++c) {
+                const int kx = (ox & 1) + 2 * c, nn = (ox + kx - 2) >> 1;
+                tok[a][c] = rok && ox + kx - 2 >= 0 && nn < Ws;
+                sidx[a][c] = tok[a][c] ? m * Ws + nn : 0;
+                kf[a][c] = p.fin_fir[15 - (ky * 4 + kx)];
+            }
+        }
+    }
+    float px[3];
+#pragma unroll
+    for (int j = 0; j < 3; ++j) {
+        float acc = p.fin_bias ? p.fin_bias[j] : 0.f;
+        acc += t3[j];
+        if (p.fin_skip) {
+            const float* sp = p.fin_skip + ((int64_t)img * 3 + j) * Hs * Ws;
+            float sv[2][2];
+#pragma unroll
+            for (int a = 0; a < 2; ++a)
+#pragma unroll
+                for (int c = 0; c < 2; ++c) sv[a][c] = sp[sidx[a][c]];
+            float o = 0.f;
+#pragma unroll
+            for (int a = 0; a < 2; ++a)
+#pragma unroll
+                for (int c = 0; c < 2; ++c) o = tok[a][c] ? fmaf(sv[a][c], kf[a][c], o) : o;
+            acc += o;
+        }
+        px[j] = acc;
+    }
+    if (p.fin == 1) {
+#pragma unroll
+        for (int j = 0; j < 3; ++j) p.fin_y[((int64_t)img * 3 + j) * HW + rem] = px[j];
+    } else {
+        unsigned char* dst = p.fin_y8 + ((int64_t)img * p.H + oy) * p.fin_pitch + (int64_t)(p.fin_xoff + ox) * 3;
+#pragma unroll
+        for (int c = 0; c < 3; ++c) {
+            float f = fminf(fmaxf(px[p.fin_swap ? 2 - c : c], -1.f), 1.f);
+            f = (f + 1.f) / (2.f + 1e-5f) * 255.f;
+            dst[c] = (unsigned char)f;
+        }
+    }
+}
 
 template <int N>
 __device__ __forceinline__ void split_wait_vmcnt() {
@@ -154,6 +217,7 @@
     constexpr bool UP = (MODE == SGDFR_MODE_UP3) || UPF, DOWN = (MODE == SGDFR_MODE_DOWN3);
     static_assert(!UPF || (XIN && NSS == 1 && MI == 1 && NI == 2 && NW == 8), "the fused blur epilogue is written for the 64 x 256 deep plan");
     constexpr int PH = UP ? 4 : 1;
+    constexpr bool FIN = MODE == SGDFR_MODE_PLAIN3 && WM == 1;
     static_assert(!DOWN || (XIN && NSS == 1), "DOWN3 stages pre-split planes, one (channel block, phase) pair per stage");
     static_assert(NW == 8 || NW == 4, "4 or 8 waves per block");
     static_assert(NT % 64 == 0 && (NSS == 1 || NSS == 3), "cout tiles are packed 64 wide");
@@ -283,7 +347,7 @@
     const int n0 = ct * NT;
 
     const bool whole = p.ksplit == 1;
-    const bool fuse_rgb = !UP && !DOWN && whole && p.rgb_part != nullptr;
+    const bool fuse_rgb = !UP && !DOWN && whole && (p.rgb_part != nullptr || (FIN && p.fin != 0));
     const bool early = p.simgs <= 2;
     constexpr bool SLIM = XIN && NW == 4;
     float* const dl = early ? ls + ((DOWN || SLIM) ? 0 : ((p.simgs * p.Cin + 3) & ~3)) : reinterpret_cast<float*>(smem);
@@ -1179,12 +1243,19 @@
             for (int n = 0; n < NI; ++n) {
                 if (ybase[n] < 0) continue;
                 const int rem = (int)(ybase[n] - (int64_t)dimg[n] * p.Cout * HW);
+                float t3[3];
 #pragma unroll
                 for (int j = 0; j < 3; ++j) {
                     float t = 0.f;
 #pragma unroll
                     for (int w2 = 0; w2 < WM; ++w2) t += red[(w2 * PT + (wn * NI + n) * 32 + l31) * 3 + j];
-                    p.rgb_part[(((int64_t)dimg[n] * p.n_cout_tiles + ct) * 3 + j) * HW + rem] = t;
+                    t3[j] = t;
+                }
+                if (!FIN || p.fin == 0) {
+#pragma unroll
+                    for (int j = 0; j < 3; ++j) p.rgb_part[(((int64_t)dimg[n] * p.n_cout_tiles + ct) * 3 + j) * HW + rem] = t3[j];
+                } else {
+                    split_fin_store(p, dimg[n], rem, t3);
                 }
             }
         }
diff --git a/stylegan_directions_face_reenactment_amd/functional.py b/stylegan_directions_face_reenactment_amd/functional.py
--- a/stylegan_directions_face_reenactment_amd/functional.py
+++ b/stylegan_directions_face_reenactment_amd/functional.py
@@ -1,5 +1,6 @@
 import functools
 import math
+import os
 import sys
 import threading
 import types
@@ -15,7 +16,7 @@
 
 SQRT2 = 2 ** 0.5
 
-_CHAIN_NAMES = ('SplitAct', 'xin_ok', 'styled_conv_split', 'wsplit_chain_f', 'wsplit_chain_arith', 'xs_chain_arith', 'xs_plain_arith', 'wsplit_chain_ok', 'rgb_fusable', 'StreamPipeline')
+_CHAIN_NAMES = ('SplitAct', 'xin_ok', 'styled_conv_split', 'wsplit_chain_f', 'wsplit_chain_arith', 'xs_chain_arith', 'xs_plain_arith', 'wsplit_chain_ok', 'rgb_fusable', 'fin_chain_ok', 'StreamPipeline')
 
 
 class _Facade(types.ModuleType):
@@ -398,7 +399,7 @@
 
 def modconv_split(x, wsp, s, d, cout, noise=None, noise_weight=None, bias=None, activate=False, slope=0.2, gain=SQRT2,
                   batch=None, desc=None, mode=N.MODE_PLAIN3, arith=None, rgb=None, out=None, want_y=True, x_split=None, s_next=None,
-                  plane_stride=0):
+                  plane_stride=0, fin=None):
     arith = _WSPLIT_ARITH[arith or config().precision]
     N.require_device(s, d, bias, noise_weight)
     if not wsp.is_cuda or wsp.dtype != torch.int16:
@@ -451,9 +452,32 @@
         N.require_device(rgb_w, rgb_s)
         tiles = _shape_query('sgdfr_modconv2d_split_cout_tiles_xin' if (x_split is not None and ks <= 1) else
                              'sgdfr_modconv2d_split_cout_tiles', B, cin, cout, H, W, mode)
-        part = torch.empty(B, tiles * 3, H, W, device=x.device, dtype=torch.float32)
-    _timed_conv((desc or ('split mode%d%s %d->%d @%dx%d%s' % (mode, _plan_tag(B, cin, cout, H, W, mode, ks), cin, cout, H, W,
-                                                              ' K/%d' % ks if ks > 1 else ''))) + _f8_tag(arith),
+        if fin is None:
+            part = torch.empty(B, tiles * 3, H, W, device=x.device, dtype=torch.float32)
+        elif not _shape_query('sgdfr_modconv2d_split_fin_ok', B, cin, cout, H, W, int(x_split is not None and ks <= 1)):
+            raise RuntimeError('modconv_split: the ToRGB finish folds into launches of one cout tile of 64 (check fin_foldable first)')
+    elif fin is not None:
+        raise RuntimeError('modconv_split: fin=... finishes the fused ToRGB (rgb=...)')
+    desc = (desc or ('split mode%d%s %d->%d @%dx%d%s' % (mode, _plan_tag(B, cin, cout, H, W, mode, ks), cin, cout, H, W,
+                                                         ' K/%d' % ks if ks > 1 else ''))) + _f8_tag(arith)
+    if fin is not None:
+        N.require_device(fin.bias, fin.skip, fin.fir)
+        if fin.skip is not None and (tuple(fin.skip.shape) != (B, 3, H // 2, W // 2) or fin.fir is None):
+            raise RuntimeError('skip shape %s does not match output [%d,3,%d,%d]/2 (and needs fir)' % (tuple(fin.skip.shape), B, H, W))
+        frames = _u8_frames(fin.u8, B, H, W, x.device) if fin.u8 is not None else None
+        img = torch.empty(B, 3, H, W, device=x.device, dtype=torch.float32) if frames is None else None
+        _timed_conv(desc, B * conv_flops(cin, cout, H, W), lambda: N.call(
+            'sgdfr_modconv2d_split_fin_f32', N.ptr(x), xb, N.ptr(wsp), N.ptr(s), N.ptr(d), N.ptr(nz), nzb,
+            N.ptr(noise_weight) if nz is not None else None, N.ptr(bias), N.ptr(_zero_words(x.device)), N.ptr(y),
+            N.ptr(rgb_w), N.ptr(rgb_s), int(x_split is not None), N.ptr(xs_out), N.ptr(s_next) if s_next is not None else None,
+            B, cin, cout, H, W, arith, int(activate), float(slope), float(gain),
+            N.ptr(N.f32c(fin.bias)) if fin.bias is not None else None, N.ptr(N.f32c(fin.skip)) if fin.skip is not None else None,
+            N.ptr(N.f32c(fin.fir)) if fin.skip is not None else None, N.ptr(img), N.ptr(frames),
+            frames.shape[2] * 3 if frames is not None else 0, fin.u8.panel * W if frames is not None else 0,
+            int(fin.u8.swap_rb) if frames is not None else 0, sat, st))
+        part = img if frames is None else frames
+        return (y, part, xs_out) if s_next is not None else (y, part)
+    _timed_conv(desc,
                 B * conv_flops(cin, cout, H, W), lambda: N.call(
         'sgdfr_modconv2d_split_f32', N.ptr(x), xb, N.ptr(wsp), N.ptr(s), N.ptr(d), N.ptr(nz), nzb,
         N.ptr(noise_weight) if nz is not None else None, N.ptr(bias), N.ptr(_zero_words(x.device)), N.ptr(y),
@@ -554,6 +578,34 @@
         self.frames, self.panel, self.swap_rb = frames, int(panel), bool(swap_rb)
 
 
+def _u8_frames(u8, B, H, W, device):
+    frames = u8.frames
+    if frames is None:
+        frames = torch.empty(B, H, W, 3, device=device, dtype=torch.uint8)
+    if frames.dtype != torch.uint8 or not frames.is_cuda or not frames.is_contiguous() or frames.ndim != 4 or \
+            frames.shape[0] != B or frames.shape[1] != H or frames.shape[3] != 3 or frames.shape[2] < (u8.panel + 1) * W:
+        raise RuntimeError('uint8 target %s cannot hold panel %d of [%d,%d,%d,3] frames' % (tuple(frames.shape), u8.panel, B, H, W))
+    return frames
+
+
+class TorgbFin:
+    __slots__ = ('bias', 'skip', 'fir', 'u8')
+
+    def __init__(self, bias=None, skip=None, fir=None, u8=None):
+        self.bias, self.skip, self.fir, self.u8 = bias, skip, fir, u8
+
+
+def fold_finish_on():
+    return os.environ.get('SGDFR_FOLD_FINISH', '1') != '0'
+
+
+def fin_foldable(B, cin, cout, H, W, x_is_split):
+    ks = _shape_query('sgdfr_modconv2d_split_ksplit_hint', B, cin, cout, H, W, N.MODE_PLAIN3) if config().use_splitk else 1
+    if ks > 1 or not fold_finish_on() or config().precision not in _SPLIT_ARITH:
+        return False
+    return bool(_shape_query('sgdfr_modconv2d_split_fin_ok', B, cin, cout, H, W, int(bool(x_is_split))))
+
+
 def torgb_finish(part, bias=None, skip=None, fir=None, u8=None):
     N.require_device(part, bias, skip, fir)
     B, c3, H, W = part.shape
@@ -561,12 +613,7 @@
         raise RuntimeError('skip shape %s does not match output [%d,3,%d,%d]/2' % (tuple(skip.shape), B, H, W))
     skip_bytes = 3 * (H // 2) * (W // 2) * 4 if skip is not None else 0
     if u8 is not None:
-        frames = u8.frames
-        if frames is None:
-            frames = torch.empty(B, H, W, 3, device=part.device, dtype=torch.uint8)
-        if frames.dtype != torch.uint8 or not frames.is_cuda or not frames.is_contiguous() or frames.ndim != 4 or \
-                frames.shape[0] != B or frames.shape[1] != H or frames.shape[3] != 3 or frames.shape[2] < (u8.panel + 1) * W:
-            raise RuntimeError('uint8 target %s cannot hold panel %d of [%d,%d,%d,3] frames' % (tuple(frames.shape), u8.panel, B, H, W))
+        frames = _u8_frames(u8, B, H, W, part.device)
         _timed_hbm('torgb_finish_u8 T=%d @%dx%d' % (c3 // 3, H, W), B * (c3 * H * W * 4 + skip_bytes + 3 * H * W), lambda: N.call(
             'sgdfr_torgb_finish_u8_f32', N.ptr(part), c3 // 3, N.ptr(N.f32c(bias)) if bias is not None else None,
             N.ptr(N.f32c(skip)) if skip is not None else None, N.ptr(N.f32c(fir)) if fir is not None else None, N.ptr(frames),
diff --git a/stylegan_directions_face_reenactment_amd/model.py b/stylegan_directions_face_reenactment_amd/model.py
--- a/stylegan_directions_face_reenactment_amd/model.py
+++ b/stylegan_directions_face_reenactment_amd/model.py
@@ -291,13 +291,14 @@
             return AG.ToRGBFn.apply(input, s, conv.weight, self.bias, skip, fir)
         return F_.torgb(input, conv.weight.view(3, conv.in_channel), s, bias=self.bias.view(3), skip=skip, fir=fir)
 
+    def skip_fir(self):
+        up = getattr(self, 'upsample', None)
+        if up is None or tuple(up.kernel.shape) != (4, 4) or up.pad != (2, 1):
+            raise NotImplementedError('ToRGB skip path is built for the 4-tap 2x Upsample')
+        return up.kernel
+
     def finish(self, part, skip=None, u8=None):
-        fir = None
-        if skip is not None:
-            up = getattr(self, 'upsample', None)
-            if up is None or tuple(up.kernel.shape) != (4, 4) or up.pad != (2, 1):
-                raise NotImplementedError('ToRGB skip path is built for the 4-tap 2x Upsample')
-            fir = up.kernel
+        fir = self.skip_fir() if skip is not None else None
         return F_.torgb_finish(part, bias=self.bias.view(3), skip=skip, fir=fir, u8=u8)
 
 
@@ -526,12 +527,25 @@
             raise RuntimeError('image_out (uint8 frames) is an inference output: call the generator under torch.no_grad()')
         wrote_u8 = [False]
 
-        def rgb(layer, x, part_in, skip_in, sdl, last=False):
+        def skip_to_main(skip_in):
+            if on_side[0]:
+                main.wait_stream(side)
+                skip_in.record_stream(main)
+                on_side[0] = False
+
+        def fin_of(layer, skip_in, last):
+            if skip_in is not None:
+                skip_to_main(skip_in)
+            u8 = image_out if (last and image_out is not None) else None
+            if u8 is not None:
+                wrote_u8[0] = True
+            return F_.TorgbFin(layer.bias.view(3), skip_in, layer.skip_fir() if skip_in is not None else None, u8)
+
+        def rgb(layer, x, part_in, skip_in, sdl, last=False, finished=False):
+            if finished:
+                return part_in
             if part_in is not None:
-                if on_side[0]:
-                    main.wait_stream(side)
-                    skip_in.record_stream(main)
-                    on_side[0] = False
+                skip_to_main(skip_in)
                 if last and image_out is not None:
                     wrote_u8[0] = True
                     return layer.finish(part_in, skip_in, u8=image_out)
@@ -558,6 +572,7 @@
             first = li == 0
             use_chain, fuse, to_next, want_y, wino_next, arith_next, xs_arith = plan[li]
             k = li // 2
+            folded = False
             if not use_chain:
                 if isinstance(x, F_.SplitAct):
                     raise RuntimeError('internal: a split activation reached a layer that cannot take it')
@@ -565,14 +580,18 @@
             else:
                 rgb_arg = (to_rgbs[k].conv.weight.view(3, c.out_channel), sd[sd_of_rgb[k]][0]) if fuse else None
                 wino_in = x.wino if isinstance(x, F_.SplitAct) else 0
+                if fuse and not up:
+                    xh, xw = x.shape[2], x.shape[3]
+                    folded = F_.fin_chain_ok(x, batch, c.in_channel, c.out_channel, xh, xw)
+                fin = fin_of(to_rgbs[k], skip, li == len(layers) - 1) if folded else None
                 out, part = F_.styled_conv_split(
                     x, c.packed_wsplit(arith=x.arith, f=wino_in) if wino_in else c.packed_split(arith=getattr(x, 'arith', None)),
                     sdl[0], sdl[1], c.out_channel, upsample=up,
                     fir=c.blur.kernel if up else None, noise=nz, noise_weight=layer.noise.weight, bias=layer.activate.bias,
                     batch=batch if first else None, s_next=sd[sd_of_layer[li + 1]][0] if to_next else None, rgb=rgb_arg,
-                    want_y=want_y, wino_next=wino_next, arith_next=arith_next, xs_arith=xs_arith)
+                    want_y=want_y, wino_next=wino_next, arith_next=arith_next, xs_arith=xs_arith, fin=fin)
             if not up:
-                skip = rgb(to_rgbs[k], out, part, skip, sd[sd_of_rgb[k]], last=li == len(layers) - 1)
+                skip = rgb(to_rgbs[k], out, part, skip, sd[sd_of_rgb[k]], last=li == len(layers) - 1, finished=folded)
             x = out
         if side is not None and on_side[0]:
             main.wait_stream(side)
```

Result: no change. 11340 (-0.6%).
